# haesungpyun/seoul_tourism_recommendation_NGCF

Hardware: NVIDIA B200
Metric: ngcf_epoch_time_fwd_bwd_bpr (lower is better)
Workload: dtype f32

## Files before the change

### include/ngcf_b200.h

```cpp
#ifndef NGCF_B200_H
#define NGCF_B200_H

#include <stddef.h>
#include <stdint.h>

#ifdef __cplusplus
extern "C" {
#endif

#define NGCF_B200_ABI_VERSION 4
#define NGCF_MAX_LAYERS 8
#define NGCF_MAX_WIDTH 128
#define NGCF_ADAM_MAX_TENSORS 32

typedef enum {
    NGCF_OK = 0,
    NGCF_ERR_INVALID = -1,
    NGCF_ERR_CUDA = -2,
    NGCF_ERR_WORKSPACE = -3
} ngcf_status;

int ngcf_abi_version(void);
const char* ngcf_last_error(void);
uint64_t ngcf_launch_count(void);

int ngcf_coo_to_csr_workspace(int64_t nnz, int64_t n_rows, size_t* bytes_host);
int ngcf_coo_to_csr(const int64_t* coo_row, const int64_t* coo_col, int64_t nnz,
                    int64_t n_rows, int64_t n_cols, int transpose,
                    int32_t* rowptr ,
                    int32_t* colidx , int32_t* perm ,
                    void* workspace, size_t workspace_bytes, void* stream);

typedef struct ngcf_csr {
    int64_t n_rows;
    const int32_t* rowptr;
    const int32_t* ent;
    const int32_t* tiles;
    const int32_t* hub_of_row;
    const int32_t* hub_chunk_ptr;
    const int32_t* chunk_ptr;
    const int32_t* hub_ent;
    const int32_t* chunk_row;
    const int32_t* chunk_tiles;
    const int32_t* hub_rows;
    int32_t* hub_done;
    const uint32_t* key_l;
    const uint32_t* key_t;
    int64_t key_row_offset;
    int32_t n_tiles, n_hub, n_chunks, n_chunk_tiles;
    int32_t rowptr_nnz;
    const uint32_t* tile_hubmask;
} ngcf_csr;

int ngcf_spmm_split_threshold(void);
int ngcf_spmm_tile_rows(void);
int ngcf_spmm_tile_entries(void);

int ngcf_edge_entries(const int32_t* colidx, const float* coo_val, const int32_t* perm, const uint8_t* keep_mask,
                      int32_t* ent_out, int64_t nnz, void* stream);

int ngcf_feature_mix(float* user_w, int64_t n_user, int d,
                     const float* const* tables_host, const int* widths_host,
                     const int64_t* const* idx_host, const int64_t* u_id, int64_t batch,
                     float ratio, int32_t* winner, void* stream);

int ngcf_spmm(const ngcf_csr* csr_host, const float* X, int64_t ldx, int d,
              const float* addend, int64_t ld_add,
              const int32_t* slot, const float* gsum, int64_t ld_gsum,
              float* hub_partial,
              float drop_p, uint64_t seed, const uint64_t* seed_dev, int layer, int transposed, int64_t row_offset,
              const uint8_t* keep_bits, const int32_t* c_ent, const int32_t* c_cnt,
              float* Y, int64_t ldy, void* stream);

int ngcf_node_dropout_bits(const ngcf_csr* csr_host, float drop_p, uint64_t seed, const uint64_t* seed_dev,
                           int n_layers, int64_t row_offset, uint8_t* bits_as_L, uint8_t* bits_as_Lt, void* stream);

int ngcf_node_dropout_compact(const ngcf_csr* csr_host, float drop_p, uint64_t seed, const uint64_t* seed_dev,
                              int n_layers, int64_t row_offset,
                              int32_t* const* ent_as_L_host, int32_t* const* cnt_as_L_host,
                              int32_t* const* ent_as_Lt_host, int32_t* const* cnt_as_Lt_host, void* stream);

int ngcf_entry_keys(const ngcf_csr* csr_host, int64_t row_offset, uint32_t* key_l, uint32_t* key_t, void* stream);

int ngcf_plgraph_entries(int64_t n_user, int64_t n_item, int64_t n_edges, double alpha, uint64_t seed,
                         int64_t row0, int64_t n_rows, unsigned long long* total_dev,
                         unsigned long long* keys_or_null, int64_t capacity, void* stream);
int ngcf_build_tiles(const int32_t* rowptr, int64_t n_rows, int max_rows, int max_ent, int32_t* next_scratch,
                     int32_t* tiles_out, int64_t capacity, int32_t* count_out, void* stream);

int ngcf_exchange_flag_words(void);
int ngcf_push_rows(float* const* matrix_on_rank_host, uint32_t* const* flags_on_rank_host, uint32_t* local_state,
                   int world, int rank, int64_t row0, int64_t n_rows, int d, float* multicast_or_null, void* stream);
int ngcf_push_selected_rows(float* const* matrix_on_rank_host, uint32_t* const* flags_on_rank_host, uint32_t* local_state,
                            int world, int rank, int64_t row0, int64_t n_rows, int d,
                            const int64_t* const* lists_host, const int64_t* list_offsets_host,
                            const int64_t* list_sizes_host, int n_lists, float* multicast_or_null, void* stream);

int ngcf_pack_weights(const float* W1, const float* b1, const float* W2, const float* b2,
                      int d_in, int d_out, float* wcat , float* bias_eff ,
                      void* stream);
int ngcf_pack_weights_all(const float* const* W1_host, const float* const* b1_host, const float* const* W2_host,
                          const float* const* b2_host, const int* d_in_host, const int* d_out_host, int n_layers,
                          float* const* wcat_host, float* const* bias_host, void* stream);
int ngcf_dense_fwd(const float* S, const float* E, int64_t n_rows, int d_in, int d_out,
                   const float* wcat, const float* bias_eff, float slope,
                   const float* mess_mult, const uint32_t* mess_bits, float mess_p, uint64_t seed,
                   const uint64_t* seed_dev, int layer, int64_t row_offset, float* E_out, void* stream);

int ngcf_mess_dropout_bits(int64_t n_rows, int d_out, float mess_p, uint64_t seed, const uint64_t* seed_dev, int layer,
                           int64_t row_offset, uint32_t* bits, void* stream);

int ngcf_gather_concat(const float* const* layers_host, const int* dims_host, int n_layers_plus1,
                       const int64_t* rows, int64_t row_offset, int64_t n_out,
                       float* out, int64_t ld_out, void* stream);
int ngcf_gather_concat_sets(const float* const* layers_host, const int* dims_host, int n_layers_plus1,
                            const int64_t* const* rows_host, const int64_t* offsets_host, const int64_t* sizes_host,
                            float* const* outs_host, int n_sets, int64_t ld_out, void* stream);

int ngcf_bpr_fwd_bwd(const float* u, const float* p, const float* n, int64_t batch, int D,
                     float weight_decay, float batch_size_ctor, float reg_w_u, float reg_w_p, float reg_w_n,
                     float* loss, float* gu, float* gp, float* gn, void* stream);

int ngcf_rowgrad_scatter(const int64_t* const* rows_host, const int64_t* offsets_host,
                         const float* const* g_host, const int64_t* batch_host, int n_sets, int D,
                         int32_t* slot, float* gsum, void* stream);
int ngcf_rowgrad_normalize(const int64_t* const* rows_host, const int64_t* offsets_host,
                           const int64_t* batch_host, int n_sets, const float* const* layers_host,
                           const int* dims_host, int n_layers_plus1, const int32_t* slot, float* gsum, int D,
                           void* stream);
int ngcf_rowgrad_reset(const int64_t* const* rows_host, const int64_t* offsets_host,
                       const int64_t* batch_host, int n_sets, int32_t* slot, void* stream);

int ngcf_set_wgrad_stream(void* stream_or_null);
int ngcf_wgrad_stream_forked(void);
int ngcf_dense_bwd(const float* gE_next, const int32_t* slot, const float* gsum, int64_t ld_gsum, int col_off,
                   const float* E_out, const float* S, const float* E, int64_t n_rows, int d_in, int d_out,
                   const float* W1, const float* W2, float slope,
                   const float* mess_mult, const uint32_t* mess_bits, float mess_p, uint64_t seed,
                   const uint64_t* seed_dev, int layer, int64_t row_offset, int gh_normalized, float* gS, float* gEl,
                   float* gW1, float* gb1, float* gW2, float* gb2, float* gM_scratch, void* stream);

int ngcf_score_topk_workspace(int64_t n_users, int64_t n_items, int D, int k, size_t* bytes_host);
int ngcf_score_topk(const float* U, int64_t n_users, const float* I, int64_t n_items, int D, int k,
                    float* out_val , int64_t* out_idx ,
                    void* workspace, size_t workspace_bytes, void* stream);
int ngcf_score_topk_excluding(const float* U, int64_t n_users, const float* I, int64_t n_items, int D, int k,
                              const int64_t* excl_ptr , const int32_t* excl_idx,
                              float* out_val , int64_t* out_idx ,
                              void* workspace, size_t workspace_bytes, void* stream);

int ngcf_rank_metrics(const int64_t* topk_idx, int64_t n_users, int k, const int64_t* truth_ptr,
                      const int32_t* truth_idx, const int* Ks_host, int n_K, float* per_user, float* totals,
                      void* stream);

int ngcf_adam_step(float* const* params_host, float* const* grads_host, float* const* exp_avg_host,
                   float* const* exp_avg_sq_host, const int64_t* sizes_host, int n_tensors, double lr, double beta1,
                   double beta2, double eps, double weight_decay, int64_t step, const int64_t* step_dev,
                   int zero_grads, void* stream);

int ngcf_eval_groups(const float* u, const float* items, const int64_t* item_ids, const float* rating,
                     const int64_t* group_ptr, int64_t n_groups, int group, int D, int k_hr, int k_ndcg, float weight_decay,
                     float batch_size_ctor, float* bpr, float* hit, float* ndcg, float* rmse, float* scores,
                     float* totals, void* stream);

int ngcf_sample_negatives(const int32_t* pos_ptr, const int32_t* pos_idx, const int64_t* row_user, int64_t n_rows,
                          const int64_t* candidates, int n_candidates, int ng_ratio, uint64_t seed, int64_t* out,
// ... 15 lines not shown
```

### seoul_tourism_recommendation_ngcf_b200/NGCF.py

```python
from __future__ import annotations

import ctypes as C
import os

import numpy as np
import torch
import torch.nn as nn

import torch.distributed as dist

from . import _lib
from .plan import LaplacianPlan, node_dropout_bits, node_dropout_compact, spmm
from .sharded import RowShards, all_gather_rows

LEAKY_SLOPE = 0.2


def _stream() -> int:
    return _lib.current_stream()


class _Ctx:
    __slots__ = ("plan", "E", "S", "dims", "vals_f", "vals_b", "mess_mult", "mess_p", "seed", "seed_dev", "masked", "drop_p", "bits_f", "bits_b", "comp_f", "comp_b", "mess_bits",
                 "rows", "offsets", "W1", "W2", "fresh_key", "node_mode", "last_partial", "fm_stream")


def _capturing() -> bool:
    return torch.cuda.is_current_stream_capturing()


def _join_feature_mix(st):
    if st.fm_stream is not None:
        torch.cuda.current_stream().wait_stream(st.fm_stream)
        st.fm_stream = None


class _Propagate(torch.autograd.Function):

    @staticmethod
    def forward(ctx, mod, st: _Ctx, n_sets, user_w, item_w, *wb):
        lib = _lib.load()
        K = mod.n_layer
        W1, b1, W2, b2 = wb[0:K], wb[K:2 * K], wb[2 * K:3 * K], wb[3 * K:4 * K]
        dev = user_w.device
        sh = mod._shard
        N = mod.n_user + mod.n_item
        r0, nloc, nv = (sh.r0, sh.rows, sh.valid) if sh is not None else (0, N, N)
        X0 = mod._packed_table()
        if mod._snapshot:
            _join_feature_mix(st)
            X0 = X0.clone()
        st.E, st.S, st.W1, st.W2 = [X0], [], list(W1), list(W2)
        side = st.plan.fwd
        st.bits_f = st.bits_b = st.comp_f = st.comp_b = None
        st.node_mode = mod._node_mode
        st.last_partial = None
        if st.drop_p > 0:
            shared = st.plan.side(True, False) is side
            node_mode = mod._node_mode if all(d % 4 == 0 for d in st.dims) or mod._node_mode == "inkernel" else "bits"
            st.node_mode = node_mode
            if node_mode == "compact":
                st.comp_f, ct = node_dropout_compact(side, st.drop_p, st.seed, st.seed_dev, K, r0, as_L=True, as_Lt=shared)
                if shared:
                    st.comp_b = ct
            elif node_mode == "bits":
                st.bits_f, bt = node_dropout_bits(side, st.drop_p, st.seed, st.seed_dev, K, r0, as_L=True, as_Lt=shared)
                if shared:
                    st.bits_b = bt
        self_uses_mess_bits = mod._mess_bits
        st.mess_bits = [None] * K
        for k in range(K):
            if self_uses_mess_bits and st.mess_mult is None and st.mess_p[k] > 0 and st.dims[k + 1] % 4 == 0:
                bits = torch.empty(nloc * ((st.dims[k + 1] + 31) // 32), dtype=torch.int32, device=dev)
                _lib.check(lib.ngcf_mess_dropout_bits(nv, st.dims[k + 1], float(st.mess_p[k]), st.seed,
                                                      _lib.ptr(st.seed_dev), k, r0, bits.data_ptr(), _stream()),
                           "mess_dropout_bits")
                st.mess_bits[k] = bits
        wcats = [torch.empty(2 * st.dims[k] * st.dims[k + 1], dtype=torch.float32, device=dev) for k in range(K)]
        biases = [torch.empty(st.dims[k + 1], dtype=torch.float32, device=dev) for k in range(K)]
        _lib.check(lib.ngcf_pack_weights_all(_lib.ptr_array(W1), _lib.ptr_array(b1), _lib.ptr_array(W2), _lib.ptr_array(b2),
                                             _lib.int_array(st.dims[:K]), _lib.int_array(st.dims[1:]), K,
                                             _lib.ptr_array(wcats), _lib.ptr_array(biases), _stream()), "pack_weights_all")
        _join_feature_mix(st)
        for k in range(K):
            d_in, d_out = st.dims[k], st.dims[k + 1]
            vals = st.vals_f[k] if st.vals_f is not None else None
            S = spmm(side, vals, st.E[k], d_in, drop_p=st.drop_p, seed=st.seed, seed_dev=st.seed_dev, layer=k,
                     row_offset=r0, keep_bits=st.bits_f,
                     compact=st.comp_f[k] if st.comp_f is not None else None)
            wcat, bias = wcats[k], biases[k]
            xkey = None
            if sh is None:
                Xn = En = torch.empty(N, d_out, dtype=torch.float32, device=dev)
            elif mod._xchg is not None and d_out % 4 == 0:
                xkey = ("E", k + 1)
                Xn = mod._xchg.matrix(xkey, sh.N_pad, d_out)
                En = Xn[r0:r0 + nloc]
            else:
                Xn = torch.empty(sh.N_pad, d_out, dtype=torch.float32, device=dev)
                En = torch.zeros(nloc, d_out, dtype=torch.float32, device=dev) if nv < nloc else \
                    torch.empty(nloc, d_out, dtype=torch.float32, device=dev)
            mm = st.mess_mult[k] if st.mess_mult is not None else None
            E_loc = st.E[k][r0:r0 + nloc]
            _lib.check(lib.ngcf_dense_fwd(S.data_ptr(), E_loc.data_ptr(), nv, d_in, d_out, wcat.data_ptr(),
                                          bias.data_ptr(), LEAKY_SLOPE, _lib.ptr(mm[r0:r0 + nloc] if mm is not None else None),
                                          _lib.ptr(st.mess_bits[k]), float(st.mess_p[k]), st.seed, _lib.ptr(st.seed_dev), k, r0, En.data_ptr(),
                                          _stream()),
                       "dense_fwd")
            if xkey is not None and k == K - 1:
                mod._xchg.push_selected(xkey, r0, nloc, st.rows[:n_sets], st.offsets[:n_sets])
                st.last_partial = xkey
            elif xkey is not None:
                mod._xchg.push(xkey, r0, nloc)
            elif sh is not None:
                all_gather_rows(Xn, En, mod._group)
            st.S.append(S)
            st.E.append(Xn)
        D = sum(st.dims)
        layers, dims = _lib.ptr_array(st.E), _lib.int_array(st.dims)
        outs = [torch.empty(st.rows[j].numel(), D, dtype=torch.float32, device=dev) for j in range(n_sets)]
        _lib.check(lib.ngcf_gather_concat_sets(layers, dims, K + 1, _lib.ptr_array(st.rows[:n_sets]),
                                               _lib.i64_array(st.offsets[:n_sets]),
                                               _lib.i64_array([r.numel() for r in st.rows[:n_sets]]), _lib.ptr_array(outs),
                                               n_sets, D, _stream()), "gather_concat_sets")
        ctx.st, ctx.mod, ctx.n_sets = st, mod, n_sets
        return tuple(outs)

    @staticmethod
    def backward(ctx, *gouts):
        lib = _lib.load()
        st, mod, n_sets = ctx.st, ctx.mod, ctx.n_sets
        mod._check_fresh(st, "loss.backward()")
        K, dims = mod.n_layer, st.dims
        dev = st.E[0].device
        sh = mod._shard
        N = mod.n_user + mod.n_item
        r0, nloc, nv, N_all = (sh.r0, sh.rows, sh.valid, sh.N_pad) if sh is not None else (0, N, N, N)
        D = sum(dims)
        g = [(go.contiguous() if go is not None else torch.zeros(st.rows[j].numel(), D, device=dev))
             for j, go in enumerate(gouts)]
        batch = [r.numel() for r in st.rows[:n_sets]]
        rows_h, offs_h = _lib.ptr_array(st.rows[:n_sets]), _lib.i64_array(st.offsets[:n_sets])
        g_h, batch_h = _lib.ptr_array(g), _lib.i64_array(batch)
        slot = mod._slot_map(N_all, dev)
        gsum = torch.empty(sum(batch), D, dtype=torch.float32, device=dev)
        _lib.check(lib.ngcf_rowgrad_scatter(rows_h, offs_h, g_h, batch_h, n_sets, D, slot.data_ptr(),
                                            gsum.data_ptr(), _stream()), "rowgrad_scatter")
        _lib.check(lib.ngcf_rowgrad_normalize(rows_h, offs_h, batch_h, n_sets, _lib.ptr_array(st.E), _lib.int_array(dims),
                                              K + 1, slot.data_ptr(), gsum.data_ptr(), D, _stream()), "rowgrad_normalize")
        slot_loc = slot[r0:r0 + nloc]
        sizes = [dims[k + 1] * dims[k] for k in range(K)]
        n_flat = 2 * sum(sizes) + 2 * sum(dims[1:])
        if sh is not None and mod._xchg is not None:
            f_pad = (n_flat + 3) // 4 * 4
            wg_all = mod._xchg.matrix(("wgrad", f_pad), sh.world, f_pad)
            flat = wg_all[sh.rank, :n_flat]
            flat.zero_()
        else:
            wg_all = None
            flat = torch.zeros(n_flat, dtype=torch.float32, device=dev)
        gW1, gW2, gb1, gb2, o = [], [], [], [], 0
        for k in range(K):
            gW1.append(flat[o:o + sizes[k]].view(dims[k + 1], dims[k])); o += sizes[k]
            gW2.append(flat[o:o + sizes[k]].view(dims[k + 1], dims[k])); o += sizes[k]
            gb1.append(flat[o:o + dims[k + 1]]); o += dims[k + 1]
            gb2.append(flat[o:o + dims[k + 1]]); o += dims[k + 1]
        side = st.plan.side(True, st.vals_b is not None)
        if st.drop_p > 0 and st.node_mode == "compact" and st.comp_b is None:
            _, st.comp_b = node_dropout_compact(side, st.drop_p, st.seed, st.seed_dev, K, r0, as_L=False, as_Lt=True)
        if st.drop_p > 0 and st.node_mode == "bits" and st.bits_b is None:
            _, st.bits_b = node_dropout_bits(side, st.drop_p, st.seed, st.seed_dev, K, r0, as_L=False, as_Lt=True)
        gE_next = None
        col_off = D
        overlap = _capturing() or (sh is not None and mod._xchg is not None)
        if overlap:
            if mod._side_stream is None:
                mod._side_stream = torch.cuda.Stream(device=dev)
            _lib.check(lib.ngcf_set_wgrad_stream(mod._side_stream.cuda_stream), "set_wgrad_stream")
            lib.ngcf_wgrad_stream_forked()
            gM_keep = []
        else:
            gM_scratch = torch.empty(nloc, max(dims[1:]), dtype=torch.float32, device=dev)
        for k in range(K - 1, -1, -1):
            d_in, d_out = dims[k], dims[k + 1]
            col_off -= d_out
            peer = sh is not None and mod._xchg is not None and d_in % 4 == 0
            if peer:
                gS_all = mod._xchg.matrix(("gS", d_in), N_all, d_in)
                gS = gS_all[r0:r0 + nloc]
            else:
                gS = torch.empty(nloc, d_in, dtype=torch.float32, device=dev)
            if peer and k == 0:
                gE0_all = mod._xchg.matrix(("gE0", d_in), N_all, d_in)
                gEl = gE0_all[r0:r0 + nloc]
            else:
                gEl = torch.empty(nloc, d_in, dtype=torch.float32, device=dev)
            mm = st.mess_mult[k] if st.mess_mult is not None else None
            if overlap:
                gM_scratch = torch.empty(nloc, dims[k + 1], dtype=torch.float32, device=dev)
                gM_keep.append(gM_scratch)
            _lib.check(lib.ngcf_dense_bwd(_lib.ptr(gE_next), slot_loc.data_ptr(), gsum.data_ptr(), D, col_off,
                                          st.E[k + 1][r0:r0 + nloc].data_ptr(), st.S[k].data_ptr(),
                                          st.E[k][r0:r0 + nloc].data_ptr(), nv, d_in, d_out,
                                          st.W1[k].data_ptr(), st.W2[k].data_ptr(), LEAKY_SLOPE,
                                          _lib.ptr(mm[r0:r0 + nloc] if mm is not None else None),
                                          _lib.ptr(st.mess_bits[k]), float(st.mess_p[k]), st.seed,
                                          _lib.ptr(st.seed_dev), k, r0, 1, gS.data_ptr(),
                                          gEl.data_ptr(),
                                          gW1[k].data_ptr(), gb1[k].data_ptr(), gW2[k].data_ptr(), gb2[k].data_ptr(),
                                          gM_scratch.data_ptr(), _stream()), "dense_bwd")
            if peer:
                mod._xchg.push(("gS", d_in), r0, nloc)
            elif sh is not None:
                gS_all = torch.empty(N_all, d_in, dtype=torch.float32, device=dev)
                all_gather_rows(gS_all, gS, mod._group)
            else:
                gS_all = gS
            vals = st.vals_b[k] if st.vals_b is not None else None
            last = (k == 0)
            gE_next = spmm(side, vals, gS_all, d_in, addend=gEl, slot=slot_loc if last else None,
                           gsum=gsum if last else None, drop_p=st.drop_p, seed=st.seed, seed_dev=st.seed_dev, layer=k,
                           transposed=True, row_offset=r0, keep_bits=st.bits_b,
                           compact=st.comp_b[k] if st.comp_b is not None else None)
            if mod._trace is not None:
                mod._trace.append(dict(k=k, gS=gS.clone(), gEl=gEl.clone(), gE=gE_next.clone()))
        if overlap:
            _lib.check(lib.ngcf_set_wgrad_stream(None), "set_wgrad_stream")
            if lib.ngcf_wgrad_stream_forked():
                torch.cuda.current_stream().wait_stream(mod._side_stream)
        _lib.check(lib.ngcf_rowgrad_reset(rows_h, offs_h, batch_h, n_sets, slot.data_ptr(), _stream()),
                   "rowgrad_reset")
        if sh is not None:
            if mod._xchg is not None and dims[0] % 4 == 0:
                mod._xchg.push(("gE0", dims[0]), r0, nloc)
                gE0 = gE0_all.clone()
            else:
                gE0 = torch.empty(N_all, dims[0], dtype=torch.float32, device=dev)
                all_gather_rows(gE0, gE_next, mod._group)
            if wg_all is not None:
                mod._xchg.push(("wgrad", wg_all.shape[1]), sh.rank, 1)
                total = wg_all.sum(0)[:n_flat]
                gW1, gW2, gb1, gb2, o = [], [], [], [], 0
                for k in range(K):
                    gW1.append(total[o:o + sizes[k]].view(dims[k + 1], dims[k])); o += sizes[k]
                    gW2.append(total[o:o + sizes[k]].view(dims[k + 1], dims[k])); o += sizes[k]
                    gb1.append(total[o:o + dims[k + 1]]); o += dims[k + 1]
                    gb2.append(total[o:o + dims[k + 1]]); o += dims[k + 1]
            else:
                dist.all_reduce(flat, group=mod._group)
        else:
            gE0 = gE_next
        gU, gI = gE0[:mod.n_user], gE0[mod.n_user:N]
        return (None, None, None, gU, gI, *gW1, *gb1, *gW2, *gb2)


class NGCF(nn.Module):

    def __init__(self, embed_size: int, layer_size: list, node_dropout: float, mess_dropout: list,
                 emb_ratio: float, lap_list: list, num_dict: dict, batch_size: int, device, *, rng: str = "device",
                 snapshot: bool = False):
        super().__init__()
        if rng not in ("device", "reference"):
            raise ValueError("rng must be 'device' or 'reference'")
        self.n_user = int(num_dict['user'])
        self.n_item = int(num_dict['item'])
        self.emb_size = int(embed_size)
        self.weight_size = list(layer_size)
        self.n_layer = len(self.weight_size)
# ... 59 lines not shown
        self.w2_list = nn.Sequential(*w2)
        self.node_dropout_list = nn.Sequential(*nd)
        self.mess_dropout_list = nn.Sequential(*md)

    def shard(self, group=None, shards=None):
        if not dist.is_initialized():
            raise RuntimeError("NGCF.shard() needs an initialised torch.distributed process group")
        if self.rng != "device":
            raise ValueError("row-sharded runs need rng='device' (masks are keyed on global coordinates in-kernel)")
        world, rank = dist.get_world_size(group), dist.get_rank(group)
        self._shard = shards if shards is not None else RowShards(self.n_user + self.n_item, world, rank)
        if self._shard.N != self.n_user + self.n_item or self._shard.world != world or self._shard.rank != rank:
            raise ValueError("the shard descriptor does not match this model / process group")
        self._group = group
        self._plans, self._table, self._slot = {}, None, None
        self._xchg = None
        if world > 1 and os.environ.get("NGCF_B200_EXCHANGE", "peer") != "nccl":
            try:
                from .sharded import PeerExchange
                self._xchg = PeerExchange(group, self.user_embedding.weight.device)
            except Exception as e:
                self._xchg_error = f"{type(e).__name__}: {e}"
                ok = torch.tensor([0], device=self.user_embedding.weight.device)
            else:
                ok = torch.tensor([1], device=self.user_embedding.weight.device)
            dist.all_reduce(ok, op=dist.ReduceOp.MIN, group=group)
            if int(ok) == 0:
                self._xchg = None
        if self._xchg is None and world > 1 and not getattr(self._shard, "equal", True):
            raise RuntimeError("unequal row blocks (BalancedShards) need the peer-memory exchange, which is not available "
                               "here: " + getattr(self, "_xchg_error", "disabled by NGCF_B200_EXCHANGE=nccl"))
        return self

    def exchange_description(self) -> str:
        if self._shard is None:
            return "single GPU"
        if self._xchg is not None:
            how = "NVLS multicast stores (multimem.st)" if self._xchg.multicast() else "peer-memory stores"
            return (f"contiguous row blocks; per-layer exchange of E / gS / table-gradient rows by {how} over NVLink "
                    "(ngcf_push_rows on symmetric memory, no NCCL collective anywhere in the step; the last layer's "
                    "output travels for the batch rows only; W/b gradients: one more push + a rank-ordered sum)")
        return "equal row blocks, per-layer NCCL all-gather of E / gS, all-reduce of W/b grads"

    def _packed_table(self) -> torch.Tensor:
        u, i = self.user_embedding.weight, self.item_embedding.weight
        d = self.emb_size
        adjacent = (u.is_contiguous() and i.is_contiguous() and u.dtype == torch.float32 and
                    u.data_ptr() + self.n_user * d * 4 == i.data_ptr() and
                    getattr(self, "_table", None) is not None and self._table.data_ptr() == u.data_ptr())
        if not adjacent:
            n_rows = self._shard.N_pad if self._shard is not None else self.n_user + self.n_item
            table = torch.zeros(n_rows, d, dtype=torch.float32, device=u.device)
            table[:self.n_user].copy_(u.data)
            table[self.n_user:self.n_user + self.n_item].copy_(i.data)
            u.data = table[:self.n_user]
            i.data = table[self.n_user:self.n_user + self.n_item]
            self._table = table
        return self._table if self._shard is None else self._table

    def _slot_map(self, N, dev):
        if self._slot is None or self._slot.device != dev or self._slot.numel() != N:
            self._slot = torch.full((N,), -1, dtype=torch.int32, device=dev)
        return self._slot

    def _plan(self, year_idx: int, dev) -> LaplacianPlan:
        L = self.lap_list[year_idx]
        p = self._plans.get(year_idx)
        if p is None or p.src is not L or p.coo_val.device != dev:
            p = LaplacianPlan(L, dev, shard=self._shard)
            self._plans[year_idx] = p
        return p

    def _reference_node_masks(self, nnz: int, dev):
        alive = np.arange(nnz)
        out = []
        for _ in range(self.n_layer):
            m = nn.Dropout(self.node_dropout)(torch.tensor(np.ones(alive.size))).type(torch.bool).numpy()
            alive = alive[m]
            full = np.zeros(nnz, dtype=np.uint8)
            full[alive] = 1
            out.append(torch.from_numpy(full).to(dev))
        return out

    @_lib.on_device
    def forward(self, year, u_id, age, sex, month, day, dow, pos_item, neg_item, node_flag):
        lib = _lib.load()
        dev = self.user_embedding.weight.device
        if dev.type != "cuda":
            raise RuntimeError("NGCF (B200) runs on a CUDA device only; there is no CPU fallback. "
                               "Move the module with .to('cuda').")
        K, N = self.n_layer, self.n_user + self.n_item
        if (self._side_stream is None or self._side_stream.device != dev) and not _capturing():
            self._side_stream, self._side_stream3 = (torch.cuda.Stream(device=dev) for _ in range(2))

        def ix(t):
            return t.to(device=dev, dtype=torch.int64).contiguous()

        u_id, pos_item = ix(u_id), ix(pos_item)
        feats_idx = [ix(age), ix(sex), ix(month), ix(day), ix(dow)]
        has_neg = len(neg_item) > 0
        neg_item = ix(neg_item) if has_neg else None
        year_idx = int(year.min()) % 18

        table = self._packed_table()
        if self._winner is None or self._winner.device != dev or self._winner.numel() != self.n_user:
            self._winner = torch.full((self.n_user,), -1, dtype=torch.int32, device=dev)
        tabs = [self.age_emb.weight, self.sex_emb.weight, self.month_emb.weight, self.day_emb.weight, self.dow_emb.weight]
        def mix():
            _lib.check(lib.ngcf_feature_mix(table.data_ptr(), self.n_user, self.emb_size, _lib.ptr_array(tabs),
                                            _lib.int_array(self.feat_widths), _lib.ptr_array(feats_idx), u_id.data_ptr(),
                                            u_id.numel(), float(self.emb_ratio), self._winner.data_ptr(), _stream()),
                       "feature_mix")

        fm_stream = None
        if self._shard is None and _capturing() and bool(node_flag) and \
                (self.node_dropout or 0) > 0 and self.rng == "device":
            main = torch.cuda.current_stream()
            if self._side_stream3 is None:
                self._side_stream3 = torch.cuda.Stream(device=dev)
            self._side_stream3.wait_stream(main)
            with torch.cuda.stream(self._side_stream3):
                mix()
            fm_stream = self._side_stream3
        else:
            mix()

        self._mix_count += 1
        st = _Ctx()
        st.fm_stream = fm_stream
        st.fresh_key = self._fresh_key()
        st.plan = plan = self._plan(year_idx, dev)
        if self._shard is not None and "edge_keep" in (self._inject or {}):
            raise ValueError("explicit edge masks are not supported in row-sharded mode")
        if plan.N != N:
            raise ValueError(f"Laplacian is {plan.N}x{plan.N} but n_user+n_item = {N}")
        st.dims = [self.emb_size] + self.weight_size
        inj = self._inject or {}
        st.masked = bool(node_flag) and (self.node_dropout is not None) and \
            (self.node_dropout > 0 or "edge_keep" in inj)
        st.vals_f = st.vals_b = None
        st.drop_p = 0.0
        masks = None
        if st.masked:
            if "edge_keep" in inj:
                masks = [m.to(device=dev, dtype=torch.uint8).contiguous() for m in inj["edge_keep"]]
            elif self.rng == "reference":
                masks = self._reference_node_masks(plan.nnz, dev)
            else:
                st.drop_p = float(self.node_dropout)
        st.mess_mult = None
        st.mess_p = [0.0] * K
        if "mess_mult" in inj:
            st.mess_mult = [m.to(device=dev, dtype=torch.float32).contiguous() for m in inj["mess_mult"]]
        elif self.training and self.mess_dropout is not None:
            st.mess_p = [float(p) for p in self.mess_dropout[:K]]
        need_seed = st.drop_p > 0 or any(p > 0 for p in st.mess_p)
        if not need_seed:
            st.seed = 0
        elif self.rng == "reference":
            if self._seed_gen is None:
                self._seed_gen = torch.Generator().manual_seed(torch.initial_seed() & (2 ** 63 - 1))
            st.seed = int(torch.randint(0, 2 ** 62, (1,), generator=self._seed_gen).item())
        else:
            st.seed = int(torch.randint(0, 2 ** 62, (1,)).item())
        st.seed_dev = self._seed_dev if need_seed else None
        if masks is not None:
            st.vals_f = [plan.entries(plan.fwd, masks[k]) for k in range(K)]
            st.vals_b = [plan.entries(plan.bwd, masks[k]) for k in range(K)]
        st.rows = [u_id, pos_item] + ([neg_item] if has_neg else [])
        st.offsets = [0, self.n_user] + ([self.n_user] if has_neg else [])

        wb = [l.weight for l in self.w1_list] + [l.bias for l in self.w1_list] + \
             [l.weight for l in self.w2_list] + [l.bias for l in self.w2_list]
        outs = _Propagate.apply(self, st, len(st.rows), self.user_embedding.weight, self.item_embedding.weight, *wb)
        self._last, self._all_E = st, None
        u_embeddings, pos_i_embeddings = outs[0], outs[1]
        neg_i_embeddings = outs[2] if has_neg else torch.empty(0)
        return u_embeddings, pos_i_embeddings, neg_i_embeddings

    def _fresh_key(self):
        return (self._mix_count, _lib.param_epoch(), self.user_embedding.weight._version,
                self.item_embedding.weight._version)

    def _check_fresh(self, st, what: str):
        if self._snapshot or st.fresh_key == self._fresh_key():
            return
        why = "the step that produced it also ran the optimizer" if st.fresh_key is None else \
            "another forward (feature mix) or an optimizer step ran since"
        raise RuntimeError(f"NGCF (B200): {what} needs the embedding table as the forward left it, but {why}. "
                           "Run the forward again, or construct the module with snapshot=True to keep a per-forward "
                           "copy like the reference's torch.cat (NGCF.py:120).")

    @_lib.on_device
    def _materialize(self):
        if self._last is None:
            raise AttributeError("all_users_emb / all_items_emb exist after the first forward (NGCF.py:148-149)")
        if self._all_E is None:
            self._check_fresh(self._last, "all_users_emb / all_items_emb")
            if self._last.last_partial is not None:
                sh = self._shard
                self._xchg.push(self._last.last_partial, sh.r0, sh.rows)
                self._last.last_partial = None
            st, lib = self._last, _lib.load()
            N, D = self.n_user + self.n_item, sum(st.dims)
            out = torch.empty(N, D, dtype=torch.float32, device=st.E[0].device)
            _lib.check(lib.ngcf_gather_concat(_lib.ptr_array(st.E), _lib.int_array(st.dims), self.n_layer + 1, None, 0,
                                              N, out.data_ptr(), D, _stream()), "gather_concat")
            self._all_E = out
        return self._all_E

    @property
    def all_users_emb(self):
        return self._materialize()[:self.n_user, :]

    @property
    def all_items_emb(self):
        return self._materialize()[self.n_user:, :]
```

### seoul_tourism_recommendation_ngcf_b200/_lib.py

```python
from __future__ import annotations

import ctypes as C
import os

_PKG = os.path.dirname(os.path.abspath(__file__))
LIB_PATH = os.environ.get("NGCF_B200_LIB") or os.path.join(_PKG, "libngcf_b200.so")

_vp, _i64, _i32, _f32, _u64, _sz = C.c_void_p, C.c_int64, C.c_int32, C.c_float, C.c_uint64, C.c_size_t



class NgcfCsr(C.Structure):
    _fields_ = [("n_rows", _i64), ("rowptr", _vp), ("ent", _vp), ("tiles", _vp),
                ("hub_of_row", _vp), ("hub_chunk_ptr", _vp), ("chunk_ptr", _vp), ("hub_ent", _vp),
                ("chunk_row", _vp), ("chunk_tiles", _vp), ("hub_rows", _vp), ("hub_done", _vp), ("key_l", _vp), ("key_t", _vp), ("key_row_offset", _i64),
                ("n_tiles", _i32), ("n_hub", _i32), ("n_chunks", _i32),
                ("n_chunk_tiles", _i32), ("rowptr_nnz", _i32), ("tile_hubmask", _vp)]


_csr_p = C.POINTER(NgcfCsr)

SIGNATURES = {
    "ngcf_abi_version": [],
    "ngcf_last_error": [],
    "ngcf_launch_count": [],
    "ngcf_coo_to_csr_workspace": [_i64, _i64, C.POINTER(_sz)],
    "ngcf_coo_to_csr": [_vp, _vp, _i64, _i64, _i64, C.c_int, _vp, _vp, _vp, _vp, _sz, _vp],
    "ngcf_edge_entries": [_vp, _vp, _vp, _vp, _vp, _i64, _vp],
    "ngcf_spmm_tile_rows": [],
    "ngcf_spmm_tile_entries": [],
    "ngcf_feature_mix": [_vp, _i64, C.c_int, C.POINTER(_vp), C.POINTER(C.c_int), C.POINTER(_vp), _vp, _i64, _f32,
                         _vp, _vp],
    "ngcf_spmm_split_threshold": [],
    "ngcf_spmm": [_csr_p, _vp, _i64, C.c_int, _vp, _i64, _vp, _vp, _i64, _vp, _f32, _u64, _vp, C.c_int, C.c_int, _i64,
                  _vp, _vp, _vp, _vp, _i64, _vp],
    "ngcf_entry_keys": [_csr_p, _i64, _vp, _vp, _vp],
    "ngcf_node_dropout_compact": [_csr_p, _f32, _u64, _vp, C.c_int, _i64, C.POINTER(_vp), C.POINTER(_vp), C.POINTER(_vp),
                                  C.POINTER(_vp), _vp],
    "ngcf_node_dropout_bits": [_csr_p, _f32, _u64, _vp, C.c_int, _i64, _vp, _vp, _vp],
    "ngcf_pack_weights": [_vp, _vp, _vp, _vp, C.c_int, C.c_int, _vp, _vp, _vp],
    "ngcf_pack_weights_all": [C.POINTER(_vp), C.POINTER(_vp), C.POINTER(_vp), C.POINTER(_vp), C.POINTER(C.c_int),
                              C.POINTER(C.c_int), C.c_int, C.POINTER(_vp), C.POINTER(_vp), _vp],
    "ngcf_dense_fwd": [_vp, _vp, _i64, C.c_int, C.c_int, _vp, _vp, _f32, _vp, _vp, _f32, _u64, _vp, C.c_int, _i64, _vp,
                       _vp],
    "ngcf_mess_dropout_bits": [_i64, C.c_int, _f32, _u64, _vp, C.c_int, _i64, _vp, _vp],
    "ngcf_gather_concat": [C.POINTER(_vp), C.POINTER(C.c_int), C.c_int, _vp, _i64, _i64, _vp, _i64, _vp],
    "ngcf_gather_concat_sets": [C.POINTER(_vp), C.POINTER(C.c_int), C.c_int, C.POINTER(_vp), C.POINTER(_i64), C.POINTER(_i64),
                                C.POINTER(_vp), C.c_int, _i64, _vp],
    "ngcf_bpr_fwd_bwd": [_vp, _vp, _vp, _i64, C.c_int, _f32, _f32, _f32, _f32, _f32, _vp, _vp, _vp, _vp, _vp],
    "ngcf_rowgrad_scatter": [C.POINTER(_vp), C.POINTER(_i64), C.POINTER(_vp), C.POINTER(_i64), C.c_int, C.c_int, _vp,
                             _vp, _vp],
    "ngcf_rowgrad_reset": [C.POINTER(_vp), C.POINTER(_i64), C.POINTER(_i64), C.c_int, _vp, _vp],
    "ngcf_dense_bwd": [_vp, _vp, _vp, _i64, C.c_int, _vp, _vp, _vp, _i64, C.c_int, C.c_int, _vp, _vp, _f32, _vp, _vp, _f32,
                       _u64, _vp, C.c_int, _i64, C.c_int, _vp, _vp, _vp, _vp, _vp, _vp, _vp, _vp],
    "ngcf_set_wgrad_stream": [_vp],
    "ngcf_wgrad_stream_forked": [],
    "ngcf_rowgrad_normalize": [C.POINTER(_vp), C.POINTER(_i64), C.POINTER(_i64), C.c_int, C.POINTER(_vp),
                               C.POINTER(C.c_int), C.c_int, _vp, _vp, C.c_int, _vp],
    "ngcf_adam_step": [C.POINTER(_vp), C.POINTER(_vp), C.POINTER(_vp), C.POINTER(_vp), C.POINTER(_i64), C.c_int,
                       C.c_double, C.c_double, C.c_double, C.c_double, C.c_double, _i64, _vp, C.c_int, _vp],
    "ngcf_debug_bwd_timeline": [C.c_int, _vp],
    "ngcf_debug_spmm_timeline": [_vp],
    "ngcf_debug_compact_timeline": [_vp],
    "ngcf_score_topk_workspace": [_i64, _i64, C.c_int, C.c_int, C.POINTER(_sz)],
    "ngcf_eval_groups": [_vp, _vp, _vp, _vp, _vp, _i64, C.c_int, C.c_int, C.c_int, C.c_int, _f32, _f32, _vp, _vp, _vp, _vp, _vp,
                         _vp, _vp],
    "ngcf_sample_negatives": [_vp, _vp, _vp, _i64, _vp, C.c_int, C.c_int, _u64, _vp, _vp, _vp],
    "ngcf_laplacian_entries": [_vp, _vp, _vp, _i64, _i64, _i64, _vp, _vp, _vp, _vp, _vp],
    "ngcf_plgraph_entries": [_i64, _i64, _i64, C.c_double, _u64, _i64, _i64, _vp, _vp, _i64, _vp],
    "ngcf_build_tiles": [_vp, _i64, C.c_int, C.c_int, _vp, _vp, _i64, _vp, _vp],
    "ngcf_exchange_flag_words": [],
    "ngcf_push_rows": [C.POINTER(_vp), C.POINTER(_vp), _vp, C.c_int, C.c_int, _i64, _i64, C.c_int, _vp, _vp],
    "ngcf_push_selected_rows": [C.POINTER(_vp), C.POINTER(_vp), _vp, C.c_int, C.c_int, _i64, _i64, C.c_int, C.POINTER(_vp),
                                C.POINTER(_i64), C.POINTER(_i64), C.c_int, _vp, _vp],
    "ngcf_score_topk": [_vp, _i64, _vp, _i64, C.c_int, C.c_int, _vp, _vp, _vp, _sz, _vp],
    "ngcf_score_topk_excluding": [_vp, _i64, _vp, _i64, C.c_int, C.c_int, _vp, _vp, _vp, _vp, _vp, _sz, _vp],
    "ngcf_rank_metrics": [_vp, _i64, C.c_int, _vp, _vp, C.POINTER(C.c_int), C.c_int, _vp, _vp, _vp],
}

_lib = None


def load() -> C.CDLL:
    global _lib
    if _lib is not None:
        return _lib
    if not os.path.exists(LIB_PATH):
        raise RuntimeError(
            f"{LIB_PATH} is missing: the NGCF B200 hot path has no CPU/PyTorch fallback. "
            "Build it with `python -m seoul_tourism_recommendation_ngcf_b200.build` (needs nvcc, targets sm_100a).")
    lib = C.CDLL(LIB_PATH)
    for name, argtypes in SIGNATURES.items():
        fn = getattr(lib, name)
        fn.argtypes = argtypes
        fn.restype = {"ngcf_last_error": C.c_char_p, "ngcf_launch_count": C.c_uint64}.get(name, C.c_int)
    _lib = lib
    return lib


def check(rc: int, what: str = "") -> None:
    if rc != 0:
        msg = load().ngcf_last_error()
        raise RuntimeError(f"ngcf_b200 {what} failed (status {rc}): {msg.decode() if msg else '?'}")


def ptr(t) -> int | None:
    return None if t is None else t.data_ptr()


def ptr_array(tensors):
    return (_vp * len(tensors))(*[None if t is None else t.data_ptr() for t in tensors])


def ptr_array_int(addrs):
    return (_vp * len(addrs))(*[int(a) for a in addrs])


def int_array(vals):
    return (C.c_int * len(vals))(*[int(v) for v in vals])


# ... 48 lines not shown
```

### seoul_tourism_recommendation_ngcf_b200/csrc/bpr.cu

```cuda
#include "common.cuh"

namespace {

struct GatherArgs {
    const float* layer[NGCF_MAX_LAYERS + 1];
    int dim[NGCF_MAX_LAYERS + 1];
    int n;
    const int64_t* rows;
    int64_t row_offset;
    int64_t n_out;
    float* out;
    int64_t ld_out;
};

struct GatherSetsArgs {
    const float* layer[NGCF_MAX_LAYERS + 1];
    int dim[NGCF_MAX_LAYERS + 1];
    int n;
    const int64_t* rows[4];
    int64_t row_offset[4];
    int64_t base[5];
    float* out[4];
    int n_sets;
    int64_t ld_out;
// ... 30 lines not shown
    if (b >= a.n_out) return;
    gather_row(a, (a.rows ? a.rows[b] : b) + a.row_offset, a.out + b * a.ld_out, lane);
}
__global__ void gather_concat_sets_kernel(GatherSetsArgs a) {
    const int64_t b = (blockIdx.x * (int64_t)blockDim.x + threadIdx.x) >> 5;
    const int lane = threadIdx.x & 31;
    if (b >= a.base[a.n_sets]) return;
    int j = 0;
    while (b >= a.base[j + 1]) ++j;
    const int64_t i = b - a.base[j];
    gather_row(a, a.rows[j][i] + a.row_offset[j], a.out[j] + i * a.ld_out, lane);
}

constexpr int BPR_WARPS = 8;

__global__ void __launch_bounds__(BPR_WARPS * 32)
bpr_kernel(const float* __restrict__ u, const float* __restrict__ p, const float* __restrict__ n, int64_t batch, int D,
           float wd, float wu, float wp, float wn, float inv_bs, float* __restrict__ loss, float* __restrict__ gu,
           float* __restrict__ gp, float* __restrict__ gn) {
    __shared__ float part[BPR_WARPS];
    const int warp = threadIdx.x >> 5, lane = threadIdx.x & 31;
    const int64_t b = (int64_t)blockIdx.x * BPR_WARPS + warp;
    float contrib = 0.f;
    if (b < batch) {
        const float* ur = u + b * D;
        const float* pr = p + b * D;
        const float* nr = n + b * D;
        float xp = 0.f, xn = 0.f, su = 0.f, sp = 0.f, sn = 0.f;
        for (int c = lane; c < D; c += 32) {
            const float a = ur[c], bb = pr[c], cc = nr[c];
            xp = fmaf(a, bb, xp); xn = fmaf(a, cc, xn);
            su = fmaf(a, a, su); sp = fmaf(bb, bb, sp); sn = fmaf(cc, cc, sn);
        }
        xp = warp_sum(xp); xn = warp_sum(xn); su = warp_sum(su); sp = warp_sum(sp); sn = warp_sum(sn);
        const float x = fabsf(xp) - fabsf(xn);
        const float logsig = fminf(x, 0.f) - log1pf(expf(-fabsf(x)));
        contrib = (-logsig + wd * (wu * su + wp * sp + wn * sn)) * inv_bs;
        if (gu) {
            const float c = -1.f / (1.f + expf(x));
            const float sgp = xp > 0.f ? 1.f : (xp < 0.f ? -1.f : 0.f);
            const float sgn = xn > 0.f ? 1.f : (xn < 0.f ? -1.f : 0.f);
            const float cp = c * sgp * inv_bs, cn = -c * sgn * inv_bs;
            const float ru = 2.f * wd * wu * inv_bs, rp = 2.f * wd * wp * inv_bs, rn = 2.f * wd * wn * inv_bs;
            for (int col = lane; col < D; col += 32) {
                const float a = ur[col], bb = pr[col], cc = nr[col];
                gu[b * D + col] = cp * bb + cn * cc + ru * a;
                gp[b * D + col] = cp * a + rp * bb;
                gn[b * D + col] = cn * a + rn * cc;
            }
        }
    }
    if (lane == 0) part[warp] = contrib;
    __syncthreads();
    if (threadIdx.x == 0) {
        float s = 0.f;
#pragma unroll
        for (int w = 0; w < BPR_WARPS; ++w) s += part[w];
        atomicAdd(loss, s);
    }
}

struct RowSets {
    const int64_t* rows[4];
    int64_t offset[4];
    const float* g[4];
    int64_t batch[4];
    int64_t base[4];
    int n_sets;
    int64_t total;
};

__device__ __forceinline__ bool locate(const RowSets& s, int64_t i, int& j, int64_t& b) {
    if (i >= s.total) return false;
    j = 0;
    while (j + 1 < s.n_sets && i >= s.base[j + 1]) ++j;
    b = i - s.base[j];
    return true;
}

__global__ void rowgrad_claim_kernel(RowSets s, int32_t* __restrict__ slot) {
    const int64_t i = blockIdx.x * (int64_t)blockDim.x + threadIdx.x;
    int j; int64_t b;
    if (!locate(s, i, j, b)) return;
    slot[s.rows[j][b] + s.offset[j]] = (int32_t)i;
}

__global__ void rowgrad_accum_kernel(RowSets s, int D, const int32_t* __restrict__ slot, float* __restrict__ gsum) {
    const int64_t i = (blockIdx.x * (int64_t)blockDim.x + threadIdx.x) >> 5;
    const int lane = threadIdx.x & 31;
    int j; int64_t b;
    if (!locate(s, i, j, b)) return;
    const int32_t w = slot[s.rows[j][b] + s.offset[j]];
    const float* g = s.g[j] + b * D;
    float* dst = gsum + (int64_t)w * D;
    for (int c = lane; c < D; c += 32) atomicAdd(dst + c, g[c]);
}

struct NormArgs {
    const float* layer[NGCF_MAX_LAYERS + 1];
    int dim[NGCF_MAX_LAYERS + 1];
    int n;
};
__global__ void rowgrad_normalize_kernel(RowSets s, NormArgs L, int D, const int32_t* __restrict__ slot,
                                         float* __restrict__ gsum) {
    const int64_t i = (blockIdx.x * (int64_t)blockDim.x + threadIdx.x) >> 5;
    const int lane = threadIdx.x & 31;
    int j; int64_t b;
    if (!locate(s, i, j, b)) return;
    const int64_t row = s.rows[j][b] + s.offset[j];
    if (slot[row] != (int32_t)i) return;
    float* g = gsum + i * D;
    int col = L.dim[0];
    for (int k = 1; k < L.n; ++k) {
        const int d = L.dim[k];
        const float* e = L.layer[k] + row * d;
        float nrm2 = 0.f, dot = 0.f;
        for (int c = lane; c < d; c += 32) {
            nrm2 = fmaf(e[c], e[c], nrm2);
            dot = fmaf(e[c], g[col + c], dot);
        }
        nrm2 = warp_sum(nrm2);
        dot = warp_sum(dot);
        const float n = fmaxf(sqrtf(nrm2), 1e-12f);
        const float hd = dot / n;
        for (int c = lane; c < d; c += 32) g[col + c] = (g[col + c] - (e[c] / n) * hd) / n;
        col += d;
    }
}

__global__ void rowgrad_reset_kernel(RowSets s, int32_t* __restrict__ slot) {
    const int64_t i = blockIdx.x * (int64_t)blockDim.x + threadIdx.x;
    int j; int64_t b;
    if (!locate(s, i, j, b)) return;
    slot[s.rows[j][b] + s.offset[j]] = -1;
}

int fill_sets(RowSets& s, const int64_t* const* rows_host, const int64_t* offsets_host, const float* const* g_host,
              const int64_t* batch_host, int n_sets) {
    NGCF_REQUIRE(rows_host && offsets_host && batch_host, "rowgrad: null host array");
    NGCF_REQUIRE(n_sets >= 1 && n_sets <= 4, "rowgrad: n_sets %d not in [1,4]", n_sets);
    s.n_sets = n_sets;
    s.total = 0;
    for (int j = 0; j < 4; ++j) {
        s.rows[j] = nullptr; s.g[j] = nullptr; s.offset[j] = 0; s.batch[j] = 0; s.base[j] = 0;
    }
    for (int j = 0; j < n_sets; ++j) {
        NGCF_REQUIRE(batch_host[j] >= 0 && (batch_host[j] == 0 || rows_host[j]), "rowgrad: set %d has no rows", j);
        s.rows[j] = rows_host[j];
        s.offset[j] = offsets_host[j];
        s.g[j] = g_host ? g_host[j] : nullptr;
        s.batch[j] = batch_host[j];
        s.base[j] = s.total;
        s.total += batch_host[j];
    }
    NGCF_REQUIRE(s.total < ((int64_t)1 << 31), "rowgrad: too many rows");
    return NGCF_OK;
}

}

extern "C" int ngcf_gather_concat(const float* const* layers_host, const int* dims_host, int n_layers_plus1,
                                  const int64_t* rows, int64_t row_offset, int64_t n_out, float* out, int64_t ld_out,
                                  void* stream) {
    NGCF_REQUIRE(layers_host && dims_host && out, "gather_concat: null pointer");
    NGCF_REQUIRE(n_layers_plus1 >= 1 && n_layers_plus1 <= NGCF_MAX_LAYERS + 1, "gather_concat: %d blocks", n_layers_plus1);
    GatherArgs a;
    int D = 0;
    for (int k = 0; k < n_layers_plus1; ++k) {
        NGCF_REQUIRE(layers_host[k] && dims_host[k] > 0 && dims_host[k] <= NGCF_MAX_WIDTH, "gather_concat: bad block %d", k);
        a.layer[k] = layers_host[k];
        a.dim[k] = dims_host[k];
        D += dims_host[k];
    }
    NGCF_REQUIRE(ld_out >= D, "gather_concat: ld_out %lld < total width %d", (long long)ld_out, D);
    a.n = n_layers_plus1; a.rows = rows; a.row_offset = row_offset; a.n_out = n_out; a.out = out; a.ld_out = ld_out;
    if (n_out <= 0) return NGCF_OK;
    gather_concat_kernel<<<(unsigned)ceil_div64(n_out * 32, 256), 256, 0, as_stream(stream)>>>(a);
    NGCF_LAUNCH_OK("gather_concat_kernel");
    return NGCF_OK;
}

extern "C" int ngcf_gather_concat_sets(const float* const* layers_host, const int* dims_host, int n_layers_plus1,
                                       const int64_t* const* rows_host, const int64_t* offsets_host,
                                       const int64_t* sizes_host, float* const* outs_host, int n_sets, int64_t ld_out,
                                       void* stream) {
    NGCF_REQUIRE(layers_host && dims_host && rows_host && offsets_host && sizes_host && outs_host, "gather_concat_sets: null pointer");
    NGCF_REQUIRE(n_layers_plus1 >= 1 && n_layers_plus1 <= NGCF_MAX_LAYERS + 1, "gather_concat_sets: %d blocks", n_layers_plus1);
    NGCF_REQUIRE(n_sets >= 1 && n_sets <= 4, "gather_concat_sets: n_sets %d not in [1,4]", n_sets);
    GatherSetsArgs a{};
    int D = 0;
    for (int k = 0; k < n_layers_plus1; ++k) {
        NGCF_REQUIRE(layers_host[k] && dims_host[k] > 0 && dims_host[k] <= NGCF_MAX_WIDTH, "gather_concat_sets: bad block %d", k);
        a.layer[k] = layers_host[k];
        a.dim[k] = dims_host[k];
        D += dims_host[k];
    }
    NGCF_REQUIRE(ld_out >= D, "gather_concat_sets: ld_out %lld < total width %d", (long long)ld_out, D);
    a.n = n_layers_plus1; a.n_sets = n_sets; a.ld_out = ld_out;
    int64_t total = 0;
    for (int j = 0; j < n_sets; ++j) {
        NGCF_REQUIRE(sizes_host[j] >= 0 && (sizes_host[j] == 0 || (rows_host[j] && outs_host[j])), "gather_concat_sets: set %d", j);
        a.rows[j] = rows_host[j]; a.row_offset[j] = offsets_host[j]; a.out[j] = outs_host[j];
        a.base[j] = total;
        total += sizes_host[j];
    }
    for (int j = n_sets; j <= 4; ++j) a.base[j] = total;
    if (total == 0) return NGCF_OK;
    gather_concat_sets_kernel<<<(unsigned)ceil_div64(total * 32, 256), 256, 0, as_stream(stream)>>>(a);
    NGCF_LAUNCH_OK("gather_concat_sets_kernel");
    return NGCF_OK;
}

extern "C" int ngcf_bpr_fwd_bwd(const float* u, const float* p, const float* n, int64_t batch, int D,
                                float weight_decay, float batch_size_ctor, float reg_w_u, float reg_w_p,
                                float reg_w_n, float* loss, float* gu, float* gp, float* gn, void* stream) {
    NGCF_REQUIRE(u && p && n && loss, "bpr: null pointer");
    NGCF_REQUIRE((gu && gp && gn) || (!gu && !gp && !gn), "bpr: give all three gradient buffers or none");
    NGCF_REQUIRE(batch >= 0 && D > 0 && batch_size_ctor != 0.f, "bpr: bad sizes");
    cudaStream_t st = as_stream(stream);
    NGCF_CUDA(cudaMemsetAsync(loss, 0, sizeof(float), st));
    if (batch == 0) return NGCF_OK;
    bpr_kernel<<<(unsigned)ceil_div64(batch, BPR_WARPS), BPR_WARPS * 32, 0, st>>>(
        u, p, n, batch, D, weight_decay, reg_w_u, reg_w_p, reg_w_n, 1.0f / batch_size_ctor, loss, gu, gp, gn);
    NGCF_LAUNCH_OK("bpr_kernel");
    return NGCF_OK;
}

extern "C" int ngcf_rowgrad_scatter(const int64_t* const* rows_host, const int64_t* offsets_host,
                                    const float* const* g_host, const int64_t* batch_host, int n_sets, int D,
                                    int32_t* slot, float* gsum, void* stream) {
    NGCF_REQUIRE(g_host && slot && gsum && D > 0, "rowgrad_scatter: null pointer");
    RowSets s;
    int rc = fill_sets(s, rows_host, offsets_host, g_host, batch_host, n_sets);
    if (rc != NGCF_OK) return rc;
    for (int j = 0; j < n_sets; ++j) NGCF_REQUIRE(s.batch[j] == 0 || s.g[j], "rowgrad_scatter: set %d has no gradient", j);
    if (s.total == 0) return NGCF_OK;
    cudaStream_t st = as_stream(stream);
    NGCF_CUDA(cudaMemsetAsync(gsum, 0, sizeof(float) * (size_t)s.total * D, st));
    rowgrad_claim_kernel<<<(unsigned)ceil_div64(s.total, 256), 256, 0, st>>>(s, slot);
    NGCF_LAUNCH_OK("rowgrad_claim_kernel");
    rowgrad_accum_kernel<<<(unsigned)ceil_div64(s.total * 32, 256), 256, 0, st>>>(s, D, slot, gsum);
    NGCF_LAUNCH_OK("rowgrad_accum_kernel");
    return NGCF_OK;
}

extern "C" int ngcf_rowgrad_normalize(const int64_t* const* rows_host, const int64_t* offsets_host,
                                      const int64_t* batch_host, int n_sets, const float* const* layers_host,
                                      const int* dims_host, int n_layers_plus1, const int32_t* slot, float* gsum,
                                      int D, void* stream) {
    NGCF_REQUIRE(slot && gsum && layers_host && dims_host, "rowgrad_normalize: null pointer");
    NGCF_REQUIRE(n_layers_plus1 >= 1 && n_layers_plus1 <= NGCF_MAX_LAYERS + 1, "rowgrad_normalize: %d blocks", n_layers_plus1);
    RowSets s;
    int rc = fill_sets(s, rows_host, offsets_host, nullptr, batch_host, n_sets);
    if (rc != NGCF_OK) return rc;
    NormArgs L;
    int total = 0;
    for (int k = 0; k < n_layers_plus1; ++k) {
        NGCF_REQUIRE(layers_host[k] && dims_host[k] > 0 && dims_host[k] <= NGCF_MAX_WIDTH, "rowgrad_normalize: bad block %d", k);
        L.layer[k] = layers_host[k];
        L.dim[k] = dims_host[k];
        total += dims_host[k];
    }
    L.n = n_layers_plus1;
    NGCF_REQUIRE(total == D, "rowgrad_normalize: block widths sum to %d, D = %d", total, D);
    if (s.total == 0 || n_layers_plus1 == 1) return NGCF_OK;
    rowgrad_normalize_kernel<<<(unsigned)ceil_div64(s.total * 32, 256), 256, 0, as_stream(stream)>>>(s, L, D, slot, gsum);
    NGCF_LAUNCH_OK("rowgrad_normalize_kernel");
    return NGCF_OK;
}

extern "C" int ngcf_rowgrad_reset(const int64_t* const* rows_host, const int64_t* offsets_host,
                                  const int64_t* batch_host, int n_sets, int32_t* slot, void* stream) {
    NGCF_REQUIRE(slot, "rowgrad_reset: null pointer");
    RowSets s;
    int rc = fill_sets(s, rows_host, offsets_host, nullptr, batch_host, n_sets);
    if (rc != NGCF_OK) return rc;
    if (s.total == 0) return NGCF_OK;
    rowgrad_reset_kernel<<<(unsigned)ceil_div64(s.total, 256), 256, 0, as_stream(stream)>>>(s, slot);
    NGCF_LAUNCH_OK("rowgrad_reset_kernel");
    return NGCF_OK;
}
```

### seoul_tourism_recommendation_ngcf_b200/csrc/dense.cu

```cuda
#include "common.cuh"

namespace {

__global__ void pack_weights_kernel(const float* __restrict__ W1, const float* __restrict__ b1,
                                    const float* __restrict__ W2, const float* __restrict__ b2, int d_in, int d_out,
                                    float* __restrict__ wcat, float* __restrict__ bias_eff) {
    const int total = 2 * d_in * d_out;
    for (int i = blockIdx.x * blockDim.x + threadIdx.x; i < total; i += gridDim.x * blockDim.x) {
        const int k = i / d_out, o = i % d_out;
        wcat[i] = k < d_in ? W1[o * d_in + k] : W2[o * d_in + (k - d_in)];
    }
    for (int o = blockIdx.x * blockDim.x + threadIdx.x; o < d_out; o += gridDim.x * blockDim.x)
        bias_eff[o] = 2.0f * b1[o] + b2[o];
}

struct PackAllArgs {
    const float* W1[NGCF_MAX_LAYERS];
    const float* b1[NGCF_MAX_LAYERS];
    const float* W2[NGCF_MAX_LAYERS];
    const float* b2[NGCF_MAX_LAYERS];
    float* wcat[NGCF_MAX_LAYERS];
    float* bias[NGCF_MAX_LAYERS];
    int d_in[NGCF_MAX_LAYERS], d_out[NGCF_MAX_LAYERS];
};
// ... 330 lines not shown
                               fmaf(t2[r][2], e4.z, t1[r][2]), fmaf(t2[r][3], e4.w, t1[r][3])};
                float ge[4] = {fmaf(t2[r][0], s4.x, t1[r][0]), fmaf(t2[r][1], s4.y, t1[r][1]),
                               fmaf(t2[r][2], s4.z, t1[r][2]), fmaf(t2[r][3], s4.w, t1[r][3])};
                if (vec_in) {
                    st_f4(a.gS + row * d_in + j0, make_float4(gs[0], gs[1], gs[2], gs[3]));
                    st_f4(a.gEl + row * d_in + j0, make_float4(ge[0], ge[1], ge[2], ge[3]));
                } else {
#pragma unroll
                    for (int c = 0; c < 4; ++c)
                        if (j0 + c < d_in) {
                            a.gS[row * d_in + j0 + c] = gs[c];
                            a.gEl[row * d_in + j0 + c] = ge[c];
                        }
                }
            }
        }

        for (int r = 0; r < R; ++r) {
            const float4 s4 = ld_f4(Ss + r * LD + tx * 4), e4 = ld_f4(Es + r * LD + tx * 4);
            const float x1[4] = {s4.x + e4.x, s4.y + e4.y, s4.z + e4.z, s4.w + e4.w};
            const float x2[4] = {s4.x * e4.x, s4.y * e4.y, s4.z * e4.z, s4.w * e4.w};
#pragma unroll
            for (int q = 0; q < OB; ++q) {
                const float4 g4 = ld_f4(GM + r * LD + (ty + TY * q) * 4);
                const float g[4] = {g4.x, g4.y, g4.z, g4.w};
#pragma unroll
                for (int o = 0; o < 4; ++o)
#pragma unroll
                    for (int j = 0; j < 4; ++j) {
                        accW1[q][o][j] = fmaf(g[o], x1[j], accW1[q][o][j]);
                        accW2[q][o][j] = fmaf(g[o], x2[j], accW2[q][o][j]);
                    }
            }
        }
    }

#pragma unroll
    for (int q = 0; q < OB; ++q)
#pragma unroll
        for (int o = 0; o < 4; ++o) {
            const int oo = (ty + TY * q) * 4 + o;
            if (oo >= d_out) continue;
#pragma unroll
            for (int j = 0; j < 4; ++j) {
                const int jj = tx * 4 + j;
                if (jj < d_in) {
                    atomicAdd(a.gW1 + oo * d_in + jj, accW1[q][o][j]);
                    atomicAdd(a.gW2 + oo * d_in + jj, accW2[q][o][j]);
                }
            }
        }
    __syncthreads();
#pragma unroll
    for (int q = 0; q < QN; ++q) CS[warp * DC + lane + 32 * q] = colsum[q];
    __syncthreads();
    for (int c = tid; c < d_out; c += THREADS) {
        float s = 0.f;
        for (int w = 0; w < NW; ++w) s += CS[w * DC + c];
        atomicAdd(a.gb2 + c, s);
        atomicAdd(a.gb1 + c, 2.0f * s);
    }
}

template <typename K>
int set_smem(K kernel, size_t bytes) {
    if (bytes > 48 * 1024) {
        cudaError_t e = cudaFuncSetAttribute(kernel, cudaFuncAttributeMaxDynamicSharedMemorySize, (int)bytes);
        if (e != cudaSuccess) {
            ngcf_set_error("cudaFuncSetAttribute(%zu bytes smem) failed: %s", bytes, cudaGetErrorString(e));
            return NGCF_ERR_CUDA;
        }
    }
    return NGCF_OK;
}

inline bool aligned16(const void* p) { return (reinterpret_cast<uintptr_t>(p) & 15) == 0; }

}

bool ngcf_dense_fwd_tc_eligible(int d_in, int d_out);
int ngcf_dense_fwd_tc(const float* S, const float* E, int64_t n_rows, int d_in, int d_out, const float* wcat,
                      const float* bias_eff, float slope, const float* mess_mult, const uint32_t* mess_bits, float mess_p,
                      uint64_t seed,
                      const uint64_t* seed_dev, int layer, int64_t row_offset, float* E_out, cudaStream_t st);

bool ngcf_dense_bwd_tc_eligible(int d_in, int d_out, int gh_normalized);
int ngcf_dense_bwd_tc(const float* gE_next, const int32_t* slot, const float* gsum, int64_t ld_gsum, int col_off,
                      const float* E_out, const float* S, const float* E, int64_t n_rows, int d_in, int d_out,
                      const float* W1, const float* W2, float slope, const float* mess_mult, const uint32_t* mess_bits,
                      float mess_p,
                      uint64_t seed, const uint64_t* seed_dev, int layer, int64_t row_offset, int gh_normalized, float* gS, float* gEl,
                      float* gW1, float* gb1, float* gW2, float* gb2, float* gM_scratch, cudaStream_t st);

extern "C" int ngcf_pack_weights(const float* W1, const float* b1, const float* W2, const float* b2, int d_in,
                                 int d_out, float* wcat, float* bias_eff, void* stream) {
    NGCF_REQUIRE(W1 && b1 && W2 && b2 && wcat && bias_eff, "pack_weights: null pointer");
    NGCF_REQUIRE(d_in > 0 && d_in <= NGCF_MAX_WIDTH && d_out > 0 && d_out <= NGCF_MAX_WIDTH,
                 "pack_weights: widths %d -> %d not in [1,%d]", d_in, d_out, NGCF_MAX_WIDTH);
    pack_weights_kernel<<<32, 256, 0, as_stream(stream)>>>(W1, b1, W2, b2, d_in, d_out, wcat, bias_eff);
    NGCF_LAUNCH_OK("pack_weights_kernel");
    return NGCF_OK;
}

extern "C" int ngcf_pack_weights_all(const float* const* W1_host, const float* const* b1_host, const float* const* W2_host,
                                     const float* const* b2_host, const int* d_in_host, const int* d_out_host, int n_layers,
                                     float* const* wcat_host, float* const* bias_host, void* stream) {
    NGCF_REQUIRE(W1_host && b1_host && W2_host && b2_host && d_in_host && d_out_host && wcat_host && bias_host,
                 "pack_weights_all: null pointer");
    NGCF_REQUIRE(n_layers >= 1 && n_layers <= NGCF_MAX_LAYERS, "pack_weights_all: %d layers", n_layers);
    PackAllArgs a{};
    for (int l = 0; l < n_layers; ++l) {
        NGCF_REQUIRE(W1_host[l] && b1_host[l] && W2_host[l] && b2_host[l] && wcat_host[l] && bias_host[l],
                     "pack_weights_all: null pointer (layer %d)", l);
        NGCF_REQUIRE(d_in_host[l] > 0 && d_in_host[l] <= NGCF_MAX_WIDTH && d_out_host[l] > 0 && d_out_host[l] <= NGCF_MAX_WIDTH,
                     "pack_weights_all: widths %d -> %d not in [1,%d]", d_in_host[l], d_out_host[l], NGCF_MAX_WIDTH);
        a.W1[l] = W1_host[l]; a.b1[l] = b1_host[l]; a.W2[l] = W2_host[l]; a.b2[l] = b2_host[l];
        a.wcat[l] = wcat_host[l]; a.bias[l] = bias_host[l]; a.d_in[l] = d_in_host[l]; a.d_out[l] = d_out_host[l];
    }
    pack_weights_all_kernel<<<dim3(32, (unsigned)n_layers), 256, 0, as_stream(stream)>>>(a);
    NGCF_LAUNCH_OK("pack_weights_all_kernel");
    return NGCF_OK;
}

extern "C" int ngcf_dense_fwd(const float* S, const float* E, int64_t n_rows, int d_in, int d_out, const float* wcat,
                              const float* bias_eff, float slope, const float* mess_mult, const uint32_t* mess_bits, float mess_p,
                      uint64_t seed,
                              const uint64_t* seed_dev, int layer, int64_t row_offset, float* E_out, void* stream) {
    NGCF_REQUIRE(S && E && wcat && bias_eff && E_out, "dense_fwd: null pointer");
    NGCF_REQUIRE(d_in > 0 && d_in <= NGCF_MAX_WIDTH && d_out > 0 && d_out <= NGCF_MAX_WIDTH,
                 "dense_fwd: widths %d -> %d not in [1,%d]", d_in, d_out, NGCF_MAX_WIDTH);
    NGCF_REQUIRE(mess_p >= 0.f && mess_p < 1.f, "dense_fwd: mess_p %f not in [0,1)", mess_p);
    NGCF_REQUIRE(n_rows >= 0 && n_rows < ((int64_t)1 << 31), "dense_fwd: n_rows %lld", (long long)n_rows);
    if (n_rows == 0) return NGCF_OK;
    if (ngcf_dense_fwd_tc_eligible(d_in, d_out) && aligned16(S) && aligned16(E) &&
        aligned16(E_out) && (!mess_mult || aligned16(mess_mult)))
        return ngcf_dense_fwd_tc(S, E, n_rows, d_in, d_out, wcat, bias_eff, slope, mess_mult, mess_bits, mess_p, seed, seed_dev,
                                 layer, row_offset, E_out, as_stream(stream));
    FwdArgs a{S, E, n_rows, d_in, d_out, wcat, bias_eff, slope, mess_mult, mess_bits, mess_p, seed, seed_dev, layer, E_out,
              (2 * d_in + 3) & ~3, (int)ceil_div64(n_rows, FWD_R), row_offset};
    const int ncg = d_out <= 64 ? 1 : 2;
    const size_t smem = sizeof(float) * ((size_t)a.KP * 64 * ncg + (size_t)FWD_R * (a.KP + 4) + 64 * ncg);
    const int per_sm = smem > 110 * 1024 ? 1 : (smem > 72 * 1024 ? 2 : 3);
    const int grid = (int)min((int64_t)a.n_tiles, (int64_t)ngcf_num_sms() * per_sm);
    int rc;
    if (ncg == 1) {
        if ((rc = set_smem(dense_fwd_kernel<1>, smem)) != NGCF_OK) return rc;
        dense_fwd_kernel<1><<<grid, FWD_THREADS, smem, as_stream(stream)>>>(a);
    } else {
        if ((rc = set_smem(dense_fwd_kernel<2>, smem)) != NGCF_OK) return rc;
        dense_fwd_kernel<2><<<grid, FWD_THREADS, smem, as_stream(stream)>>>(a);
    }
    NGCF_LAUNCH_OK("dense_fwd_kernel");
    return NGCF_OK;
}

extern "C" int ngcf_dense_bwd(const float* gE_next, const int32_t* slot, const float* gsum, int64_t ld_gsum,
                              int col_off, const float* E_out, const float* S, const float* E, int64_t n_rows,
                              int d_in, int d_out, const float* W1, const float* W2, float slope,
                              const float* mess_mult, const uint32_t* mess_bits, float mess_p, uint64_t seed,
                              const uint64_t* seed_dev, int layer, int64_t row_offset, int gh_normalized, float* gS,
                              float* gEl, float* gW1, float* gb1, float* gW2, float* gb2, float* gM_scratch, void* stream) {
    NGCF_REQUIRE(E_out && S && E && W1 && W2 && gS && gEl && gW1 && gb1 && gW2 && gb2, "dense_bwd: null pointer");
    NGCF_REQUIRE(!slot || gsum, "dense_bwd: slot given without gsum");
    NGCF_REQUIRE(d_in > 0 && d_in <= NGCF_MAX_WIDTH && d_out > 0 && d_out <= NGCF_MAX_WIDTH,
                 "dense_bwd: widths %d -> %d not in [1,%d]", d_in, d_out, NGCF_MAX_WIDTH);
    NGCF_REQUIRE(mess_p >= 0.f && mess_p < 1.f, "dense_bwd: mess_p %f not in [0,1)", mess_p);
    NGCF_REQUIRE(n_rows >= 0 && n_rows < ((int64_t)1 << 31), "dense_bwd: n_rows %lld", (long long)n_rows);
    if (n_rows == 0) return NGCF_OK;
    if (gM_scratch && ngcf_dense_bwd_tc_eligible(d_in, d_out, gh_normalized) && aligned16(S) &&
        aligned16(E) && aligned16(gS) && aligned16(gEl) && aligned16(gM_scratch))
        return ngcf_dense_bwd_tc(gE_next, slot, gsum, ld_gsum, col_off, E_out, S, E, n_rows, d_in, d_out, W1, W2,
                                 slope, mess_mult, mess_bits, mess_p, seed, seed_dev, layer, row_offset, gh_normalized, gS,
                                 gEl, gW1, gb1, gW2, gb2, gM_scratch, as_stream(stream));
    BwdArgs a{gE_next, slot, gsum, ld_gsum, col_off, E_out, S, E, n_rows, d_in, d_out, W1, W2, slope, mess_mult,
              mess_bits, mess_p, seed, seed_dev, layer, gS, gEl, gW1, gb1, gW2, gb2, 0, row_offset, gh_normalized};
    int rc;
    if (d_in <= 64 && d_out <= 64) {
        constexpr int DC = 64, R = 64, T = 256;
        a.n_tiles = (int)ceil_div64(n_rows, R);
        const size_t smem = sizeof(float) * (2 * DC * DC + 3 * R * (DC + 4) + (T / 32) * DC);
        const int grid = (int)min((int64_t)a.n_tiles, (int64_t)ngcf_num_sms() * 2);
        if ((rc = set_smem(dense_bwd_kernel<DC, R, T>, smem)) != NGCF_OK) return rc;
        dense_bwd_kernel<DC, R, T><<<grid, T, smem, as_stream(stream)>>>(a);
    } else {
        constexpr int DC = 128, R = 32, T = 512;
        a.n_tiles = (int)ceil_div64(n_rows, R);
        const size_t smem = sizeof(float) * (2 * DC * DC + 3 * R * (DC + 4) + (T / 32) * DC);
        const int grid = (int)min((int64_t)a.n_tiles, (int64_t)ngcf_num_sms());
        if ((rc = set_smem(dense_bwd_kernel<DC, R, T>, smem)) != NGCF_OK) return rc;
        dense_bwd_kernel<DC, R, T><<<grid, T, smem, as_stream(stream)>>>(a);
    }
    NGCF_LAUNCH_OK("dense_bwd_kernel");
    return NGCF_OK;
}

namespace {
__global__ void mess_bits_kernel(int64_t n_rows, int d_out, int words, float p, uint64_t seed0, const uint64_t* seed_dev,
                                 int layer, int64_t row_off, uint32_t* __restrict__ bits) {
    const int64_t i = blockIdx.x * (int64_t)blockDim.x + threadIdx.x;
    if (i >= n_rows * words) return;
    const int64_t row = i / words;
    const int w = (int)(i % words);
    const uint64_t seed = ngcf_seed(seed0, seed_dev);
    uint32_t out = 0;
#pragma unroll
    for (int q = 0; q < 8; ++q) {
        const int col = w * 32 + q * 4;
        if (col < d_out) {
            const float4 m = mess_multiplier4(p, seed, layer, (uint64_t)((row + row_off) * d_out + col) >> 2);
            out |= (m.x != 0.f ? 1u : 0u) << (q * 4) | (m.y != 0.f ? 2u : 0u) << (q * 4) | (m.z != 0.f ? 4u : 0u) << (q * 4) |
                   (m.w != 0.f ? 8u : 0u) << (q * 4);
        }
    }
    bits[i] = out;
}
}

extern "C" int ngcf_mess_dropout_bits(int64_t n_rows, int d_out, float mess_p, uint64_t seed, const uint64_t* seed_dev,
                                      int layer, int64_t row_offset, uint32_t* bits, void* stream) {
    NGCF_REQUIRE(bits && n_rows >= 0, "mess_dropout_bits: null pointer");
    NGCF_REQUIRE(d_out > 0 && d_out <= NGCF_MAX_WIDTH && d_out % 4 == 0, "mess_dropout_bits: width %d", d_out);
    NGCF_REQUIRE(mess_p > 0.f && mess_p < 1.f, "mess_dropout_bits: mess_p %f not in (0,1)", mess_p);
    if (n_rows == 0) return NGCF_OK;
    const int words = (d_out + 31) / 32;
    mess_bits_kernel<<<(unsigned)ceil_div64(n_rows * words, 256), 256, 0, as_stream(stream)>>>(
        n_rows, d_out, words, mess_p, seed, seed_dev, layer, row_offset, bits);
    NGCF_LAUNCH_OK("mess_bits_kernel");
    return NGCF_OK;
}
```

### seoul_tourism_recommendation_ngcf_b200/csrc/dense_tc.cu

```cuda
#include <stdlib.h>

#include "tc.cuh"
#include "tmap.h"

namespace {

using namespace tc;

__device__ long long g_bwd_dbg[4][8][8];
__device__ int g_bwd_dbg_on = 0;
#define BWD_STAMP(role, it, k)                                                   \
    do {                                                                         \
        if (dbg && lane == 0 && (it) < 8) g_bwd_dbg[role][it][k] = clock64();    \
    } while (0)

constexpr int TC_ROWS = 128;
constexpr int TC_EPI_WARPS = 4;
constexpr int TC_LOAD_WARPS = 8;
constexpr int TC_THREADS = (TC_EPI_WARPS + 1 + TC_LOAD_WARPS) * 32;
constexpr int TC_MAX_KB = 4;
constexpr int TC_A_BLOCK = TC_ROWS * 128;

struct FwdTcArgs {
    const float* S;
    const float* E;
    int64_t n_rows;
    int d_in, d_out;
    const float* wcat;
    const float* bias_eff;
    float slope;
    const float* mess_mult;
    const uint32_t* mess_bits;
    float mess_p;
    uint64_t seed;
    const uint64_t* seed_dev;
    int layer;
    float* E_out;
    int n_tiles;
    int64_t row_off;
    int64_t ld_in;
    int in_off, w_row1, w_row2, out_off, d_out_full, mode;
};
enum { FW_SINGLE = 0, FW_PARTIAL = 1, FW_FINAL = 2 };

constexpr int FW_EPI_WARPS = 8;
constexpr int FW_MMA_WARP = FW_EPI_WARPS;

__device__ __forceinline__ int stage_off(int r, int c) { return r * 32 + ((c ^ (r & 7)) << 2); }

enum { MM_NONE = 0, MM_MULT = 1, MM_BITS = 2, MM_HASH = 3 };
static inline int mess_mode(const float* mess_mult, const uint32_t* mess_bits, float mess_p) {
    return mess_mult ? MM_MULT : (mess_p > 0.f ? (mess_bits ? MM_BITS : MM_HASH) : MM_NONE);
}

template <int MM>
__device__ __forceinline__ void fwd_epilogue_role(const FwdTcArgs& a, float* stage, const float* bias_s, uint64_t* tmem_full,
                                                  uint64_t* tmem_empty, uint32_t tmem_base, int n_my, int warp, int lane,
                                                  bool dbg) {
    const int d_out = a.d_out;
    const uint64_t seed = MM == MM_HASH ? ngcf_seed(a.seed, a.seed_dev) : 0ull;
    const uint32_t thr = ngcf_threshold16(a.mess_p);
    float* st = stage + warp * 32 * 32;
    const int quarter = warp & 3, c = warp >> 2;
    const int rr = lane >> 3, c4 = lane & 7;
    const bool has_chunk = c * 32 < d_out;
    const float inv_keep = 1.0f / (1.0f - a.mess_p);
    for (int it = 0; it < n_my; ++it) {
        const int tile = blockIdx.x + it * gridDim.x;
        const int buf = it & 1;
        BWD_STAMP(0, it, 0);
        mbar_wait(&tmem_full[buf], (it >> 1) & 1);
        BWD_STAMP(0, it, 1);
        tc_fence_after_sync();
        float v[32];
        if (has_chunk) tmem_ld_32x32(tmem_base + ((uint32_t)(quarter * 32) << 16) + buf * 64 + c * 32, v);
        tc_fence_before_sync();
        __syncwarp();
        if (lane == 0) mbar_arrive(&tmem_empty[buf]);
        BWD_STAMP(0, it, 3);
        if (!has_chunk) continue;
        const int64_t row_base = (int64_t)tile * TC_ROWS + quarter * 32;
#pragma unroll
        for (int j = 0; j < 32; j += 4)
            st_f4(st + stage_off(lane, j >> 2), make_float4(v[j], v[j + 1], v[j + 2], v[j + 3]));
        __syncwarp();
        float4 r4[8];
#pragma unroll
        for (int i = 0; i < 8; ++i) r4[i] = ld_f4(st + stage_off(i * 4 + rr, c4));
        __syncwarp();
        BWD_STAMP(0, it, 4);
        const int col = c * 32 + c4 * 4;
        if (col < d_out) {
            const int gcol = a.out_off + col;
            const float4 b4 = *reinterpret_cast<const float4*>(bias_s + col);
            const int words = (a.d_out_full + 31) >> 5;
#pragma unroll
            for (int i = 0; i < 8; ++i) {
                const int64_t row = row_base + i * 4 + rr;
                if (row >= a.n_rows) continue;
                float* dst = a.E_out + row * a.d_out_full + gcol;
                float4 x = r4[i];
                if (a.mode == FW_PARTIAL) {
                    st_f4(dst, x);
                    continue;
                }
                if (a.mode == FW_FINAL) {
                    const float4 prev = ld_f4(dst);
                    x.x += prev.x; x.y += prev.y; x.z += prev.z; x.w += prev.w;
                }
                x.x += b4.x; x.y += b4.y; x.z += b4.z; x.w += b4.w;
                x.x = x.x > 0.f ? x.x : a.slope * x.x;
                x.y = x.y > 0.f ? x.y : a.slope * x.y;
                x.z = x.z > 0.f ? x.z : a.slope * x.z;
                x.w = x.w > 0.f ? x.w : a.slope * x.w;
                if (MM == MM_BITS) {
                    const uint32_t w = a.mess_bits[row * words + (gcol >> 5)] >> (gcol & 31);
                    x.x = w & 1u ? x.x * inv_keep : 0.f; x.y = w & 2u ? x.y * inv_keep : 0.f;
                    x.z = w & 4u ? x.z * inv_keep : 0.f; x.w = w & 8u ? x.w * inv_keep : 0.f;
                } else if (MM == MM_HASH) {
                    const float4 mm = mess_multiplier4_pre(thr, inv_keep, seed, a.layer,
                                                           (uint64_t)((row + a.row_off) * a.d_out_full + gcol) >> 2);
                    x.x *= mm.x; x.y *= mm.y; x.z *= mm.z; x.w *= mm.w;
                } else if (MM == MM_MULT) {
                    const float4 mm = ld_f4(a.mess_mult + row * a.d_out_full + gcol);
                    x.x *= mm.x; x.y *= mm.y; x.z *= mm.z; x.w *= mm.w;
                }
                st_f4(dst, x);
            }
        }
        BWD_STAMP(0, it, 2);
    }
}

constexpr int F2_CONV_WARPS = 4;
constexpr int F2_TMA_WARP = FW_EPI_WARPS + 1;
constexpr int F2_THREADS = (FW_EPI_WARPS + 2 + F2_CONV_WARPS) * 32;
constexpr int F2_RAW_STAGES = 2;
constexpr int F2_A_SLOTS = 2;
constexpr int F2_RAW_BYTES = 2 * TC_A_BLOCK;

struct FwdTmaArgs {
    FwdTcArgs b;
    alignas(64) CUtensorMap tmS;
    alignas(64) CUtensorMap tmE;
};

struct Bars2 {
    uint64_t raw_full[F2_RAW_STAGES], raw_empty[F2_RAW_STAGES];
    uint64_t a_full[F2_A_SLOTS], a_empty[F2_A_SLOTS];
    uint64_t tmem_full[2], tmem_empty[2];
    uint64_t b_ready;
    uint32_t tmem_base;
};

template <int MM>
__global__ void __launch_bounds__(F2_THREADS, 1) dense_fwd_tma_kernel(const __grid_constant__ FwdTmaArgs p) {
    extern __shared__ uint8_t smem_raw[];
    const FwdTcArgs& a = p.b;
    const uint32_t base = (smem_u32(smem_raw) + 1023u) & ~1023u;
    uint8_t* smem = smem_raw + (base - smem_u32(smem_raw));
    const int d_in = a.d_in, d_out = a.d_out;
    const int KBH = d_in / 32, KB = 2 * KBH;
    const int b_block = d_out * 128;
    uint8_t* RAW = smem;
    uint8_t* AOP = RAW + F2_RAW_STAGES * F2_RAW_BYTES;
    uint8_t* B_hi = AOP + F2_A_SLOTS * 2 * TC_A_BLOCK;
    uint8_t* B_lo = B_hi + KB * b_block;
    float* bias_s = reinterpret_cast<float*>(B_lo + KB * b_block);
    float* stage = bias_s + 64;
    Bars2* bars = reinterpret_cast<Bars2*>(stage + FW_EPI_WARPS * 32 * 32);

    const int tid = threadIdx.x, warp = tid >> 5, lane = tid & 31;
    pdl_launch_dependents();
    if (tid == 0) {
        for (int i = 0; i < F2_RAW_STAGES; ++i) {
            mbar_init(&bars->raw_full[i], 1);
            mbar_init(&bars->raw_empty[i], F2_CONV_WARPS);
        }
        for (int i = 0; i < F2_A_SLOTS; ++i) {
            mbar_init(&bars->a_full[i], F2_CONV_WARPS);
            mbar_init(&bars->a_empty[i], 1);
        }
        for (int i = 0; i < 2; ++i) {
            mbar_init(&bars->tmem_full[i], 1);
            mbar_init(&bars->tmem_empty[i], FW_EPI_WARPS);
        }
        mbar_init(&bars->b_ready, FW_EPI_WARPS);
        fence_mbar_init();
        tma_prefetch_desc(&p.tmS);
        tma_prefetch_desc(&p.tmE);
    }
    if (warp == FW_MMA_WARP) tmem_alloc(&bars->tmem_base, 128);
    tc_fence_before_sync();
    __syncthreads();
    tc_fence_after_sync();
    const uint32_t tmem_base = bars->tmem_base;
    const int n_my = (a.n_tiles - (int)blockIdx.x + (int)gridDim.x - 1) / (int)gridDim.x;
    const int n_q = n_my * KBH;
    const bool dbg = g_bwd_dbg_on == 1 && blockIdx.x == 0 && (warp == 0 || warp >= FW_MMA_WARP);
    if (dbg && lane == 0 && warp == 0) g_bwd_dbg[0][7][7] = clock64();
    pdl_wait();
    if (dbg && lane == 0 && warp == 0) g_bwd_dbg[0][7][6] = clock64();

    if (warp < FW_EPI_WARPS) {
        constexpr int ET = FW_EPI_WARPS * 32;
        constexpr int WMAX = 64 * TC_MAX_KB * 8 / ET;
        float4 wv[WMAX];
        const int n_items = d_out * KB * 8;
// ... 109 lines not shown
                    split_tf32_trunc(x, hi, lo);
                    *reinterpret_cast<float4*>(hi_p + off) = hi;
                    *reinterpret_cast<float4*>(hi_p + TC_A_BLOCK + off) = lo;
                }
                fence_proxy_async_smem();
                __syncwarp();
                if (lane == 0) {
                    mbar_arrive(&bars->raw_empty[s]);
                    mbar_arrive(&bars->a_full[slot]);
                }
            }
            {
                const int slot = (j + 1) % F2_A_SLOTS;
                mbar_wait(&bars->a_empty[slot], (((j + 1) / F2_A_SLOTS) & 1) ^ 1);
                uint8_t* hi_p = AOP + slot * 2 * TC_A_BLOCK;
#pragma unroll
                for (int i = 0; i < NQ; ++i) {
                    const uint32_t off = (uint32_t)(i * LT + lt) * 16u;
                    const float4 x = make_float4(sv[i].x * ev[i].x, sv[i].y * ev[i].y, sv[i].z * ev[i].z, sv[i].w * ev[i].w);
                    float4 hi, lo;
                    split_tf32_trunc(x, hi, lo);
                    *reinterpret_cast<float4*>(hi_p + off) = hi;
                    *reinterpret_cast<float4*>(hi_p + TC_A_BLOCK + off) = lo;
                }
                fence_proxy_async_smem();
                __syncwarp();
                if (lane == 0) mbar_arrive(&bars->a_full[slot]);
                if (dbg && lane == 0 && warp == F2_TMA_WARP + 1 && q / KBH < 8) g_bwd_dbg[2][q / KBH][(q % KBH) * 3 + 2] = clock64();
            }
        }
    }

    tc_fence_before_sync();
    __syncthreads();
    if (dbg && lane == 0 && warp == 0) g_bwd_dbg[1][7][7] = clock64();
    if (warp == FW_MMA_WARP) {
        tc_fence_after_sync();
        tmem_dealloc(tmem_base, 128);
    }
}

}
namespace {

struct BwdTcArgs {
    const float* gE_next;
    const int32_t* slot;
    const float* gsum;
    int64_t ld_gsum;
    int col_off;
    const float* E_out;
    const float* S;
    const float* E;
    int64_t n_rows;
    int d_in, d_out;
    const float* W1;
    const float* W2;
    float slope;
    const float* mess_mult;
    const uint32_t* mess_bits;
    float mess_p;
    uint64_t seed;
    const uint64_t* seed_dev;
    int layer;
    float* gS;
    float* gEl;
    float* gM;
    float* gb1;
    float* gb2;
    int n_tiles;
    int64_t row_off;
    int d_out_full, out_off, d_in_full, in_off, accumulate, first_in;
    int pf;
};

struct BwdBars {
    uint64_t full_gm, empty_gm, tmem_full[2], tmem_empty[2];
    uint32_t tmem_base;
    float colsum[64];
};

__device__ __forceinline__ uint32_t es_off(int r, int c) { return (uint32_t)r * 256u + (uint32_t)((c ^ (r & 15)) << 4); }

template <int MM, bool PRE>
__global__ void __launch_bounds__(TC_THREADS, 1) dense_bwd_tc_kernel(BwdTcArgs a) {
    extern __shared__ uint8_t smem_raw[];
    const uint32_t base = (smem_u32(smem_raw) + 1023u) & ~1023u;
    uint8_t* smem = smem_raw + (base - smem_u32(smem_raw));
    constexpr int d_in = 64;
    const int d_out = a.d_out;
    const int KBo = d_out / 32;
    uint8_t* GM_hi = smem;
    uint8_t* GM_lo = GM_hi + KBo * TC_A_BLOCK;
    uint8_t* BT_hi = GM_lo + KBo * TC_A_BLOCK;
    uint8_t* BT_lo = BT_hi + KBo * TC_A_BLOCK;
    uint8_t* E_s = BT_lo + KBo * TC_A_BLOCK;
    uint8_t* S_s = E_s + TC_ROWS * 256;
    BwdBars* bars = reinterpret_cast<BwdBars*>(S_s + TC_ROWS * 256);

    const int tid = threadIdx.x, warp = tid >> 5, lane = tid & 31;
    pdl_launch_dependents();

    if (tid == 0) {
        mbar_init(&bars->full_gm, TC_LOAD_WARPS);
        mbar_init(&bars->empty_gm, 1);
        for (int i = 0; i < 2; ++i) {
            mbar_init(&bars->tmem_full[i], 1);
            mbar_init(&bars->tmem_empty[i], TC_EPI_WARPS);
        }
        fence_mbar_init();
    }
    if (warp == TC_EPI_WARPS) tmem_alloc(&bars->tmem_base, 256);
    if (tid < 64) bars->colsum[tid] = 0.f;
    auto prefetch_tile = [&](int tile, bool fwd_tensors, bool grad) {
        const int64_t row0 = (int64_t)tile * TC_ROWS;
        if (row0 >= a.n_rows) return;
        const int64_t nr = a.n_rows - row0 < TC_ROWS ? a.n_rows - row0 : TC_ROWS;
        if (fwd_tensors) {
            l2_prefetch_bulk(a.E_out + row0 * a.d_out_full, (uint32_t)(nr * a.d_out_full * 4));
            l2_prefetch_bulk(a.S + row0 * a.d_in_full, (uint32_t)(nr * a.d_in_full * 4));
            l2_prefetch_bulk(a.E + row0 * a.d_in_full, (uint32_t)(nr * a.d_in_full * 4));
        }
        if (grad && a.gE_next) l2_prefetch_bulk(a.gE_next + row0 * a.d_out_full, (uint32_t)(nr * a.d_out_full * 4));
    };
    if (a.pf > 0 && warp == TC_EPI_WARPS + 1 && lane == 0) {
        for (int i = 0; i < a.pf; ++i) {
            const int tile = blockIdx.x + i * gridDim.x;
            if (tile < a.n_tiles) prefetch_tile(tile, true, false);
        }
    }
    for (int i = tid; i < 128 * KBo * 8; i += TC_THREADS) {
        const int n = i & 127, c = (i >> 7) & 7, kb = i >> 10;
        const float* W = (n < d_in ? a.W1 : a.W2) + a.in_off + (n & 63);
        const int o0 = a.out_off + kb * 32 + c * 4;
        const int64_t ldw = a.d_in_full;
        float4 w = make_float4(W[(int64_t)o0 * ldw], W[(int64_t)(o0 + 1) * ldw], W[(int64_t)(o0 + 2) * ldw],
                               W[(int64_t)(o0 + 3) * ldw]);
        float4 hi, lo;
        split_tf32(w, hi, lo);
        const uint32_t off = kb * TC_A_BLOCK + sw128_offset(n, c);
        *reinterpret_cast<float4*>(BT_hi + off) = hi;
        *reinterpret_cast<float4*>(BT_lo + off) = lo;
    }
    fence_proxy_async_smem();
    tc_fence_before_sync();
    __syncthreads();
    tc_fence_after_sync();
    pdl_wait();
    const uint32_t tmem_base = bars->tmem_base;
    const int n_my = (a.n_tiles - (int)blockIdx.x + (int)gridDim.x - 1) / (int)gridDim.x;
    const bool dbg = g_bwd_dbg_on == 1 && blockIdx.x == 0 && (warp == 0 || warp == TC_EPI_WARPS || warp == TC_EPI_WARPS + 1);
    if (dbg && lane == 0 && warp == 0) g_bwd_dbg[0][7][7] = clock64();

    if (warp < TC_EPI_WARPS) {
        const int r = warp * 32 + lane;
        uint8_t* e_row = E_s + r * 256;
        uint8_t* s_row = S_s + r * 256;
        const int sw = r & 15;
        const int c = lane & 15, hsel = lane >> 4;
        const uint32_t e_s32 = smem_u32(E_s), s_s32 = smem_u32(S_s);
        auto fill = [&](int tile) {
            const int64_t row0 = (int64_t)tile * TC_ROWS;
#pragma unroll 4
            for (int i = 0; i < 16; ++i) {
                const int rl = warp * 32 + 2 * i + hsel;
                const int64_t row = row0 + rl;
                const bool ok = row < a.n_rows;
// ... 46 lines not shown
                const int rl = warp * 32 + 2 * i + hsel;
                const int64_t row = row0 + rl;
                const uint32_t off = es_off(rl, c);
                float4 x = *reinterpret_cast<const float4*>(E_s + off);
                float4 y = *reinterpret_cast<const float4*>(S_s + off);
                if (row < a.n_rows) {
                    float* ps = a.gS + row * a.d_in_full + a.in_off + c * 4;
                    float* pe = a.gEl + row * a.d_in_full + a.in_off + c * 4;
                    if (a.accumulate) {
                        const float4 x0 = ld_f4(ps), y0 = ld_f4(pe);
                        x.x += x0.x; x.y += x0.y; x.z += x0.z; x.w += x0.w;
                        y.x += y0.x; y.y += y0.y; y.z += y0.z; y.w += y0.w;
                    }
                    st_f4(ps, x);
                    st_f4(pe, y);
                }
            }
            __syncwarp();
            BWD_STAMP(0, it, 4);
            if (it + 1 < n_my) fill(tile + gridDim.x);
        }
    } else if (warp == TC_EPI_WARPS) {
        const uint32_t idesc1 = umma_idesc_tf32(TC_ROWS, 2 * d_in, 0, 0);
        if (a.pf > 0 && lane == 0)
            for (int i = 0; i < a.pf && i < n_my; ++i) prefetch_tile(blockIdx.x + i * gridDim.x, false, true);
        for (int it = 0; it < n_my; ++it) {
            const int buf = it & 1;
            BWD_STAMP(1, it, 0);
            if (a.pf > 0 && lane == 0 && it + a.pf < n_my) prefetch_tile(blockIdx.x + (it + a.pf) * gridDim.x, true, true);
            mbar_wait(&bars->full_gm, it & 1);
            BWD_STAMP(1, it, 1);
            mbar_wait(&bars->tmem_empty[buf], ((it >> 1) & 1) ^ 1);
            BWD_STAMP(1, it, 2);
            tc_fence_after_sync();
            if (lane == 0) {
                const uint32_t tmem_t = tmem_base + buf * 128;
                const uint32_t gm_hi = smem_u32(GM_hi), gm_lo = smem_u32(GM_lo);
                uint32_t acc1 = 0;
                for (int kb = 0; kb < KBo; ++kb) {
#pragma unroll
                    for (int k = 0; k < 4; ++k) {
                        const uint32_t off = kb * TC_A_BLOCK + k * 32;
                        const uint64_t dah = umma_desc_sw128(gm_hi + off, 16, 1024);
                        const uint64_t dal = umma_desc_sw128(gm_lo + off, 16, 1024);
                        const uint64_t dbh = umma_desc_sw128(smem_u32(BT_hi) + off, 16, 1024);
                        const uint64_t dbl = umma_desc_sw128(smem_u32(BT_lo) + off, 16, 1024);
                        umma_tf32(tmem_t, dah, dbh, idesc1, acc1);
                        umma_tf32(tmem_t, dal, dbh, idesc1, 1);
                        umma_tf32(tmem_t, dah, dbl, idesc1, 1);
                        acc1 = 1;
                    }
                }
                umma_commit(&bars->tmem_full[buf]);
                umma_commit(&bars->empty_gm);
            }
            __syncwarp();
            BWD_STAMP(1, it, 3);
        }
    } else {
        const int lw = warp - (TC_EPI_WARPS + 1);
        const int hl = lane & 15, hsel = lane >> 4;
        const int c0 = hl * 4;
        const bool col_ok = c0 < d_out;
        const uint64_t seed = MM == MM_HASH ? ngcf_seed(a.seed, a.seed_dev) : 0ull;
        const uint32_t thr = ngcf_threshold16(a.mess_p);
        const float inv_keep = 1.0f / (1.0f - a.mess_p);
        float4 colsum = make_float4(0.f, 0.f, 0.f, 0.f);
        constexpr int HP = TC_ROWS / (4 * TC_LOAD_WARPS);
        struct Half {
            float4 e[HP], gn[HP];
            int sl[HP];
        };
        auto issue = [&](Half& h, int tile, int half) {
            const int64_t row0 = (int64_t)tile * TC_ROWS;
#pragma unroll
            for (int j = 0; j < HP; ++j) {
                const int64_t row = row0 + 2 * (lw + TC_LOAD_WARPS * (half * HP + j)) + hsel;
                const bool ok = row < a.n_rows && col_ok;
                h.e[j] = h.gn[j] = make_float4(0.f, 0.f, 0.f, 0.f);
                h.sl[j] = -1;
                if (ok) {
                    h.e[j] = ld_stream_f4(a.E_out + row * a.d_out_full + a.out_off + c0);
                    if (a.gE_next) h.gn[j] = ld_stream_f4(a.gE_next + row * a.d_out_full + a.out_off + c0);
                    if (a.slot) h.sl[j] = a.slot[row];
                }
            }
        };
        auto compute = [&](Half& h, int tile, int half) {
            const int64_t row0 = (int64_t)tile * TC_ROWS;
            if (PRE) {
#pragma unroll
                for (int j = 0; j < HP; ++j) {
                    const int s = h.sl[j];
                    if (s >= 0) {
                        const float* gp = a.gsum + (int64_t)s * a.ld_gsum + a.col_off + a.out_off + c0;
                        h.gn[j].x += gp[0]; h.gn[j].y += gp[1]; h.gn[j].z += gp[2]; h.gn[j].w += gp[3];
                    }
                }
            } else {
#pragma unroll
                for (int j = 0; j < HP; ++j) {
                    const int s = h.sl[j];
                    if (__any_sync(FULL_MASK, s >= 0)) {
                        float4 gh = make_float4(0.f, 0.f, 0.f, 0.f);
                        if (s >= 0) {
                            const float* gp = a.gsum + (int64_t)s * a.ld_gsum + a.col_off + a.out_off + c0;
                            gh = make_float4(gp[0], gp[1], gp[2], gp[3]);
                        }
                        const float4 e = h.e[j];
                        float nrm2 = e.x * e.x + e.y * e.y + e.z * e.z + e.w * e.w;
                        float dot = e.x * gh.x + e.y * gh.y + e.z * gh.z + e.w * gh.w;
#pragma unroll
                        for (int o = 8; o > 0; o >>= 1) {
                            nrm2 += __shfl_xor_sync(FULL_MASK, nrm2, o);
                            dot += __shfl_xor_sync(FULL_MASK, dot, o);
                        }
                        if (s >= 0) {
                            const float rn = 1.0f / fmaxf(sqrtf(nrm2), 1e-12f);
                            const float hd = dot * rn;
                            h.gn[j].x += (gh.x - (e.x * rn) * hd) * rn;
                            h.gn[j].y += (gh.y - (e.y * rn) * hd) * rn;
                            h.gn[j].z += (gh.z - (e.z * rn) * hd) * rn;
                            h.gn[j].w += (gh.w - (e.w * rn) * hd) * rn;
                        }
                    }
                }
            }
#pragma unroll
            for (int j = 0; j < HP; ++j) {
                const int r = 2 * (lw + TC_LOAD_WARPS * (half * HP + j)) + hsel;
                const int64_t row = row0 + r;
                const bool in = row < a.n_rows && col_ok;
                const float4 e = h.e[j];
                float4 g = h.gn[j];
                float4 mult = make_float4(1.f, 1.f, 1.f, 1.f);
                if (MM == MM_MULT) {
                    if (in) mult = ld_f4(a.mess_mult + row * a.d_out_full + a.out_off + c0);
                } else if (MM == MM_BITS) {
                    uint32_t w = 0;
                    if (in) w = a.mess_bits[row * ((a.d_out_full + 31) >> 5) + ((a.out_off + c0) >> 5)] >> ((a.out_off + c0) & 31);
                    mult = make_float4(w & 1u ? inv_keep : 0.f, w & 2u ? inv_keep : 0.f, w & 4u ? inv_keep : 0.f,
                                       w & 8u ? inv_keep : 0.f);
                } else if (MM == MM_HASH) {
                    mult = mess_multiplier4_pre(thr, inv_keep, seed, a.layer,
                                                (uint64_t)((row + a.row_off) * a.d_out_full + a.out_off + c0) >> 2);
                }
                g.x *= mult.x * (e.x > 0.f ? 1.f : a.slope);
                g.y *= mult.y * (e.y > 0.f ? 1.f : a.slope);
                g.z *= mult.z * (e.z > 0.f ? 1.f : a.slope);
                g.w *= mult.w * (e.w > 0.f ? 1.f : a.slope);
                if (!in) g = make_float4(0.f, 0.f, 0.f, 0.f);
                if (in && a.first_in) st_f4(a.gM + row * a.d_out_full + a.out_off + c0, g);
                colsum.x += g.x; colsum.y += g.y; colsum.z += g.z; colsum.w += g.w;
                if (col_ok) {
                    float4 hi, lo;
                    split_tf32_trunc(g, hi, lo);
                    const uint32_t off = (hl >> 3) * TC_A_BLOCK + sw128_offset(r, hl & 7);
                    *reinterpret_cast<float4*>(GM_hi + off) = hi;
                    *reinterpret_cast<float4*>(GM_lo + off) = lo;
                }
            }
        };
        Half h0, h1;
        if (n_my > 0) issue(h0, blockIdx.x, 0);
        for (int it = 0; it < n_my; ++it) {
            const int tile = blockIdx.x + it * gridDim.x;
            BWD_STAMP(2, it, 0);
            issue(h1, tile, 1);
            BWD_STAMP(2, it, 1);
            mbar_wait(&bars->empty_gm, (it & 1) ^ 1);
            BWD_STAMP(2, it, 2);
            compute(h0, tile, 0);
            BWD_STAMP(3, it, 0);
            if (it + 1 < n_my) issue(h0, tile + gridDim.x, 0);
            BWD_STAMP(3, it, 1);
            compute(h1, tile, 1);
            BWD_STAMP(3, it, 2);
            fence_proxy_async_smem();
            BWD_STAMP(3, it, 3);
            __syncwarp();
            if (lane == 0) mbar_arrive(&bars->full_gm);
            BWD_STAMP(2, it, 3);
        }
        colsum.x += __shfl_xor_sync(FULL_MASK, colsum.x, 16);
        colsum.y += __shfl_xor_sync(FULL_MASK, colsum.y, 16);
        colsum.z += __shfl_xor_sync(FULL_MASK, colsum.z, 16);
        colsum.w += __shfl_xor_sync(FULL_MASK, colsum.w, 16);
        if (hsel == 0 && col_ok) {
            atomicAdd(&bars->colsum[c0 + 0], colsum.x);
            atomicAdd(&bars->colsum[c0 + 1], colsum.y);
            atomicAdd(&bars->colsum[c0 + 2], colsum.z);
            atomicAdd(&bars->colsum[c0 + 3], colsum.w);
        }
        asm volatile("bar.sync 1, %0;" ::"n"(TC_LOAD_WARPS * 32) : "memory");
        const int lt = tid - (TC_EPI_WARPS + 1) * 32;
        if (lt < d_out && a.first_in) {
            const float cs = bars->colsum[lt];
            atomicAdd(a.gb2 + a.out_off + lt, cs);
            atomicAdd(a.gb1 + a.out_off + lt, 2.0f * cs);
        }
    }

    tc_fence_before_sync();
    __syncthreads();
    if (dbg && lane == 0 && warp == 0) g_bwd_dbg[1][7][7] = clock64();
    if (warp == TC_EPI_WARPS) {
        tc_fence_after_sync();
        tmem_dealloc(tmem_base, 256);
    }
}

constexpr int WG_ROWS = 64;
constexpr int WG_BLOCK = WG_ROWS * 128;

struct WgradArgs {
    const float* S;
    const float* E;
    const float* gM;
    int64_t n_rows;
    int d_out;
    float* gW1;
    float* gW2;
    int n_chunks;
    int d_in_full, in_off, d_out_full, out_off;
    int pf;
};

struct WgBars {
// ... 88 lines not shown
        constexpr int LT = TC_LOAD_WARPS * 32;
        const int gq = d_out / 4;
        struct Half {
            float4 s[2], e[2], g[2];
        };
        const int total = 2 * n_my;
        auto issue = [&](Half& h, int i) {
            const int64_t row0 = (int64_t)(blockIdx.x + (i >> 1) * gridDim.x) * WG_ROWS;
#pragma unroll
            for (int q2 = 0; q2 < 2; ++q2) {
                const int idx = ((i & 1) * 2 + q2) * LT + lt, r = idx >> 4, c = idx & 15;
                const int64_t row = row0 + r;
                h.s[q2] = h.e[q2] = h.g[q2] = make_float4(0.f, 0.f, 0.f, 0.f);
                if (row < a.n_rows) {
                    h.s[q2] = ld_stream_f4(a.S + row * a.d_in_full + a.in_off + c * 4);
                    h.e[q2] = ld_stream_f4(a.E + row * a.d_in_full + a.in_off + c * 4);
                    if (c < gq) h.g[q2] = ld_stream_f4(a.gM + row * a.d_out_full + a.out_off + c * 4);
                }
            }
        };
        auto convert = [&](const Half& h, int i) {
            const int sgi = (i >> 1) & 1;
            uint8_t* x_hi = smem + sgi * stage_bytes;
            uint8_t* x_lo = x_hi + 4 * WG_BLOCK;
            uint8_t* g_hi = x_lo + 4 * WG_BLOCK;
            uint8_t* g_lo = g_hi + KBo * WG_BLOCK;
#pragma unroll
            for (int q2 = 0; q2 < 2; ++q2) {
                const int idx = ((i & 1) * 2 + q2) * LT + lt, r = idx >> 4, c = idx & 15;
                const uint32_t off = (c >> 3) * WG_BLOCK + sw128b32_offset(r, c & 7);
                const float4 sv = h.s[q2], ev = h.e[q2];
                const float4 x1 = make_float4(sv.x + ev.x, sv.y + ev.y, sv.z + ev.z, sv.w + ev.w);
                const float4 x2 = make_float4(sv.x * ev.x, sv.y * ev.y, sv.z * ev.z, sv.w * ev.w);
                float4 hi, lo;
                split_tf32(x1, hi, lo);
                *reinterpret_cast<float4*>(x_hi + off) = hi;
                *reinterpret_cast<float4*>(x_lo + off) = lo;
                split_tf32(x2, hi, lo);
                *reinterpret_cast<float4*>(x_hi + 2 * WG_BLOCK + off) = hi;
                *reinterpret_cast<float4*>(x_lo + 2 * WG_BLOCK + off) = lo;
                if (c < gq) {
                    split_tf32(h.g[q2], hi, lo);
                    *reinterpret_cast<float4*>(g_hi + off) = hi;
                    *reinterpret_cast<float4*>(g_lo + off) = lo;
                }
            }
        };
        Half h0, h1;
        if (total > 0) issue(h0, 0);
        for (int i = 0; i < total; i += 2) {
            const int it = i >> 1, sgi = it & 1;
            issue(h1, i + 1);
            mbar_wait(&bars->empty[sgi], ((it >> 1) & 1) ^ 1);
            convert(h0, i);
            if (i + 2 < total) issue(h0, i + 2);
            convert(h1, i + 1);
            fence_proxy_async_smem();
            __syncwarp();
            if (lane == 0) mbar_arrive(&bars->full[sgi]);
            BWD_STAMP(2, it, 0);
        }
    }

    tc_fence_before_sync();
    __syncthreads();
    if (dbg && lane == 0 && warp == 0) g_bwd_dbg[1][7][7] = clock64();
    if (warp == TC_EPI_WARPS) {
        tc_fence_after_sync();
        tmem_dealloc(tmem_d, 64);
    }
}

}

bool ngcf_dense_fwd_tc_eligible(int d_in, int d_out) {
    const bool in_ok = d_in == 32 || d_in == 64 || d_in == 128;
    const bool out_ok = (d_out >= 16 && d_out <= 64 && d_out % 16 == 0) || d_out == 128;
    return in_ok && out_ok;
}

int ngcf_dense_fwd_tc(const float* S, const float* E, int64_t n_rows, int d_in, int d_out, const float* wcat,
                      const float* bias_eff, float slope, const float* mess_mult, const uint32_t* mess_bits, float mess_p,
                      uint64_t seed, const uint64_t* seed_dev, int layer, int64_t row_offset, float* E_out,
                      cudaStream_t st) {
    static bool attr_set_dev[64] = {};
    int cur_dev = 0;
    NGCF_CUDA(cudaGetDevice(&cur_dev));
    bool& attr_set = attr_set_dev[cur_dev & 63];
    if (!attr_set) {
        NGCF_CUDA(cudaFuncSetAttribute(dense_fwd_tma_kernel<MM_NONE>, cudaFuncAttributeMaxDynamicSharedMemorySize, 227 * 1024));
        NGCF_CUDA(cudaFuncSetAttribute(dense_fwd_tma_kernel<MM_MULT>, cudaFuncAttributeMaxDynamicSharedMemorySize, 227 * 1024));
        NGCF_CUDA(cudaFuncSetAttribute(dense_fwd_tma_kernel<MM_BITS>, cudaFuncAttributeMaxDynamicSharedMemorySize, 227 * 1024));
        NGCF_CUDA(cudaFuncSetAttribute(dense_fwd_tma_kernel<MM_HASH>, cudaFuncAttributeMaxDynamicSharedMemorySize, 227 * 1024));
        attr_set = true;
    }
    const int bk = d_in > 64 ? 64 : d_in, bn = d_out > 64 ? 64 : d_out;
    const int KH = d_in / bk, NH = d_out / bn;
    const int n_tiles = (int)ceil_div64(n_rows, TC_ROWS);
    const int grid = (int)min((int64_t)n_tiles, (int64_t)ngcf_num_sms());
    const int KB = 2 * bk / 32;
    const size_t smem = 1024 + (size_t)F2_RAW_STAGES * F2_RAW_BYTES + (size_t)F2_A_SLOTS * 2 * TC_A_BLOCK +
                        (size_t)KB * 2 * bn * 128 + 64 * sizeof(float) + FW_EPI_WARPS * 32 * 32 * sizeof(float) +
                        sizeof(Bars2);
    FwdTmaArgs p{};
    int rc = ngcf_encode_tmap_2d(&p.tmS, S, (uint64_t)n_rows, (uint64_t)d_in, (uint64_t)d_in, 32, TC_ROWS,
                                 CU_TENSOR_MAP_SWIZZLE_128B);
    if (rc == 0)
        rc = ngcf_encode_tmap_2d(&p.tmE, E, (uint64_t)n_rows, (uint64_t)d_in, (uint64_t)d_in, 32, TC_ROWS,
                                 CU_TENSOR_MAP_SWIZZLE_128B);
    NGCF_REQUIRE(rc == 0, "dense_fwd: cuTensorMapEncodeTiled failed (%d)", rc);
    for (int nh = 0; nh < NH; ++nh)
        for (int kh = 0; kh < KH; ++kh) {
            FwdTcArgs a{S, E, n_rows, bk, bn, wcat, bias_eff, slope, mess_mult, mess_bits, mess_p, seed, seed_dev, layer,
                        E_out, n_tiles, row_offset};
            a.ld_in = d_in; a.in_off = kh * bk;
            a.w_row1 = kh * bk; a.w_row2 = d_in + kh * bk;
            a.out_off = nh * bn; a.d_out_full = d_out;
            a.mode = KH == 1 ? FW_SINGLE : (kh == 0 ? FW_PARTIAL : FW_FINAL);
            const int mm = a.mode == FW_PARTIAL ? MM_NONE : mess_mode(mess_mult, mess_bits, mess_p);
            p.b = a;
            switch (mm) {
                case MM_NONE: NGCF_CUDA(ngcf_launch_pdl(dense_fwd_tma_kernel<MM_NONE>, dim3(grid), dim3(F2_THREADS), smem, st, p)); break;
                case MM_MULT: NGCF_CUDA(ngcf_launch_pdl(dense_fwd_tma_kernel<MM_MULT>, dim3(grid), dim3(F2_THREADS), smem, st, p)); break;
                case MM_BITS: NGCF_CUDA(ngcf_launch_pdl(dense_fwd_tma_kernel<MM_BITS>, dim3(grid), dim3(F2_THREADS), smem, st, p)); break;
                default: NGCF_CUDA(ngcf_launch_pdl(dense_fwd_tma_kernel<MM_HASH>, dim3(grid), dim3(F2_THREADS), smem, st, p)); break;
            }
            NGCF_LAUNCH_OK("dense_fwd_tma_kernel");
        }
    return NGCF_OK;
}

static thread_local cudaStream_t g_wgrad_stream = nullptr;
static thread_local int g_wgrad_forked = 0;
extern "C" int ngcf_set_wgrad_stream(void* stream_or_null) {
    g_wgrad_stream = as_stream(stream_or_null);
    return NGCF_OK;
}
extern "C" int ngcf_wgrad_stream_forked(void) {
    const int v = g_wgrad_forked;
    g_wgrad_forked = 0;
    return v;
}

static int dense_prefetch_tiles() {
    static int v = -1;
    if (v < 0) {
        const char* e = getenv("NGCF_B200_PREFETCH");
        v = e ? atoi(e) : 0;
        if (v < 0) v = 0;
        if (v > 8) v = 8;
    }
    return v;
}

bool ngcf_dense_bwd_tc_eligible(int d_in, int d_out, int gh_normalized) {
    if (d_in == 64 && (d_out == 32 || d_out == 64)) return true;
    return (d_in == 64 || d_in == 128) && (d_out == 64 || d_out == 128) && (d_out <= 64 || gh_normalized);
}

int ngcf_dense_bwd_tc(const float* gE_next, const int32_t* slot, const float* gsum, int64_t ld_gsum, int col_off,
                      const float* E_out, const float* S, const float* E, int64_t n_rows, int d_in, int d_out,
                      const float* W1, const float* W2, float slope, const float* mess_mult, const uint32_t* mess_bits,
                      float mess_p, uint64_t seed, const uint64_t* seed_dev, int layer, int64_t row_offset,
                      int gh_normalized, float* gS, float* gEl, float* gW1, float* gb1, float* gW2, float* gb2,
                      float* gM_scratch, cudaStream_t st) {
    const int bn = d_out > 64 ? 64 : d_out;
    const int IH = d_in / 64, OH = d_out / bn;
    const int KBo = bn / 32;
    const int n_tiles = (int)ceil_div64(n_rows, TC_ROWS);
    const size_t smem = 1024 + (size_t)4 * KBo * TC_A_BLOCK + 2 * TC_ROWS * 256 + sizeof(BwdBars);
    const int grid = (int)min((int64_t)n_tiles, (int64_t)ngcf_num_sms());
    void (*kern)(BwdTcArgs) = nullptr;
    const bool pre = gh_normalized != 0;
    switch (mess_mode(mess_mult, mess_bits, mess_p)) {
        case MM_NONE: kern = pre ? dense_bwd_tc_kernel<MM_NONE, true> : dense_bwd_tc_kernel<MM_NONE, false>; break;
        case MM_MULT: kern = pre ? dense_bwd_tc_kernel<MM_MULT, true> : dense_bwd_tc_kernel<MM_MULT, false>; break;
        case MM_BITS: kern = pre ? dense_bwd_tc_kernel<MM_BITS, true> : dense_bwd_tc_kernel<MM_BITS, false>; break;
        default: kern = pre ? dense_bwd_tc_kernel<MM_HASH, true> : dense_bwd_tc_kernel<MM_HASH, false>; break;
    }
    NGCF_CUDA(cudaFuncSetAttribute(kern, cudaFuncAttributeMaxDynamicSharedMemorySize, 227 * 1024));
    NGCF_CUDA(cudaFuncSetAttribute(wgrad_tc_kernel, cudaFuncAttributeMaxDynamicSharedMemorySize, 227 * 1024));
    for (int ih = 0; ih < IH; ++ih)
        for (int oh = 0; oh < OH; ++oh) {
            BwdTcArgs a{gE_next, slot, gsum, ld_gsum, col_off, E_out, S, E, n_rows, 64, bn, W1, W2, slope, mess_mult,
                        mess_bits, mess_p, seed, seed_dev, layer, gS, gEl, gM_scratch, gb1, gb2, n_tiles, row_offset};
            a.d_out_full = d_out; a.out_off = oh * bn; a.d_in_full = d_in; a.in_off = ih * 64;
            a.accumulate = oh > 0; a.first_in = ih == 0;
            const bool contiguous = d_out == bn && d_in == 64 && ((uintptr_t)E_out & 15) == 0 && ((uintptr_t)S & 15) == 0 &&
                                    ((uintptr_t)E & 15) == 0 && ((uintptr_t)gE_next & 15) == 0 && bn % 4 == 0;
            a.pf = contiguous ? dense_prefetch_tiles() : 0;
            NGCF_CUDA(ngcf_launch_pdl(kern, dim3(grid), dim3(TC_THREADS), smem, st, a));
            NGCF_LAUNCH_OK("dense_bwd_tc_kernel");
        }
    const int n_chunks = (int)ceil_div64(n_rows, WG_ROWS);
    const size_t smem2 = 1024 + (size_t)2 * (8 + 2 * KBo) * WG_BLOCK + sizeof(WgBars);
    const int grid2 = (int)min((int64_t)n_chunks, (int64_t)ngcf_num_sms());
    cudaStream_t ws = st;
    if (g_wgrad_stream && g_wgrad_stream != st) {
        static cudaEvent_t ev[64] = {};
        int dev = 0;
        NGCF_CUDA(cudaGetDevice(&dev));
        if (!ev[dev & 63]) NGCF_CUDA(cudaEventCreateWithFlags(&ev[dev & 63], cudaEventDisableTiming));
        NGCF_CUDA(cudaEventRecord(ev[dev & 63], st));
        NGCF_CUDA(cudaStreamWaitEvent(g_wgrad_stream, ev[dev & 63], 0));
        ws = g_wgrad_stream;
        g_wgrad_forked = 1;
    }
    for (int ih = 0; ih < IH; ++ih)
        for (int oh = 0; oh < OH; ++oh) {
            WgradArgs w{S, E, gM_scratch, n_rows, bn, gW1, gW2, n_chunks, d_in, ih * 64, d_out, oh * bn, 0};
            w.pf = (d_out == bn && d_in == 64 && ((uintptr_t)S & 15) == 0 && ((uintptr_t)E & 15) == 0 &&
                    ((uintptr_t)gM_scratch & 15) == 0 && bn % 4 == 0) ? dense_prefetch_tiles() : 0;
            NGCF_CUDA(ngcf_launch_pdl(wgrad_tc_kernel, dim3(grid2), dim3(TC_THREADS), smem2, ws, w));
            NGCF_LAUNCH_OK("wgrad_tc_kernel");
        }
    return NGCF_OK;
}

extern "C" int ngcf_debug_bwd_timeline(int enable, long long* out_host ) {
    NGCF_CUDA(cudaMemcpyToSymbol(g_bwd_dbg_on, &enable, sizeof(int)));
    if (out_host) NGCF_CUDA(cudaMemcpyFromSymbol(out_host, g_bwd_dbg, sizeof(long long) * 4 * 8 * 8));
    return NGCF_OK;
}
```

### seoul_tourism_recommendation_ngcf_b200/csrc/spmm.cu

```cuda
#include "spmm_core.cuh"

namespace {

using namespace ngcf;

#ifndef NGCF_SPMM_THREADS
#define NGCF_SPMM_THREADS 64
#endif
constexpr int SP_THREADS = NGCF_SPMM_THREADS;
constexpr int SP_WARPS = SP_THREADS / 32;

struct TileSide {
    const TileInfo* tiles;
    const int32_t* rowptr;
    const int2* ent;
    const int32_t* row_key;
    const uint8_t* bits;
    const int2* cent;
    const int32_t* ccnt;
    float* Y;
    int64_t ldy;
};

struct SpmmArgs {
// ... 369 lines not shown
    const int2* ent;
    const int32_t* row_key;
    float p;
    uint64_t seed;
    const uint64_t* seed_dev;
    int n_layers;
    uint32_t row_off;
    uint8_t* out_f;
    uint8_t* out_t;
};

constexpr int BITS_THREADS = 256;
constexpr int BITS_TILES = 8;
__global__ void __launch_bounds__(BITS_THREADS) dropout_bits_kernel(BitsArgs a, int n_tiles) {
    __shared__ int rp_s[BITS_TILES * SP_TILE_ROWS + 1];
    const int tid = threadIdx.x;
    const int t0 = blockIdx.x * BITS_TILES, t1 = min(t0 + BITS_TILES, n_tiles) - 1;
    const int4 first = *reinterpret_cast<const int4*>(a.tiles + t0);
    const int4 last = *reinterpret_cast<const int4*>(a.tiles + t1);
    const int r0 = first.x, nr = last.y - first.x, e0 = first.z, cnt = last.w - first.z;
    for (int i = tid; i <= nr; i += BITS_THREADS) rp_s[i] = a.rowptr[r0 + i] - e0;
    __syncthreads();
    const uint64_t seed = ngcf_seed(a.seed, a.seed_dev);
    for (int i = tid; i < cnt; i += BITS_THREADS) {
        const uint32_t c = ent_col(ld_stream_i2(a.ent + e0 + i).x);
        int lo = 0, hi = nr - 1;
        while (lo < hi) {
            const int mid = (lo + hi + 1) >> 1;
            if (rp_s[mid] <= i) lo = mid; else hi = mid - 1;
        }
        const uint32_t r = (uint32_t)(a.row_key ? a.row_key[r0 + lo] : r0 + lo) + a.row_off;
        if (a.out_f) a.out_f[e0 + i] = (uint8_t)node_keep_bits(a.p, seed, a.n_layers, r, c);
        if (a.out_t) a.out_t[e0 + i] = (uint8_t)node_keep_bits(a.p, seed, a.n_layers, c, r);
    }
}

struct KeyArgs {
    const TileInfo* tiles;
    const int32_t* rowptr;
    const int2* ent;
    const int32_t* row_key;
    uint32_t row_off;
    uint32_t* key_l;
    uint32_t* key_t;
};
__global__ void __launch_bounds__(BITS_THREADS) entry_keys_kernel(KeyArgs a, int n_tiles) {
    __shared__ int rp_s[BITS_TILES * SP_TILE_ROWS + 1];
    const int tid = threadIdx.x;
    const int t0 = blockIdx.x * BITS_TILES, t1 = min(t0 + BITS_TILES, n_tiles) - 1;
    const int4 first = *reinterpret_cast<const int4*>(a.tiles + t0);
    const int4 last = *reinterpret_cast<const int4*>(a.tiles + t1);
    const int r0 = first.x, nr = last.y - first.x, e0 = first.z, cnt = last.w - first.z;
    for (int i = tid; i <= nr; i += BITS_THREADS) rp_s[i] = a.rowptr[r0 + i] - e0;
    __syncthreads();
    for (int i = tid; i < cnt; i += BITS_THREADS) {
        const uint32_t c = ent_col(ld_stream_i2(a.ent + e0 + i).x);
        int lo = 0, hi = nr - 1;
        while (lo < hi) {
            const int mid = (lo + hi + 1) >> 1;
            if (rp_s[mid] <= i) lo = mid; else hi = mid - 1;
        }
        const uint32_t r = (uint32_t)(a.row_key ? a.row_key[r0 + lo] : r0 + lo) + a.row_off;
        a.key_l[e0 + i] = ngcf_node_key(r, c);
        a.key_t[e0 + i] = ngcf_node_key(c, r);
    }
}

constexpr int WS_PER = SP_TILE_ENT / 32;
static_assert(WS_PER * 32 == SP_TILE_ENT, "tile entries must be a multiple of the warp size");

struct CompactArgs {
    const TileInfo* tiles;
    const int2* ent;
    const int32_t* row_key;
    float p;
    uint64_t seed;
    const uint64_t* seed_dev;
    int n_layers;
    uint32_t row_off;
    const uint32_t* key_l;
    const uint32_t* key_t;
    int2* out_ent[2][NGCF_MAX_LAYERS];
    int32_t* out_cnt[2][NGCF_MAX_LAYERS];
};

constexpr int CW_WARPS = 4;
__global__ void __launch_bounds__(CW_WARPS * 32) compact_kernel(CompactArgs a, int n_tiles) {
    const int lane = threadIdx.x & 31;
    const int t = blockIdx.x * CW_WARPS + (threadIdx.x >> 5);
    if (t >= n_tiles) return;
    const int4 raw = *reinterpret_cast<const int4*>(a.tiles + t);
    const TileInfo ti{raw.x, raw.y, raw.z, raw.w};
    const int cnt = ti.e1 - ti.e0;
    const int K = a.n_layers;
    const bool want_l = a.out_ent[0][0] != nullptr, want_t = a.out_ent[1][0] != nullptr;
    int2 e[WS_PER];
    uint32_t kl[WS_PER], kt[WS_PER];
#pragma unroll
    for (int q = 0; q < WS_PER; ++q) {
        const int p = q * 32 + lane;
        e[q] = make_int2(0, 0);
        kl[q] = kt[q] = 0;
        if (p < cnt) {
            e[q] = ld_stream_i2(a.ent + ti.e0 + p);
            if (a.key_l) {
                if (want_l) kl[q] = a.key_l[ti.e0 + p];
                if (want_t) kt[q] = a.key_t[ti.e0 + p];
            }
        }
    }
    const uint64_t seed = ngcf_seed(a.seed, a.seed_dev);
    const uint32_t thr = ngcf_threshold16(a.p);
    uint32_t keep[WS_PER];
#pragma unroll
    for (int q = 0; q < WS_PER; ++q) {
        const int p = q * 32 + lane;
        keep[q] = 0;
        if (p < cnt) {
            if (!a.key_l) {
                const int lr = ent_lrow(e[q].x);
                const uint32_t r = (uint32_t)(a.row_key ? a.row_key[ti.r0 + lr] : ti.r0 + lr) + a.row_off;
                kl[q] = ngcf_node_key(r, ent_col(e[q].x));
                kt[q] = ngcf_node_key(ent_col(e[q].x), r);
            }
            if (want_l) keep[q] = node_keep_bits_key(thr, seed, K, kl[q]);
            if (want_t) keep[q] |= node_keep_bits_key(thr, seed, K, kt[q]) << K;
        }
    }
    const uint32_t below = (1u << lane) - 1u;
    for (int c = 0; c < 2 * K; ++c) {
        const int dir = c >= K, layer = dir ? c - K : c;
        int2* out = a.out_ent[dir][layer];
        if (!out) continue;
        int base = 0;
#pragma unroll
        for (int q = 0; q < WS_PER; ++q) {
            const bool k = (keep[q] >> c) & 1u;
            const uint32_t m = __ballot_sync(FULL_MASK, k);
            if (k) out[ti.e0 + base + __popc(m & below)] = e[q];
            base += __popc(m);
        }
        if (lane == 0) a.out_cnt[dir][layer][t] = base;
    }
}

template <int G>
int launch(const SpmmArgs& a, int n_ctas, bool stream, cudaStream_t st) {
    if (n_ctas <= 0) return NGCF_OK;
    if constexpr (G > 0) {
        if (stream) {
            NGCF_CUDA(ngcf_launch_pdl(spmm_stream_kernel<G>, dim3((unsigned)n_ctas), dim3(SP_THREADS), 0, st, a));
            NGCF_LAUNCH_OK("spmm_stream_kernel");
            if (a.n_hub > 0) {
                NGCF_CUDA(ngcf_launch_pdl(hub_finish_kernel<G>, dim3((unsigned)a.n_hub), dim3(HF_THREADS), 0, st, a));
                NGCF_LAUNCH_OK("hub_finish_kernel");
            }
            return NGCF_OK;
        }
    }
    NGCF_CUDA(ngcf_launch_pdl(spmm_tile_kernel<G>, dim3((unsigned)n_ctas), dim3(SP_THREADS), 0, st, a));
    NGCF_LAUNCH_OK("spmm_tile_kernel");
    return NGCF_OK;
}

int launch_any(const SpmmArgs& a, int n_ctas, bool vec, bool stream, cudaStream_t st) {
    if (!vec) return launch<0>(a, n_ctas, false, st);
    const int d4 = a.d / 4;
    if (d4 <= 1) return launch<1>(a, n_ctas, stream, st);
    if (d4 <= 2) return launch<2>(a, n_ctas, stream, st);
    if (d4 <= 4) return launch<4>(a, n_ctas, stream, st);
    if (d4 <= 8) return launch<8>(a, n_ctas, stream, st);
    if (d4 <= 16) return launch<16>(a, n_ctas, stream, st);
    return launch<32>(a, n_ctas, stream, st);
}

unsigned long long* g_spmm_dbg = nullptr;
unsigned long long* g_spmm_dbg_compact = nullptr;

inline bool aligned16(const void* p) { return (reinterpret_cast<uintptr_t>(p) & 15) == 0; }

}

extern "C" int ngcf_spmm_split_threshold(void) { return ngcf::SPLIT; }
extern "C" int ngcf_spmm_tile_rows(void) { return SP_TILE_ROWS; }
extern "C" int ngcf_spmm_tile_entries(void) { return SP_TILE_ENT; }

int ngcf_check_csr(const ngcf_csr* g, const char* who) {
    NGCF_REQUIRE(g != nullptr, "%s: csr descriptor is null", who);
    NGCF_REQUIRE(g->n_rows >= 0 && g->n_rows < ((int64_t)1 << 31), "%s: n_rows %lld", who, (long long)g->n_rows);
    NGCF_REQUIRE(g->n_rows == 0 || (g->rowptr && g->ent), "%s: rowptr/ent missing", who);
    NGCF_REQUIRE(g->n_hub >= 0 && g->n_chunks >= 0, "%s: negative hub counts", who);
    NGCF_REQUIRE(g->n_hub == 0 || (g->hub_of_row && g->hub_chunk_ptr && g->chunk_ptr && g->hub_ent && g->chunk_row),
                 "%s: hub arrays missing", who);
    return NGCF_OK;
}

extern "C" int ngcf_spmm(const ngcf_csr* g, const float* X, int64_t ldx, int d, const float* addend, int64_t ld_add,
                         const int32_t* slot, const float* gsum, int64_t ld_gsum, float* hub_partial, float drop_p,
                         uint64_t seed, const uint64_t* seed_dev, int layer, int transposed, int64_t row_offset,
                         const uint8_t* keep_bits, const int32_t* c_ent, const int32_t* c_cnt, float* Y, int64_t ldy,
                         void* stream) {
    int rc = ngcf_check_csr(g, "spmm");
    if (rc != NGCF_OK) return rc;
    NGCF_REQUIRE(X && Y, "spmm: null pointer");
    NGCF_REQUIRE(d > 0 && d <= NGCF_MAX_WIDTH, "spmm: width %d not in [1,%d]", d, NGCF_MAX_WIDTH);
    NGCF_REQUIRE(ldx >= d && ldy >= d && ldx < ((int64_t)1 << 31), "spmm: bad leading dimension");
    NGCF_REQUIRE(drop_p >= 0.f && drop_p < 1.f, "spmm: drop_p %f not in [0,1)", drop_p);
    NGCF_REQUIRE(layer >= 0 && layer < NGCF_MAX_LAYERS, "spmm: layer %d", layer);
    NGCF_REQUIRE(row_offset >= 0 && row_offset < ((int64_t)1 << 31), "spmm: row_offset %lld", (long long)row_offset);
    NGCF_REQUIRE(!slot || gsum, "spmm: slot given without gsum");
    NGCF_REQUIRE((c_ent == nullptr) == (c_cnt == nullptr), "spmm: c_ent and c_cnt go together");
    NGCF_REQUIRE(g->n_hub == 0 || hub_partial, "spmm: hub_partial scratch missing");
    NGCF_REQUIRE(g->n_tiles == 0 || g->tiles, "spmm: SpMM tiles missing");
    NGCF_REQUIRE(g->n_chunk_tiles == 0 || g->chunk_tiles, "spmm: chunk tiles missing");
    if (g->n_rows == 0) return NGCF_OK;
    cudaStream_t st = as_stream(stream);
    const bool vec = (d % 4 == 0) && (ldx % 4 == 0) && (ldy % 4 == 0) && aligned16(X) && aligned16(Y) &&
                     (!addend || (aligned16(addend) && ld_add % 4 == 0)) &&
                     (!slot || (aligned16(gsum) && ld_gsum % 4 == 0)) && (g->n_hub == 0 || aligned16(hub_partial));
    const bool hubs = g->n_hub > 0 && g->n_chunks > 0;
    const bool stream_k = vec && (!hubs || (g->tile_hubmask && g->hub_rows));
    NGCF_REQUIRE(stream_k || !c_ent, "spmm: compacted survivor lists need the streaming kernel (width %% 4 == 0)");
    NGCF_REQUIRE(stream_k || !hubs || g->hub_done, "spmm: hub_done counters missing");
    SpmmArgs a{};
    a.rows = TileSide{reinterpret_cast<const TileInfo*>(g->tiles), g->rowptr, reinterpret_cast<const int2*>(g->ent), nullptr,
                      keep_bits, reinterpret_cast<const int2*>(c_ent), c_cnt, Y, ldy};
    a.n_chunk_tiles = hubs ? g->n_chunk_tiles : 0;
    if (hubs)
        a.chunks = TileSide{reinterpret_cast<const TileInfo*>(g->chunk_tiles), g->chunk_ptr,
                            reinterpret_cast<const int2*>(g->hub_ent), g->chunk_row,
                            keep_bits ? keep_bits + g->rowptr_nnz : nullptr,
                            c_ent ? reinterpret_cast<const int2*>(c_ent) + g->rowptr_nnz : nullptr,
                            c_cnt ? c_cnt + g->n_tiles : nullptr, hub_partial, d};
    a.X = X; a.ldx = (uint32_t)ldx; a.d = d;
    a.addend = addend; a.ld_add = ld_add; a.slot = slot; a.gsum = gsum; a.ld_gsum = ld_gsum;
    a.drop_p = drop_p; a.seed = seed; a.seed_dev = seed_dev; a.layer = layer; a.transposed = transposed;
    a.row_off = (uint32_t)row_offset;
    a.dbg = g_spmm_dbg;
    a.hub_of_row = hubs ? g->hub_of_row : nullptr;
    a.hub_chunk_ptr = g->hub_chunk_ptr;
    a.hub_done = g->hub_done;
    a.Yrows = Y;
    a.ld_yrows = ldy;
    a.tile_hubmask = hubs ? g->tile_hubmask : nullptr;
    a.n_row_tiles = g->n_tiles;
    a.hub_rows = g->hub_rows;
    a.n_hub = hubs ? g->n_hub : 0;
    if (stream_k && addend) {
        if (addend != Y)
            NGCF_CUDA(cudaMemcpy2DAsync(Y, (size_t)ldy * sizeof(float), addend, (size_t)ld_add * sizeof(float),
                                        (size_t)d * sizeof(float), (size_t)g->n_rows, cudaMemcpyDeviceToDevice, st));
        a.add_mode = 1;
        a.addend = nullptr;
    }
    return launch_any(a, a.n_chunk_tiles + g->n_tiles, vec, stream_k, st);
}

extern "C" int ngcf_node_dropout_bits(const ngcf_csr* g, float drop_p, uint64_t seed, const uint64_t* seed_dev,
                                      int n_layers, int64_t row_offset, uint8_t* bits_as_L, uint8_t* bits_as_Lt,
                                      void* stream) {
    int rc = ngcf_check_csr(g, "node_dropout_bits");
    if (rc != NGCF_OK) return rc;
    NGCF_REQUIRE(drop_p > 0.f && drop_p < 1.f, "node_dropout_bits: drop_p %f not in (0,1)", drop_p);
    NGCF_REQUIRE(n_layers >= 1 && n_layers <= NGCF_MAX_LAYERS, "node_dropout_bits: n_layers %d", n_layers);
    NGCF_REQUIRE(bits_as_L || bits_as_Lt, "node_dropout_bits: no output");
    NGCF_REQUIRE(row_offset >= 0 && row_offset < ((int64_t)1 << 31), "node_dropout_bits: row_offset");
    cudaStream_t st = as_stream(stream);
    if (g->n_tiles > 0) {
        BitsArgs a{reinterpret_cast<const TileInfo*>(g->tiles), g->rowptr, reinterpret_cast<const int2*>(g->ent), nullptr,
                   drop_p, seed, seed_dev, n_layers, (uint32_t)row_offset, bits_as_L, bits_as_Lt};
        dropout_bits_kernel<<<(unsigned)ceil_div64(g->n_tiles, BITS_TILES), BITS_THREADS, 0, st>>>(a, g->n_tiles);
        NGCF_LAUNCH_OK("dropout_bits_kernel(rows)");
    }
    if (g->n_hub > 0 && g->n_chunk_tiles > 0) {
        BitsArgs a{reinterpret_cast<const TileInfo*>(g->chunk_tiles), g->chunk_ptr,
                   reinterpret_cast<const int2*>(g->hub_ent), g->chunk_row, drop_p, seed, seed_dev, n_layers,
                   (uint32_t)row_offset, bits_as_L ? bits_as_L + g->rowptr_nnz : nullptr,
                   bits_as_Lt ? bits_as_Lt + g->rowptr_nnz : nullptr};
        dropout_bits_kernel<<<(unsigned)ceil_div64(g->n_chunk_tiles, BITS_TILES), BITS_THREADS, 0, st>>>(a, g->n_chunk_tiles);
        NGCF_LAUNCH_OK("dropout_bits_kernel(hub chunks)");
    }
    return NGCF_OK;
}

extern "C" int ngcf_node_dropout_compact(const ngcf_csr* g, float drop_p, uint64_t seed, const uint64_t* seed_dev,
                                         int n_layers, int64_t row_offset, int32_t* const* ent_as_L_host,
                                         int32_t* const* cnt_as_L_host, int32_t* const* ent_as_Lt_host,
                                         int32_t* const* cnt_as_Lt_host, void* stream) {
    int rc = ngcf_check_csr(g, "node_dropout_compact");
    if (rc != NGCF_OK) return rc;
    NGCF_REQUIRE(drop_p > 0.f && drop_p < 1.f, "node_dropout_compact: drop_p %f not in (0,1)", drop_p);
    NGCF_REQUIRE(n_layers >= 1 && n_layers <= NGCF_MAX_LAYERS, "node_dropout_compact: n_layers %d", n_layers);
    NGCF_REQUIRE((ent_as_L_host && cnt_as_L_host) || (ent_as_Lt_host && cnt_as_Lt_host), "node_dropout_compact: no output");
    NGCF_REQUIRE((ent_as_L_host == nullptr) == (cnt_as_L_host == nullptr) &&
                 (ent_as_Lt_host == nullptr) == (cnt_as_Lt_host == nullptr), "node_dropout_compact: ent/cnt go together");
    NGCF_REQUIRE(row_offset >= 0 && row_offset < ((int64_t)1 << 31), "node_dropout_compact: row_offset");
    for (int k = 0; k < n_layers; ++k) {
        NGCF_REQUIRE(!ent_as_L_host || (ent_as_L_host[k] && cnt_as_L_host[k]), "node_dropout_compact: null L output %d", k);
        NGCF_REQUIRE(!ent_as_Lt_host || (ent_as_Lt_host[k] && cnt_as_Lt_host[k]), "node_dropout_compact: null L^T output %d", k);
    }
    cudaStream_t st = as_stream(stream);
    for (int pass = 0; pass < 2; ++pass) {
        const int n_tiles = pass ? g->n_chunk_tiles : g->n_tiles;
        if (n_tiles <= 0 || (pass && g->n_hub == 0)) continue;
        CompactArgs a{};
        a.tiles = reinterpret_cast<const TileInfo*>(pass ? g->chunk_tiles : g->tiles);
        a.ent = reinterpret_cast<const int2*>(pass ? g->hub_ent : g->ent);
        a.row_key = pass ? g->chunk_row : nullptr;
        a.p = drop_p; a.seed = seed; a.seed_dev = seed_dev; a.n_layers = n_layers; a.row_off = (uint32_t)row_offset;
        const size_t e_off = pass ? (size_t)g->rowptr_nnz : 0, t_off = pass ? (size_t)g->n_tiles : 0;
        if (g->key_l && g->key_t && g->key_row_offset == row_offset) {
            a.key_l = g->key_l + e_off;
            a.key_t = g->key_t + e_off;
        }
        for (int k = 0; k < n_layers; ++k) {
            if (ent_as_L_host) {
                a.out_ent[0][k] = reinterpret_cast<int2*>(ent_as_L_host[k]) + e_off;
                a.out_cnt[0][k] = cnt_as_L_host[k] + t_off;
            }
            if (ent_as_Lt_host) {
                a.out_ent[1][k] = reinterpret_cast<int2*>(ent_as_Lt_host[k]) + e_off;
                a.out_cnt[1][k] = cnt_as_Lt_host[k] + t_off;
            }
        }
        compact_kernel<<<(unsigned)ceil_div64(n_tiles, CW_WARPS), CW_WARPS * 32, 0, st>>>(a, n_tiles);
        NGCF_LAUNCH_OK(pass ? "compact_kernel(hub chunks)" : "compact_kernel(rows)");
    }
    return NGCF_OK;
}

extern "C" int ngcf_debug_spmm_timeline(unsigned long long* dev_buf_or_null) {
    g_spmm_dbg = dev_buf_or_null;
    return NGCF_OK;
}
extern "C" int ngcf_debug_compact_timeline(unsigned long long* dev_buf_or_null) {
    g_spmm_dbg_compact = dev_buf_or_null;
    return NGCF_OK;
}

extern "C" int ngcf_entry_keys(const ngcf_csr* g, int64_t row_offset, uint32_t* key_l, uint32_t* key_t, void* stream) {
    int rc = ngcf_check_csr(g, "entry_keys");
    if (rc != NGCF_OK) return rc;
    NGCF_REQUIRE(key_l && key_t, "entry_keys: null output");
    NGCF_REQUIRE(row_offset >= 0 && row_offset < ((int64_t)1 << 31), "entry_keys: row_offset");
    cudaStream_t st = as_stream(stream);
    if (g->n_tiles > 0) {
        KeyArgs a{reinterpret_cast<const TileInfo*>(g->tiles), g->rowptr, reinterpret_cast<const int2*>(g->ent), nullptr,
                  (uint32_t)row_offset, key_l, key_t};
        entry_keys_kernel<<<(unsigned)ceil_div64(g->n_tiles, BITS_TILES), BITS_THREADS, 0, st>>>(a, g->n_tiles);
        NGCF_LAUNCH_OK("entry_keys_kernel(rows)");
    }
    if (g->n_hub > 0 && g->n_chunk_tiles > 0) {
        KeyArgs a{reinterpret_cast<const TileInfo*>(g->chunk_tiles), g->chunk_ptr, reinterpret_cast<const int2*>(g->hub_ent),
                  g->chunk_row, (uint32_t)row_offset, key_l + g->rowptr_nnz, key_t + g->rowptr_nnz};
        entry_keys_kernel<<<(unsigned)ceil_div64(g->n_chunk_tiles, BITS_TILES), BITS_THREADS, 0, st>>>(a, g->n_chunk_tiles);
        NGCF_LAUNCH_OK("entry_keys_kernel(hub chunks)");
    }
    return NGCF_OK;
}
```

### seoul_tourism_recommendation_ngcf_b200/graph.py

```python
from __future__ import annotations

import torch

FIELDS = ("u_id", "age", "sex", "month", "day", "dow", "pos_item", "neg_item")


class GraphedStep:

    def __init__(self, model, criterion, batch_size: int, node_flag: bool = True, warmup: int = 1, optimizer=None):
        dev = model.user_embedding.weight.device
        if dev.type != "cuda":
            raise RuntimeError("GraphedStep needs the model on a CUDA device")
        self.model, self.criterion, self.node_flag, self.warmup = model, criterion, bool(node_flag), int(warmup)
        self.B = int(batch_size)
        self.optimizer = optimizer
        self.static_idx = torch.zeros(len(FIELDS), self.B, dtype=torch.int64, device=dev)
        self.stages = [torch.zeros(len(FIELDS), self.B, dtype=torch.int64).pin_memory() for _ in range(3)]
        self.stage_events = [None] * len(self.stages)
        self._stage_i = 0
        self.seed_dev = torch.zeros(1, dtype=torch.int64, device=dev)
        self.graphs = {}
        self.launches_per_step = None

    def _run(self, year, with_optimizer: bool = True):
        m = self.model
        f = {k: self.static_idx[i] for i, k in enumerate(FIELDS)}
        u, p, n = m(year=year, u_id=f["u_id"], age=f["age"], sex=f["sex"], month=f["month"], day=f["day"], dow=f["dow"],
                    pos_item=f["pos_item"], neg_item=f["neg_item"], node_flag=self.node_flag)
        loss = self.criterion(u, p, n)
        loss.backward()
        if self.optimizer is not None and with_optimizer:
            self.optimizer.step()
        self.seed_dev.add_(0x9E3779B97F4A7C15 & (2 ** 62 - 1))
        return loss

    def _capture(self, year):
        from . import _lib
        m = self.model
        m._seed_dev = self.seed_dev
        s = torch.cuda.Stream()
        s.wait_stream(torch.cuda.current_stream())
        with torch.cuda.stream(s):
            users_before = m.user_embedding.weight.detach().clone()
            for _ in range(self.warmup):
                m.zero_grad(set_to_none=True)
                self._run(year, with_optimizer=False)
            if self.optimizer is not None:
                self.optimizer.prepare([p for p in m.parameters() if p.grad is not None])
            m.user_embedding.weight.data.copy_(users_before)
        torch.cuda.current_stream().wait_stream(s)
        m.zero_grad(set_to_none=True)
        g = torch.cuda.CUDAGraph()
        n0 = _lib.load().ngcf_launch_count()
        with torch.cuda.graph(g):
            loss = self._run(year)
        self.launches_per_step = int(_lib.load().ngcf_launch_count() - n0)
        grads = {k: p.grad for k, p in m.named_parameters() if p.grad is not None}
        return g, loss, grads, m._last

    def __call__(self, batch):
        year = batch["year"]
        if year.device.type != "cpu":
            raise ValueError("GraphedStep: pass `year` as a host tensor (it is only used to pick lap_list[year % 18])")
        on_host = [batch[k].device.type == "cpu" for k in FIELDS]
        stage = None
        if any(on_host):
            j = self._stage_i
            self._stage_i = (j + 1) % len(self.stages)
            if self.stage_events[j] is not None:
                self.stage_events[j].synchronize()
            stage = self.stages[j]
        for i, k in enumerate(FIELDS):
            t = batch[k]
            if t.numel() != self.B:
                raise ValueError(f"GraphedStep was built for batches of {self.B} rows, got {t.numel()} for {k}")
            if on_host[i]:
                stage[i].copy_(t)
        if all(on_host):
            self.static_idx.copy_(stage, non_blocking=True)
        else:
            for i, k in enumerate(FIELDS):
                self.static_idx[i].copy_(stage[i] if on_host[i] else batch[k], non_blocking=True)
        if stage is not None:
            if self.stage_events[j] is None:
                self.stage_events[j] = torch.cuda.Event()
            self.stage_events[j].record()
        key = int(year.min()) % 18
        entry = self.graphs.get(key)
        if entry is None:
            entry = self.graphs[key] = self._capture(year)
        g, loss, grads, last = entry
        g.replay()
        self.model._last, self.model._all_E = last, None
        if self.optimizer is not None:
            from . import _lib
            _lib.bump_param_epoch()
            last.fresh_key = None
        else:
            self.model._mix_count += 1
            last.fresh_key = self.model._fresh_key()
        for k, p in self.model.named_parameters():
            if k in grads and p.grad is not grads[k]:
                p.grad = grads[k]
        return loss
```

### seoul_tourism_recommendation_ngcf_b200/plan.py

```python
from __future__ import annotations

import ctypes as C

import numpy as np
import torch

from . import _lib


def _stream() -> int:
    return _lib.current_stream()


def greedy_tiles(rowptr: np.ndarray, max_rows: int, max_ent: int) -> np.ndarray:
    rowptr = np.asarray(rowptr, dtype=np.int64)
    n = rowptr.size - 1
    out = []
    r = 0
    while r < n:
        k = int(np.searchsorted(rowptr, rowptr[r] + max_ent, side="right")) - 1
        r1 = max(r + 1, min(r + max_rows, k, n))
        out.append((r, r1, rowptr[r], rowptr[r1]))
        r = r1
    return np.asarray(out, dtype=np.int32).reshape(-1, 4)
# ... 14 lines not shown
        _lib.check(lib.ngcf_build_tiles(rowptr.data_ptr(), n, int(max_rows), int(max_ent), nxt.data_ptr(),
                                        tiles.data_ptr(), capacity, count.data_ptr(), _stream()), "build_tiles")
        if int(count) <= capacity:
            return tiles[:int(count)].contiguous()
    raise RuntimeError("tile builder overflow")


DEVICE_TILE_ROWS = 1 << 18


class CsrSide:

    def __init__(self, rowptr: torch.Tensor, colidx: torch.Tensor, perm, n_rows: int, nnz: int, vals=None):
        lib = _lib.load()
        dev = rowptr.device
        self.n_rows, self.nnz = int(n_rows), int(nnz)
        split = lib.ngcf_spmm_split_threshold()
        i32 = dict(dtype=torch.int32, device=dev)
        deg = (rowptr[1:] - rowptr[:-1]).to(torch.int64)
        hub_mask = deg > split
        hub = torch.nonzero(hub_mask).flatten()
        self.n_hub = int(hub.numel())
        colidx = colidx[:self.nnz]
        perm = perm[:self.nnz] if perm is not None else None
        self.vals = vals
        if self.n_hub:
            row_of_entry = torch.repeat_interleave(torch.arange(self.n_rows, device=dev), deg)
            ent_is_hub = hub_mask[row_of_entry]
            order = torch.cat([torch.nonzero(~ent_is_hub).flatten(), torch.nonzero(ent_is_hub).flatten()])
            self.colidx = colidx[order].contiguous()
            self.perm = perm[order].contiguous() if perm is not None else None
            if vals is not None:
                self.vals = vals[order].contiguous()
            del row_of_entry, ent_is_hub, order
            hdeg = deg[hub]
            self.nnz_hub = int(hdeg.sum())
            short_deg = torch.where(hub_mask, torch.zeros_like(deg), deg)
            nch = (hdeg + split - 1) // split
            cptr = torch.zeros(self.n_hub + 1, dtype=torch.int64, device=dev)
            cptr[1:] = torch.cumsum(nch, 0)
            self.n_chunks = int(cptr[-1])
            hub_base = torch.zeros(self.n_hub + 1, dtype=torch.int64, device=dev)
            hub_base[1:] = torch.cumsum(hdeg, 0)
            owner = torch.repeat_interleave(torch.arange(self.n_hub, device=dev), nch)
            local = torch.arange(self.n_chunks, device=dev) - cptr[owner]
            chunk_ptr = torch.empty(self.n_chunks + 1, dtype=torch.int64, device=dev)
            chunk_ptr[:-1] = hub_base[owner] + local * split
            chunk_ptr[-1] = self.nnz_hub
            self.hub_of_row = torch.full((self.n_rows,), -1, **i32)
            self.hub_of_row[hub] = torch.arange(self.n_hub, **i32)
            self.hub_chunk_ptr = cptr.to(torch.int32)
            self.chunk_ptr = chunk_ptr.to(torch.int32)
            self.chunk_row = hub[owner].to(torch.int32)
            self.hub_rows = hub.to(torch.int32).contiguous()
            self.hub_done = torch.zeros(self.n_hub, **i32)
        else:
            self.colidx, self.perm = colidx.contiguous(), (perm.contiguous() if perm is not None else None)
            self.nnz_hub, self.n_chunks = 0, 0
            short_deg = deg
            self.hub_of_row = self.hub_chunk_ptr = self.chunk_ptr = self.chunk_row = self.hub_rows = self.hub_done = None
        self.nnz_short = self.nnz - self.nnz_hub
        self.rowptr = torch.zeros(self.n_rows + 1, **i32)
        self.rowptr[1:] = torch.cumsum(short_deg, 0).to(torch.int32)
        tr, te = lib.ngcf_spmm_tile_rows(), lib.ngcf_spmm_tile_entries()
        if self.n_rows > DEVICE_TILE_ROWS:
            self.tiles = device_tiles(self.rowptr, tr, te)
            self.chunk_tiles = device_tiles(self.chunk_ptr, tr, te) if self.n_chunks else None
        else:
            self.tiles = torch.from_numpy(greedy_tiles(self.rowptr.cpu().numpy(), tr, te)).to(dev)
            self.chunk_tiles = torch.from_numpy(greedy_tiles(self.chunk_ptr.cpu().numpy(), tr, te)).to(dev) \
                if self.n_chunks else None
        self._pack_local_rows()
        if self.n_hub and self.tiles.shape[0]:
            hm = torch.zeros(self.n_rows + 32, dtype=torch.int64, device=dev)
            hm[:self.n_rows] = hub_mask.to(torch.int64)
            t0 = self.tiles[:, 0].to(torch.int64)
            nr = (self.tiles[:, 1] - self.tiles[:, 0]).to(torch.int64)
            bits = torch.zeros(self.tiles.shape[0], dtype=torch.int64, device=dev)
            for i in range(int(lib.ngcf_spmm_tile_rows())):
                bits |= (hm[t0 + i] * (i < nr).to(torch.int64)) << i
            self.tile_hubmask = (bits & 0xFFFFFFFF).to(torch.int32)
        else:
            self.tile_hubmask = None
        self.ent = None
        self.key_l = self.key_t = None
        self.key_row_offset = 0
        self._partial = {}
        self._struct_cache = {}

    LR_SHIFT = 27

    def _pack_local_rows(self):
        dev = self.rowptr.device
        if self.nnz_short:
            pos = torch.arange(self.nnz_short, device=dev)
            row = torch.searchsorted(self.rowptr.to(torch.int64), pos, right=True) - 1
            t0 = self.tiles[:, 0].to(torch.int64).contiguous()
            lr = row - t0[torch.searchsorted(t0, row, right=True) - 1]
            self.colidx[:self.nnz_short] |= (lr << self.LR_SHIFT).to(torch.int32)
        if self.n_chunks:
            pos = torch.arange(self.nnz_hub, device=dev)
            chunk = torch.searchsorted(self.chunk_ptr.to(torch.int64), pos, right=True) - 1
            t0 = self.chunk_tiles[:, 0].to(torch.int64).contiguous()
            lr = chunk - t0[torch.searchsorted(t0, chunk, right=True) - 1]
            self.colidx[self.nnz_short:self.nnz] |= (lr << self.LR_SHIFT).to(torch.int32)

    def descriptor(self, ent: torch.Tensor | None = None) -> "_lib.NgcfCsr":
        ent = self.ent if ent is None else ent
        key = ent.data_ptr()
        s = self._struct_cache.get(key)
        if s is None:
            if len(self._struct_cache) > 64:
                self._struct_cache.clear()
            s = _lib.NgcfCsr()
            s.n_rows = self.n_rows
            s.rowptr = self.rowptr.data_ptr()
            s.ent = ent.data_ptr()
            s.tiles = self.tiles.data_ptr()
            s.hub_of_row = _lib.ptr(self.hub_of_row)
            s.hub_chunk_ptr = _lib.ptr(self.hub_chunk_ptr)
            s.chunk_ptr = _lib.ptr(self.chunk_ptr)
            s.hub_ent = ent.data_ptr() + 8 * self.nnz_short
            s.chunk_row = _lib.ptr(self.chunk_row)
            s.chunk_tiles = _lib.ptr(self.chunk_tiles)
            s.hub_rows = _lib.ptr(self.hub_rows)
            s.hub_done = _lib.ptr(self.hub_done)
            s.key_l = _lib.ptr(self.key_l)
            s.key_t = _lib.ptr(self.key_t)
            s.key_row_offset = self.key_row_offset
            s.n_tiles = int(self.tiles.shape[0])
            s.n_hub = self.n_hub
            s.n_chunks = self.n_chunks
            s.n_chunk_tiles = int(self.chunk_tiles.shape[0]) if self.chunk_tiles is not None else 0
            s.rowptr_nnz = self.nnz_short
            s.tile_hubmask = _lib.ptr(self.tile_hubmask)
            self._struct_cache[key] = s
        return s

    def ensure_keys(self, row_offset: int = 0):
        if self.key_l is None or self.key_row_offset != row_offset:
            lib = _lib.load()
            dev = self.rowptr.device
            kl = torch.empty(max(self.nnz, 1), dtype=torch.int32, device=dev)
            kt = torch.empty(max(self.nnz, 1), dtype=torch.int32, device=dev)
            _lib.check(lib.ngcf_entry_keys(C.byref(self.descriptor(None)), int(row_offset), kl.data_ptr(), kt.data_ptr(),
                                           _stream()), "entry_keys")
            self.key_l, self.key_t, self.key_row_offset = kl, kt, int(row_offset)
            self._struct_cache.clear()

    def hub_partial(self, d: int):
        if not self.n_hub:
            return None
        buf = self._partial.get(d)
        if buf is None:
            buf = torch.empty(self.n_chunks * d, dtype=torch.float32, device=self.rowptr.device)
            self._partial[d] = buf
        return buf


class LaplacianPlan:

    def __init__(self, L, device, shard=None):
        from .plgraph import CsrLaplacian
        if isinstance(L, CsrLaplacian):
            self._init_from_csr(L, torch.device(device), shard)
            return
# ... 22 lines not shown
        else:
            from .sharded import shard_coo
            if shard.N != self.N:
                raise ValueError("shard descriptor and Laplacian disagree on N")
            n_rows, n_cols = shard.rows, shard.N_pad
            Ld = torch.sparse_coo_tensor(idx, self.coo_val, L.shape, is_coalesced=False, check_invariants=False)
            parts = list(shard_coo(Ld, shard))
        sides = []
        for row, col, pos in parts:
            nnz = int(row.numel())
            row, col = row.contiguous(), col.contiguous()
            need = C.c_size_t(0)
            _lib.check(lib.ngcf_coo_to_csr_workspace(nnz, n_rows, C.byref(need)), "coo_to_csr_workspace")
            ws = torch.empty(need.value, dtype=torch.uint8, device=device)
            rowptr = torch.empty(n_rows + 1, dtype=torch.int32, device=device)
            colidx = torch.empty(max(nnz, 1), dtype=torch.int32, device=device)
            perm = torch.empty(max(nnz, 1), dtype=torch.int32, device=device)
            _lib.check(lib.ngcf_coo_to_csr(row.data_ptr(), col.data_ptr(), nnz, n_rows, n_cols, 0,
                                           rowptr.data_ptr(), colidx.data_ptr(), perm.data_ptr(), ws.data_ptr(),
                                           need.value, _stream()), "coo_to_csr")
            perm = pos[perm[:nnz].to(torch.int64)].to(torch.int32) if nnz else perm
            side = CsrSide(rowptr, colidx, perm, n_rows, nnz)
            side.ent = self.entries(side, None)
            sides.append(side)
            torch.cuda.current_stream().synchronize()
            del ws
        self.fwd, self.bwd = sides
        self.symmetric = bool(self.fwd.nnz == self.bwd.nnz and torch.equal(self.fwd.rowptr, self.bwd.rowptr) and
                              torch.equal(self.fwd.ent, self.bwd.ent))

    def _init_from_csr(self, L, device, shard):
        if device.type != "cuda":
            raise RuntimeError("LaplacianPlan needs a CUDA device: the NGCF B200 path has no CPU fallback")
        self.src, self.N, self.shard = L, int(L.shape[0]), shard
        n_cols = shard.N_pad if shard is not None else self.N
        if n_cols >= (1 << CsrSide.LR_SHIFT):
            raise ValueError(f"graphs of up to {1 << CsrSide.LR_SHIFT} nodes are supported (27-bit column ids)")
        if shard is not None and (L.row0 != shard.r0 or L.n_rows != shard.rows):
            raise ValueError("the CSR shard does not cover this rank's row block")
        if shard is None and L.n_rows != self.N:
            raise ValueError("an unsharded plan needs all rows of the Laplacian")
        self.nnz = L.nnz
        self.coo_val = L.vals
        side = CsrSide(L.rowptr.to(device), L.colidx.to(device), None, L.n_rows, L.nnz, vals=L.vals.to(device))
        side.ent = self.entries(side, None)
        side.vals = None
        torch.cuda.current_stream().synchronize()
        self.fwd = self.bwd = side
        self.symmetric = True

    def side(self, transposed: bool, masked: bool) -> CsrSide:
        if transposed and not (self.symmetric and not masked):
            return self.bwd
        return self.fwd

    def entries(self, side: CsrSide, keep_mask):
        lib = _lib.load()
        if side.perm is None:
            if keep_mask is not None:
                raise ValueError("explicit COO-order edge masks need a reference-format (COO) Laplacian")
            out = torch.zeros(side.nnz + 2, 2, dtype=torch.int32, device=side.colidx.device)
            out[:side.nnz, 0] = side.colidx
            out[:side.nnz, 1] = side.vals.view(torch.int32)
            return out
        out = torch.zeros(side.nnz + 2, 2, dtype=torch.int32, device=self.coo_val.device)
        _lib.check(lib.ngcf_edge_entries(side.colidx.data_ptr(), self.coo_val.data_ptr(), side.perm.data_ptr(),
                                         _lib.ptr(keep_mask), out.data_ptr(), side.nnz, _stream()), "edge_entries")
        return out


def node_dropout_bits(side: CsrSide, drop_p: float, seed: int, seed_dev, n_layers: int, row_offset: int = 0,
                      as_L: bool = True, as_Lt: bool = False):
    lib = _lib.load()
    dev = side.rowptr.device
    bl = torch.empty(side.nnz, dtype=torch.uint8, device=dev) if as_L else None
    bt = torch.empty(side.nnz, dtype=torch.uint8, device=dev) if as_Lt else None
    _lib.check(lib.ngcf_node_dropout_bits(C.byref(side.descriptor(None)), float(drop_p), int(seed) & (2 ** 64 - 1),
                                          _lib.ptr(seed_dev), int(n_layers), int(row_offset), _lib.ptr(bl), _lib.ptr(bt),
                                          _stream()), "node_dropout_bits")
    return bl, bt


def node_dropout_compact(side: CsrSide, drop_p: float, seed: int, seed_dev, n_layers: int, row_offset: int = 0,
                         as_L: bool = True, as_Lt: bool = False, static_keys: bool = True):
    lib = _lib.load()
    dev = side.rowptr.device
    if static_keys:
        side.ensure_keys(row_offset)
    elif side.key_l is not None:
        side.key_l = side.key_t = None
        side._struct_cache.clear()
    n_t = int(side.tiles.shape[0]) + (int(side.chunk_tiles.shape[0]) if side.chunk_tiles is not None else 0)

    def alloc():
        return [(torch.empty(side.nnz + 2, 2, dtype=torch.int32, device=dev),
                 torch.empty(max(n_t, 1), dtype=torch.int32, device=dev)) for _ in range(n_layers)]

    cl = alloc() if as_L else None
    ct = alloc() if as_Lt else None

    def arrs(c):
        if c is None:
            return None, None
        return _lib.ptr_array([e for e, _ in c]), _lib.ptr_array([t for _, t in c])

    el, tl = arrs(cl)
    et, tt = arrs(ct)
    _lib.check(lib.ngcf_node_dropout_compact(C.byref(side.descriptor(None)), float(drop_p), int(seed) & (2 ** 64 - 1),
                                             _lib.ptr(seed_dev), int(n_layers), int(row_offset), el, tl, et, tt,
                                             _stream()), "node_dropout_compact")
    return cl, ct


def spmm(side: CsrSide, ent, X, d: int, out=None, addend=None, slot=None, gsum=None, drop_p: float = 0.0,
         seed: int = 0, seed_dev=None, layer: int = 0, transposed: bool = False, row_offset: int = 0, keep_bits=None,
         compact=None):
    lib = _lib.load()
    if out is None:
        if addend is not None and d % 4 == 0 and addend.shape[0] == side.n_rows and addend.stride(0) % 4 == 0:
            out = addend
        else:
            out = torch.empty(side.n_rows, d, dtype=torch.float32, device=X.device)
    _lib.check(lib.ngcf_spmm(C.byref(side.descriptor(ent)), X.data_ptr(), X.stride(0), d,
                             _lib.ptr(addend), addend.stride(0) if addend is not None else 0,
                             _lib.ptr(slot), _lib.ptr(gsum), gsum.stride(0) if gsum is not None else 0,
                             _lib.ptr(side.hub_partial(d)),
                             float(drop_p), int(seed) & (2 ** 64 - 1), _lib.ptr(seed_dev), int(layer), int(transposed),
                             int(row_offset), _lib.ptr(keep_bits),
                             _lib.ptr(compact[0]) if compact is not None else None,
                             _lib.ptr(compact[1]) if compact is not None else None,
                             out.data_ptr(), out.stride(0), _stream()), "spmm")
    return out
```

Baseline: 0.4922.

## Compute last NGCF layer only for batch rows, defer full layer lazily

In the last propagation layer, the forward pass computes the sparse aggregation and dense transform only for the rows in the current BPR batch (users, positive and negative items), not for every node. The backward pass uses row-restricted dense gradients, and the transposed compact dropout entries are filtered by a column slot map. The full last-layer output is rebuilt lazily through a list wrapper only when something reads it, such as the embedding export. This drops most of the last layer's SpMM and GEMM work, at the cost of considerable complexity and several new kernels, and relies on the deferred completion reproducing identical dropout seeds.

Result: faster. 0.4500, median of 6 (-8.6%).

```diff
diff --git a/include/ngcf_b200.h b/include/ngcf_b200.h
--- a/include/ngcf_b200.h
+++ b/include/ngcf_b200.h
@@ -82,6 +82,26 @@
 
 int ngcf_entry_keys(const ngcf_csr* csr_host, int64_t row_offset, uint32_t* key_l, uint32_t* key_t, void* stream);
 
+int ngcf_batch_rows(const int64_t* const* rows_host, const int64_t* offsets_host, const int64_t* batch_host, int n_sets,
+                    int32_t* slot, int32_t* row_ids, const uint64_t* seed_dev, uint64_t* seed_used, void* stream);
+int ngcf_node_dropout_compact_cols(const ngcf_csr* csr_host, float drop_p, uint64_t seed, const uint64_t* seed_dev,
+                                   int n_layers, int64_t row_offset,
+                                   int32_t* const* ent_as_L_host, int32_t* const* cnt_as_L_host,
+                                   int32_t* const* ent_as_Lt_host, int32_t* const* cnt_as_Lt_host,
+                                   const int32_t* col_slot, int slot_layer, void* stream);
+int ngcf_spmm_rows(const ngcf_csr* csr_host, const int32_t* row_ids, const int32_t* slot, int64_t n, const float* X,
+                   int d, const int32_t* c_ent, const int32_t* c_cnt, const int32_t* tile_of_row,
+                   const int32_t* tile_of_chunk, float* hub_partial, float* Y, float* Xrows, void* stream);
+int ngcf_dense_rows_eligible(int d_in, int d_out);
+int ngcf_dense_fwd_rows(const float* S, const float* E, int64_t n, int d_in, int d_out, const float* wcat,
+                        const float* bias_eff, float slope, float mess_p, uint64_t seed, const uint64_t* seed_dev,
+                        int layer, const int32_t* row_ids, float* E_out, float* E_rows, void* stream);
+int ngcf_dense_bwd_rows(const int32_t* row_ids, const float* gsum, int64_t ld_gsum, int col_off, const float* E_out,
+                        const float* S, const float* E, int64_t n, int d_in, int d_out, const float* W1,
+                        const float* W2, float slope, float mess_p, uint64_t seed, const uint64_t* seed_dev, int layer,
+                        float* gS, float* gEl, float* gW1, float* gb1, float* gW2, float* gb2, float* gM_scratch,
+                        void* stream);
+
 int ngcf_plgraph_entries(int64_t n_user, int64_t n_item, int64_t n_edges, double alpha, uint64_t seed,
                          int64_t row0, int64_t n_rows, unsigned long long* total_dev,
                          unsigned long long* keys_or_null, int64_t capacity, void* stream);
diff --git a/seoul_tourism_recommendation_ngcf_b200/NGCF.py b/seoul_tourism_recommendation_ngcf_b200/NGCF.py
--- a/seoul_tourism_recommendation_ngcf_b200/NGCF.py
+++ b/seoul_tourism_recommendation_ngcf_b200/NGCF.py
@@ -2,6 +2,7 @@
 
 import ctypes as C
 import os
+import weakref
 
 import numpy as np
 import torch
@@ -22,7 +23,32 @@
 
 class _Ctx:
     __slots__ = ("plan", "E", "S", "dims", "vals_f", "vals_b", "mess_mult", "mess_p", "seed", "seed_dev", "masked", "drop_p", "bits_f", "bits_b", "comp_f", "comp_b", "mess_bits",
-                 "rows", "offsets", "W1", "W2", "fresh_key", "node_mode", "last_partial", "fm_stream")
+                 "rows", "offsets", "W1", "W2", "fresh_key", "node_mode", "last_partial", "fm_stream", "lastc",
+                 "__weakref__")
+
+
+class _LastRows:
+    __slots__ = ("row_ids", "seed_used", "S", "X", "E", "E_rows", "wcat", "bias")
+
+
+class _PartialLast(list):
+
+    def __init__(self, items):
+        super().__init__(items)
+        self._pending = None
+
+    def complete(self):
+        if self._pending is not None:
+            mod, st = self._pending[0](), self._pending[1]()
+            if mod is None or st is None:
+                raise RuntimeError("NGCF (B200): the step that produced this layer list no longer exists")
+            mod._complete_last(st)
+
+    def __getitem__(self, i):
+        n = len(self)
+        if self._pending is not None and (isinstance(i, slice) or (n and int(i) % n == n - 1)):
+            self.complete()
+        return super().__getitem__(i)
 
 
 def _capturing() -> bool:
@@ -55,12 +81,25 @@
         st.bits_f = st.bits_b = st.comp_f = st.comp_b = None
         st.node_mode = mod._node_mode
         st.last_partial = None
+        st.lastc = None
+        n_batch = sum(r.numel() for r in st.rows[:n_sets])
+        rows_h, offs_h = _lib.ptr_array(st.rows[:n_sets]), _lib.i64_array(st.offsets[:n_sets])
+        batch_h = _lib.i64_array([r.numel() for r in st.rows[:n_sets]])
+        rows_only = mod._last_rows_only(st)
+        if rows_only:
+            slot = mod._slot_map(N, dev)
+            lc = st.lastc = _LastRows()
+            lc.row_ids = torch.empty(n_batch, dtype=torch.int32, device=dev)
+            lc.seed_used = torch.zeros(1, dtype=torch.int64, device=dev)
+            _lib.check(lib.ngcf_batch_rows(rows_h, offs_h, batch_h, n_sets, slot.data_ptr(), lc.row_ids.data_ptr(),
+                                           _lib.ptr(st.seed_dev), lc.seed_used.data_ptr(), _stream()), "batch_rows")
         if st.drop_p > 0:
             shared = st.plan.side(True, False) is side
             node_mode = mod._node_mode if all(d % 4 == 0 for d in st.dims) or mod._node_mode == "inkernel" else "bits"
             st.node_mode = node_mode
             if node_mode == "compact":
-                st.comp_f, ct = node_dropout_compact(side, st.drop_p, st.seed, st.seed_dev, K, r0, as_L=True, as_Lt=shared)
+                st.comp_f, ct = node_dropout_compact(side, st.drop_p, st.seed, st.seed_dev, K, r0, as_L=True, as_Lt=shared,
+                                                     col_slot=slot if rows_only and shared else None, slot_layer=K - 1)
                 if shared:
                     st.comp_b = ct
             elif node_mode == "bits":
@@ -84,6 +123,28 @@
         _join_feature_mix(st)
         for k in range(K):
             d_in, d_out = st.dims[k], st.dims[k + 1]
+            if rows_only and k == K - 1:
+                lc.S = torch.empty(n_batch, d_in, dtype=torch.float32, device=dev)
+                lc.X = torch.empty(n_batch, d_in, dtype=torch.float32, device=dev)
+                lc.E = torch.empty(n_batch, d_out, dtype=torch.float32, device=dev)
+                lc.wcat, lc.bias = wcats[k], biases[k]
+                _lib.check(lib.ngcf_spmm_rows(C.byref(side.descriptor(None)), lc.row_ids.data_ptr(), slot.data_ptr(),
+                                              n_batch, st.E[k].data_ptr(), d_in, st.comp_f[k][0].data_ptr(),
+                                              st.comp_f[k][1].data_ptr(), side.tile_of_row.data_ptr(),
+                                              _lib.ptr(side.tile_of_chunk), _lib.ptr(side.hub_partial(d_in)),
+                                              lc.S.data_ptr(), lc.X.data_ptr(), _stream()), "spmm_rows")
+                _lib.check(lib.ngcf_rowgrad_reset(rows_h, offs_h, batch_h, n_sets, slot.data_ptr(), _stream()),
+                           "rowgrad_reset")
+                En = torch.empty(N, d_out, dtype=torch.float32, device=dev)
+                _lib.check(lib.ngcf_dense_fwd_rows(lc.S.data_ptr(), lc.X.data_ptr(), n_batch, d_in, d_out,
+                                                   lc.wcat.data_ptr(), lc.bias.data_ptr(), LEAKY_SLOPE,
+                                                   float(st.mess_p[k]), st.seed, _lib.ptr(st.seed_dev), k,
+                                                   lc.row_ids.data_ptr(), lc.E.data_ptr(), En.data_ptr(), _stream()),
+                           "dense_fwd_rows")
+                lc.E_rows = En
+                st.S.append(None)
+                st.E.append(En)
+                continue
             vals = st.vals_f[k] if st.vals_f is not None else None
             S = spmm(side, vals, st.E[k], d_in, drop_p=st.drop_p, seed=st.seed, seed_dev=st.seed_dev, layer=k,
                      row_offset=r0, keep_bits=st.bits_f,
@@ -123,6 +184,9 @@
                                                _lib.i64_array(st.offsets[:n_sets]),
                                                _lib.i64_array([r.numel() for r in st.rows[:n_sets]]), _lib.ptr_array(outs),
                                                n_sets, D, _stream()), "gather_concat_sets")
+        if rows_only:
+            st.E, st.S = _PartialLast(st.E), _PartialLast(st.S)
+            mod._rearm_last(st)
         ctx.st, ctx.mod, ctx.n_sets = st, mod, n_sets
         return tuple(outs)
 
@@ -166,8 +230,10 @@
             gb1.append(flat[o:o + dims[k + 1]]); o += dims[k + 1]
             gb2.append(flat[o:o + dims[k + 1]]); o += dims[k + 1]
         side = st.plan.side(True, st.vals_b is not None)
+        lc = st.lastc
         if st.drop_p > 0 and st.node_mode == "compact" and st.comp_b is None:
-            _, st.comp_b = node_dropout_compact(side, st.drop_p, st.seed, st.seed_dev, K, r0, as_L=False, as_Lt=True)
+            _, st.comp_b = node_dropout_compact(side, st.drop_p, st.seed, st.seed_dev, K, r0, as_L=False, as_Lt=True,
+                                                col_slot=slot if lc is not None else None, slot_layer=K - 1)
         if st.drop_p > 0 and st.node_mode == "bits" and st.bits_b is None:
             _, st.bits_b = node_dropout_bits(side, st.drop_p, st.seed, st.seed_dev, K, r0, as_L=False, as_Lt=True)
         gE_next = None
@@ -184,6 +250,28 @@
         for k in range(K - 1, -1, -1):
             d_in, d_out = dims[k], dims[k + 1]
             col_off -= d_out
+            if lc is not None and k == K - 1:
+                n_batch = lc.row_ids.numel()
+                gS = torch.empty(n_batch, d_in, dtype=torch.float32, device=dev)
+                gEl = torch.empty(n_batch, d_in, dtype=torch.float32, device=dev)
+                gM = gM_scratch if not overlap and gM_scratch.numel() >= n_batch * d_out else \
+                    torch.empty(n_batch, d_out, dtype=torch.float32, device=dev)
+                if overlap:
+                    gM_keep.append(gM)
+                _lib.check(lib.ngcf_dense_bwd_rows(lc.row_ids.data_ptr(), gsum.data_ptr(), D, col_off, lc.E.data_ptr(),
+                                                   lc.S.data_ptr(), lc.X.data_ptr(), n_batch, d_in, d_out,
+                                                   st.W1[k].data_ptr(), st.W2[k].data_ptr(), LEAKY_SLOPE,
+                                                   float(st.mess_p[k]), st.seed, _lib.ptr(st.seed_dev), k,
+                                                   gS.data_ptr(), gEl.data_ptr(), gW1[k].data_ptr(), gb1[k].data_ptr(),
+                                                   gW2[k].data_ptr(), gb2[k].data_ptr(), gM.data_ptr(), _stream()),
+                           "dense_bwd_rows")
+                if k == 0:
+                    gEl.add_(gsum[:, :d_in])
+                gE_next = spmm(side, None, gS, d_in, slot=slot_loc, gsum=gEl, drop_p=st.drop_p, seed=st.seed,
+                               seed_dev=st.seed_dev, layer=k, transposed=True, compact=st.comp_b[k])
+                if mod._trace is not None:
+                    mod._trace.append(dict(k=k, gS=gS.clone(), gEl=gEl.clone(), gE=gE_next.clone()))
+                continue
             peer = sh is not None and mod._xchg is not None and d_in % 4 == 0
             if peer:
                 gS_all = mod._xchg.matrix(("gS", d_in), N_all, d_in)
@@ -409,6 +497,44 @@
             out.append(torch.from_numpy(full).to(dev))
         return out
 
+    def _last_rows_only(self, st) -> bool:
+        K = self.n_layer
+        return (self._shard is None and st.drop_p > 0 and st.node_mode == "compact" and st.vals_f is None and
+                st.mess_mult is None and not (self._mess_bits and st.mess_p[K - 1] > 0) and
+                all(d % 4 == 0 for d in st.dims) and
+                bool(_lib.load().ngcf_dense_rows_eligible(st.dims[K - 1], st.dims[K])))
+
+    def _rearm_last(self, st):
+        if st.lastc is None:
+            return
+        list.__setitem__(st.E, self.n_layer, st.lastc.E_rows)
+        list.__setitem__(st.S, self.n_layer - 1, None)
+        st.E._pending = st.S._pending = (weakref.ref(self), weakref.ref(st))
+
+    @_lib.on_device
+    def _complete_last(self, st):
+        if not isinstance(st.E, _PartialLast) or st.E._pending is None:
+            return
+        lib, lc, K = _lib.load(), st.lastc, self.n_layer
+        k, N = K - 1, self.n_user + self.n_item
+        d_in, d_out = st.dims[k], st.dims[K]
+        E_in = list.__getitem__(st.E, k)
+        if k == 0:
+            self._check_fresh(st, "the last layer's output")
+        S = spmm(st.plan.fwd, None, E_in, d_in, drop_p=st.drop_p, seed=st.seed, seed_dev=lc.seed_used, layer=k,
+                 compact=st.comp_f[k])
+        E = torch.empty(N, d_out, dtype=torch.float32, device=S.device)
+        _lib.check(lib.ngcf_dense_fwd(S.data_ptr(), E_in.data_ptr(), N, d_in, d_out, lc.wcat.data_ptr(), lc.bias.data_ptr(),
+                                      LEAKY_SLOPE, None, None, float(st.mess_p[k]), st.seed, lc.seed_used.data_ptr(), k, 0,
+                                      E.data_ptr(), _stream()), "dense_fwd")
+        sel = lc.row_ids >= 0
+        rows = lc.row_ids[sel].long()
+        S[rows] = lc.S[sel]
+        E[rows] = lc.E[sel]
+        list.__setitem__(st.E, K, E)
+        list.__setitem__(st.S, k, S)
+        st.E._pending = st.S._pending = None
+
     @_lib.on_device
     def forward(self, year, u_id, age, sex, month, day, dow, pos_item, neg_item, node_flag):
         lib = _lib.load()
@@ -529,6 +655,8 @@
                 self._xchg.push(self._last.last_partial, sh.r0, sh.rows)
                 self._last.last_partial = None
             st, lib = self._last, _lib.load()
+            if isinstance(st.E, _PartialLast):
+                st.E.complete()
             N, D = self.n_user + self.n_item, sum(st.dims)
             out = torch.empty(N, D, dtype=torch.float32, device=st.E[0].device)
             _lib.check(lib.ngcf_gather_concat(_lib.ptr_array(st.E), _lib.int_array(st.dims), self.n_layer + 1, None, 0,
diff --git a/seoul_tourism_recommendation_ngcf_b200/_lib.py b/seoul_tourism_recommendation_ngcf_b200/_lib.py
--- a/seoul_tourism_recommendation_ngcf_b200/_lib.py
+++ b/seoul_tourism_recommendation_ngcf_b200/_lib.py
@@ -37,6 +37,15 @@
     "ngcf_entry_keys": [_csr_p, _i64, _vp, _vp, _vp],
     "ngcf_node_dropout_compact": [_csr_p, _f32, _u64, _vp, C.c_int, _i64, C.POINTER(_vp), C.POINTER(_vp), C.POINTER(_vp),
                                   C.POINTER(_vp), _vp],
+    "ngcf_batch_rows": [C.POINTER(_vp), C.POINTER(_i64), C.POINTER(_i64), C.c_int, _vp, _vp, _vp, _vp, _vp],
+    "ngcf_node_dropout_compact_cols": [_csr_p, _f32, _u64, _vp, C.c_int, _i64, C.POINTER(_vp), C.POINTER(_vp),
+                                       C.POINTER(_vp), C.POINTER(_vp), _vp, C.c_int, _vp],
+    "ngcf_spmm_rows": [_csr_p, _vp, _vp, _i64, _vp, C.c_int, _vp, _vp, _vp, _vp, _vp, _vp, _vp, _vp],
+    "ngcf_dense_rows_eligible": [C.c_int, C.c_int],
+    "ngcf_dense_fwd_rows": [_vp, _vp, _i64, C.c_int, C.c_int, _vp, _vp, _f32, _f32, _u64, _vp, C.c_int, _vp, _vp, _vp,
+                            _vp],
+    "ngcf_dense_bwd_rows": [_vp, _vp, _i64, C.c_int, _vp, _vp, _vp, _i64, C.c_int, C.c_int, _vp, _vp, _f32, _f32, _u64,
+                            _vp, C.c_int, _vp, _vp, _vp, _vp, _vp, _vp, _vp, _vp],
     "ngcf_node_dropout_bits": [_csr_p, _f32, _u64, _vp, C.c_int, _i64, _vp, _vp, _vp],
     "ngcf_pack_weights": [_vp, _vp, _vp, _vp, C.c_int, C.c_int, _vp, _vp, _vp],
     "ngcf_pack_weights_all": [C.POINTER(_vp), C.POINTER(_vp), C.POINTER(_vp), C.POINTER(_vp), C.POINTER(C.c_int),
diff --git a/seoul_tourism_recommendation_ngcf_b200/csrc/bpr.cu b/seoul_tourism_recommendation_ngcf_b200/csrc/bpr.cu
--- a/seoul_tourism_recommendation_ngcf_b200/csrc/bpr.cu
+++ b/seoul_tourism_recommendation_ngcf_b200/csrc/bpr.cu
@@ -136,7 +136,17 @@
     const int64_t i = blockIdx.x * (int64_t)blockDim.x + threadIdx.x;
     int j; int64_t b;
     if (!locate(s, i, j, b)) return;
-    slot[s.rows[j][b] + s.offset[j]] = (int32_t)i;
+    atomicMin(reinterpret_cast<unsigned int*>(slot) + s.rows[j][b] + s.offset[j], (unsigned int)i);
+}
+
+__global__ void batch_rows_kernel(RowSets s, const int32_t* __restrict__ slot, int32_t* __restrict__ row_ids,
+                                  const uint64_t* __restrict__ seed_dev, uint64_t* __restrict__ seed_used) {
+    const int64_t i = blockIdx.x * (int64_t)blockDim.x + threadIdx.x;
+    if (i == 0) *seed_used = seed_dev ? *seed_dev : 0ull;
+    int j; int64_t b;
+    if (!locate(s, i, j, b)) return;
+    const int64_t row = s.rows[j][b] + s.offset[j];
+    row_ids[i] = slot[row] == (int32_t)i ? (int32_t)row : -1;
 }
 
 __global__ void rowgrad_accum_kernel(RowSets s, int D, const int32_t* __restrict__ slot, float* __restrict__ gsum) {
@@ -295,6 +305,24 @@
     NGCF_LAUNCH_OK("rowgrad_claim_kernel");
     rowgrad_accum_kernel<<<(unsigned)ceil_div64(s.total * 32, 256), 256, 0, st>>>(s, D, slot, gsum);
     NGCF_LAUNCH_OK("rowgrad_accum_kernel");
+    return NGCF_OK;
+}
+
+extern "C" int ngcf_batch_rows(const int64_t* const* rows_host, const int64_t* offsets_host, const int64_t* batch_host,
+                               int n_sets, int32_t* slot, int32_t* row_ids, const uint64_t* seed_dev, uint64_t* seed_used,
+                               void* stream) {
+    NGCF_REQUIRE(slot && row_ids && seed_used, "batch_rows: null pointer");
+    RowSets s;
+    int rc = fill_sets(s, rows_host, offsets_host, nullptr, batch_host, n_sets);
+    if (rc != NGCF_OK) return rc;
+    cudaStream_t st = as_stream(stream);
+    if (s.total > 0) {
+        rowgrad_claim_kernel<<<(unsigned)ceil_div64(s.total, 256), 256, 0, st>>>(s, slot);
+        NGCF_LAUNCH_OK("rowgrad_claim_kernel");
+    }
+    batch_rows_kernel<<<(unsigned)ceil_div64(s.total > 0 ? s.total : 1, 256), 256, 0, st>>>(s, slot, row_ids, seed_dev,
+                                                                                          seed_used);
+    NGCF_LAUNCH_OK("batch_rows_kernel");
     return NGCF_OK;
 }
 
diff --git a/seoul_tourism_recommendation_ngcf_b200/csrc/dense.cu b/seoul_tourism_recommendation_ngcf_b200/csrc/dense.cu
--- a/seoul_tourism_recommendation_ngcf_b200/csrc/dense.cu
+++ b/seoul_tourism_recommendation_ngcf_b200/csrc/dense.cu
@@ -436,7 +436,8 @@
 int ngcf_dense_fwd_tc(const float* S, const float* E, int64_t n_rows, int d_in, int d_out, const float* wcat,
                       const float* bias_eff, float slope, const float* mess_mult, const uint32_t* mess_bits, float mess_p,
                       uint64_t seed,
-                      const uint64_t* seed_dev, int layer, int64_t row_offset, float* E_out, cudaStream_t st);
+                      const uint64_t* seed_dev, int layer, int64_t row_offset, float* E_out, cudaStream_t st,
+                      const int32_t* row_ids = nullptr, float* E_rows = nullptr);
 
 bool ngcf_dense_bwd_tc_eligible(int d_in, int d_out, int gh_normalized);
 int ngcf_dense_bwd_tc(const float* gE_next, const int32_t* slot, const float* gsum, int64_t ld_gsum, int col_off,
@@ -444,7 +445,8 @@
                       const float* W1, const float* W2, float slope, const float* mess_mult, const uint32_t* mess_bits,
                       float mess_p,
                       uint64_t seed, const uint64_t* seed_dev, int layer, int64_t row_offset, int gh_normalized, float* gS, float* gEl,
-                      float* gW1, float* gb1, float* gW2, float* gb2, float* gM_scratch, cudaStream_t st);
+                      float* gW1, float* gb1, float* gW2, float* gb2, float* gM_scratch, cudaStream_t st,
+                      int compact = 0);
 
 extern "C" int ngcf_pack_weights(const float* W1, const float* b1, const float* W2, const float* b2, int d_in,
                                  int d_out, float* wcat, float* bias_eff, void* stream) {
@@ -548,6 +550,43 @@
     return NGCF_OK;
 }
 
+extern "C" int ngcf_dense_rows_eligible(int d_in, int d_out) {
+    return ngcf_dense_fwd_tc_eligible(d_in, d_out) && ngcf_dense_bwd_tc_eligible(d_in, d_out, 1) ? 1 : 0;
+}
+
+extern "C" int ngcf_dense_fwd_rows(const float* S, const float* E, int64_t n, int d_in, int d_out, const float* wcat,
+                                   const float* bias_eff, float slope, float mess_p, uint64_t seed,
+                                   const uint64_t* seed_dev, int layer, const int32_t* row_ids, float* E_out,
+                                   float* E_rows, void* stream) {
+    NGCF_REQUIRE(S && E && wcat && bias_eff && row_ids && E_out, "dense_fwd_rows: null pointer");
+    NGCF_REQUIRE(ngcf_dense_rows_eligible(d_in, d_out), "dense_fwd_rows: widths %d -> %d not taken", d_in, d_out);
+    NGCF_REQUIRE(aligned16(S) && aligned16(E) && aligned16(E_out) && (!E_rows || aligned16(E_rows)),
+                 "dense_fwd_rows: S, E, E_out and E_rows must be 16-byte aligned");
+    NGCF_REQUIRE(mess_p >= 0.f && mess_p < 1.f, "dense_fwd_rows: mess_p %f not in [0,1)", mess_p);
+    NGCF_REQUIRE(n >= 0 && n < ((int64_t)1 << 31), "dense_fwd_rows: n %lld", (long long)n);
+    if (n == 0) return NGCF_OK;
+    return ngcf_dense_fwd_tc(S, E, n, d_in, d_out, wcat, bias_eff, slope, nullptr, nullptr, mess_p, seed, seed_dev, layer,
+                             0, E_out, as_stream(stream), row_ids, E_rows);
+}
+
+extern "C" int ngcf_dense_bwd_rows(const int32_t* row_ids, const float* gsum, int64_t ld_gsum, int col_off,
+                                   const float* E_out, const float* S, const float* E, int64_t n, int d_in, int d_out,
+                                   const float* W1, const float* W2, float slope, float mess_p, uint64_t seed,
+                                   const uint64_t* seed_dev, int layer, float* gS, float* gEl, float* gW1, float* gb1,
+                                   float* gW2, float* gb2, float* gM_scratch, void* stream) {
+    NGCF_REQUIRE(row_ids && gsum && E_out && S && E && W1 && W2 && gS && gEl && gW1 && gb1 && gW2 && gb2 && gM_scratch,
+                 "dense_bwd_rows: null pointer");
+    NGCF_REQUIRE(ngcf_dense_rows_eligible(d_in, d_out), "dense_bwd_rows: widths %d -> %d not taken", d_in, d_out);
+    NGCF_REQUIRE(aligned16(S) && aligned16(E) && aligned16(gS) && aligned16(gEl) && aligned16(gM_scratch),
+                 "dense_bwd_rows: S, E, gS, gEl and gM_scratch must be 16-byte aligned");
+    NGCF_REQUIRE(mess_p >= 0.f && mess_p < 1.f, "dense_bwd_rows: mess_p %f not in [0,1)", mess_p);
+    NGCF_REQUIRE(n >= 0 && n < ((int64_t)1 << 31), "dense_bwd_rows: n %lld", (long long)n);
+    if (n == 0) return NGCF_OK;
+    return ngcf_dense_bwd_tc(nullptr, row_ids, gsum, ld_gsum, col_off, E_out, S, E, n, d_in, d_out, W1, W2, slope,
+                             nullptr, nullptr, mess_p, seed, seed_dev, layer, 0, 1, gS, gEl, gW1, gb1, gW2, gb2,
+                             gM_scratch, as_stream(stream), 1);
+}
+
 namespace {
 __global__ void mess_bits_kernel(int64_t n_rows, int d_out, int words, float p, uint64_t seed0, const uint64_t* seed_dev,
                                  int layer, int64_t row_off, uint32_t* __restrict__ bits) {
diff --git a/seoul_tourism_recommendation_ngcf_b200/csrc/dense_tc.cu b/seoul_tourism_recommendation_ngcf_b200/csrc/dense_tc.cu
--- a/seoul_tourism_recommendation_ngcf_b200/csrc/dense_tc.cu
+++ b/seoul_tourism_recommendation_ngcf_b200/csrc/dense_tc.cu
@@ -40,6 +40,8 @@
     int64_t row_off;
     int64_t ld_in;
     int in_off, w_row1, w_row2, out_off, d_out_full, mode;
+    const int32_t* row_ids;
+    float* E_rows;
 };
 enum { FW_SINGLE = 0, FW_PARTIAL = 1, FW_FINAL = 2 };
 
@@ -80,6 +82,12 @@
         BWD_STAMP(0, it, 3);
         if (!has_chunk) continue;
         const int64_t row_base = (int64_t)tile * TC_ROWS + quarter * 32;
+        int grow[8];
+        if (a.row_ids) {
+            const int rid = row_base + lane < a.n_rows ? a.row_ids[row_base + lane] : -1;
+#pragma unroll
+            for (int i = 0; i < 8; ++i) grow[i] = __shfl_sync(FULL_MASK, rid, i * 4 + rr);
+        }
 #pragma unroll
         for (int j = 0; j < 32; j += 4)
             st_f4(st + stage_off(lane, j >> 2), make_float4(v[j], v[j + 1], v[j + 2], v[j + 3]));
@@ -118,12 +126,17 @@
                     x.x = w & 1u ? x.x * inv_keep : 0.f; x.y = w & 2u ? x.y * inv_keep : 0.f;
                     x.z = w & 4u ? x.z * inv_keep : 0.f; x.w = w & 8u ? x.w * inv_keep : 0.f;
                 } else if (MM == MM_HASH) {
+                    const int64_t krow = a.row_ids ? (int64_t)grow[i] : row + a.row_off;
                     const float4 mm = mess_multiplier4_pre(thr, inv_keep, seed, a.layer,
-                                                           (uint64_t)((row + a.row_off) * a.d_out_full + gcol) >> 2);
+                                                           (uint64_t)(krow * a.d_out_full + gcol) >> 2);
                     x.x *= mm.x; x.y *= mm.y; x.z *= mm.z; x.w *= mm.w;
                 } else if (MM == MM_MULT) {
                     const float4 mm = ld_f4(a.mess_mult + row * a.d_out_full + gcol);
                     x.x *= mm.x; x.y *= mm.y; x.z *= mm.z; x.w *= mm.w;
+                }
+                if (a.row_ids) {
+                    if (grow[i] < 0) x = make_float4(0.f, 0.f, 0.f, 0.f);
+                    else if (a.E_rows) st_f4(a.E_rows + (int64_t)grow[i] * a.d_out_full + gcol, x);
                 }
                 st_f4(dst, x);
             }
@@ -399,7 +412,7 @@
 
 __device__ __forceinline__ uint32_t es_off(int r, int c) { return (uint32_t)r * 256u + (uint32_t)((c ^ (r & 15)) << 4); }
 
-template <int MM, bool PRE>
+template <int MM, bool PRE, bool COMPACT = false>
 __global__ void __launch_bounds__(TC_THREADS, 1) dense_bwd_tc_kernel(BwdTcArgs a) {
     extern __shared__ uint8_t smem_raw[];
     const uint32_t base = (smem_u32(smem_raw) + 1023u) & ~1023u;
@@ -612,7 +625,7 @@
                 if (ok) {
                     h.e[j] = ld_stream_f4(a.E_out + row * a.d_out_full + a.out_off + c0);
                     if (a.gE_next) h.gn[j] = ld_stream_f4(a.gE_next + row * a.d_out_full + a.out_off + c0);
-                    if (a.slot) h.sl[j] = a.slot[row];
+                    if (a.slot) h.sl[j] = COMPACT ? (a.slot[row] >= 0 ? (int)row : -1) : a.slot[row];
                 }
             }
         };
@@ -672,8 +685,9 @@
                     mult = make_float4(w & 1u ? inv_keep : 0.f, w & 2u ? inv_keep : 0.f, w & 4u ? inv_keep : 0.f,
                                        w & 8u ? inv_keep : 0.f);
                 } else if (MM == MM_HASH) {
+                    const int64_t krow = COMPACT ? (int64_t)a.slot[row] : row + a.row_off;
                     mult = mess_multiplier4_pre(thr, inv_keep, seed, a.layer,
-                                                (uint64_t)((row + a.row_off) * a.d_out_full + a.out_off + c0) >> 2);
+                                                (uint64_t)(krow * a.d_out_full + a.out_off + c0) >> 2);
                 }
                 g.x *= mult.x * (e.x > 0.f ? 1.f : a.slope);
                 g.y *= mult.y * (e.y > 0.f ? 1.f : a.slope);
@@ -928,7 +942,7 @@
 int ngcf_dense_fwd_tc(const float* S, const float* E, int64_t n_rows, int d_in, int d_out, const float* wcat,
                       const float* bias_eff, float slope, const float* mess_mult, const uint32_t* mess_bits, float mess_p,
                       uint64_t seed, const uint64_t* seed_dev, int layer, int64_t row_offset, float* E_out,
-                      cudaStream_t st) {
+                      cudaStream_t st, const int32_t* row_ids, float* E_rows) {
     static bool attr_set_dev[64] = {};
     int cur_dev = 0;
     NGCF_CUDA(cudaGetDevice(&cur_dev));
@@ -963,6 +977,7 @@
             a.w_row1 = kh * bk; a.w_row2 = d_in + kh * bk;
             a.out_off = nh * bn; a.d_out_full = d_out;
             a.mode = KH == 1 ? FW_SINGLE : (kh == 0 ? FW_PARTIAL : FW_FINAL);
+            a.row_ids = row_ids; a.E_rows = E_rows;
             const int mm = a.mode == FW_PARTIAL ? MM_NONE : mess_mode(mess_mult, mess_bits, mess_p);
             p.b = a;
             switch (mm) {
@@ -1009,7 +1024,7 @@
                       const float* W1, const float* W2, float slope, const float* mess_mult, const uint32_t* mess_bits,
                       float mess_p, uint64_t seed, const uint64_t* seed_dev, int layer, int64_t row_offset,
                       int gh_normalized, float* gS, float* gEl, float* gW1, float* gb1, float* gW2, float* gb2,
-                      float* gM_scratch, cudaStream_t st) {
+                      float* gM_scratch, cudaStream_t st, int compact) {
     const int bn = d_out > 64 ? 64 : d_out;
     const int IH = d_in / 64, OH = d_out / bn;
     const int KBo = bn / 32;
@@ -1024,6 +1039,9 @@
         case MM_BITS: kern = pre ? dense_bwd_tc_kernel<MM_BITS, true> : dense_bwd_tc_kernel<MM_BITS, false>; break;
         default: kern = pre ? dense_bwd_tc_kernel<MM_HASH, true> : dense_bwd_tc_kernel<MM_HASH, false>; break;
     }
+    if (compact)
+        kern = mess_mode(mess_mult, mess_bits, mess_p) == MM_HASH ? dense_bwd_tc_kernel<MM_HASH, true, true>
+                                                                  : dense_bwd_tc_kernel<MM_NONE, true, true>;
     NGCF_CUDA(cudaFuncSetAttribute(kern, cudaFuncAttributeMaxDynamicSharedMemorySize, 227 * 1024));
     NGCF_CUDA(cudaFuncSetAttribute(wgrad_tc_kernel, cudaFuncAttributeMaxDynamicSharedMemorySize, 227 * 1024));
     for (int ih = 0; ih < IH; ++ih)
diff --git a/seoul_tourism_recommendation_ngcf_b200/csrc/spmm.cu b/seoul_tourism_recommendation_ngcf_b200/csrc/spmm.cu
--- a/seoul_tourism_recommendation_ngcf_b200/csrc/spmm.cu
+++ b/seoul_tourism_recommendation_ngcf_b200/csrc/spmm.cu
@@ -475,6 +475,9 @@
     const uint32_t* key_t;
     int2* out_ent[2][NGCF_MAX_LAYERS];
     int32_t* out_cnt[2][NGCF_MAX_LAYERS];
+    const int32_t* col_slot;
+    int slot_layer;
+    bool want_l, want_t;
 };
 
 constexpr int CW_WARPS = 4;
@@ -486,7 +489,7 @@
     const TileInfo ti{raw.x, raw.y, raw.z, raw.w};
     const int cnt = ti.e1 - ti.e0;
     const int K = a.n_layers;
-    const bool want_l = a.out_ent[0][0] != nullptr, want_t = a.out_ent[1][0] != nullptr;
+    const bool want_l = a.want_l, want_t = a.want_t;
     int2 e[WS_PER];
     uint32_t kl[WS_PER], kt[WS_PER];
 #pragma unroll
@@ -520,21 +523,210 @@
             if (want_t) keep[q] |= node_keep_bits_key(thr, seed, K, kt[q]) << K;
         }
     }
+    const int cs_bit = K + a.slot_layer;
+    int cs[WS_PER];
+#pragma unroll
+    for (int q = 0; q < WS_PER; ++q) {
+        cs[q] = -1;
+        if (a.col_slot && ((keep[q] >> cs_bit) & 1u)) cs[q] = a.col_slot[ent_col(e[q].x)];
+    }
     const uint32_t below = (1u << lane) - 1u;
     for (int c = 0; c < 2 * K; ++c) {
         const int dir = c >= K, layer = dir ? c - K : c;
         int2* out = a.out_ent[dir][layer];
         if (!out) continue;
+        const bool cols = a.col_slot && c == cs_bit;
         int base = 0;
 #pragma unroll
         for (int q = 0; q < WS_PER; ++q) {
-            const bool k = (keep[q] >> c) & 1u;
+            const bool k = cols ? cs[q] >= 0 : ((keep[q] >> c) & 1u);
             const uint32_t m = __ballot_sync(FULL_MASK, k);
-            if (k) out[ti.e0 + base + __popc(m & below)] = e[q];
+            const int2 v = cols ? make_int2((int)(((uint32_t)e[q].x & ~COL_MASK) | (uint32_t)cs[q]), e[q].y) : e[q];
+            if (k) out[ti.e0 + base + __popc(m & below)] = v;
             base += __popc(m);
         }
         if (lane == 0) a.out_cnt[dir][layer][t] = base;
     }
+}
+
+
+constexpr int RW_WARPS = 4;
+struct RowsArgs {
+    const int32_t* row_ids;
+    const int32_t* slot;
+    int64_t n;
+    const TileInfo* tiles;
+    const int32_t* tile_of_row;
+    const int2* cent;
+    const int32_t* ccnt;
+    const TileInfo* ctiles;
+    const int32_t* ctile_of_chunk;
+    const int2* ccent;
+    const int32_t* cccnt;
+    const int32_t* hub_of_row;
+    const int32_t* hub_chunk_ptr;
+    const int32_t* chunk_row;
+    const int32_t* hub_rows;
+    int n_chunks;
+    const float* X;
+    int d;
+    float* partial;
+    float* Y;
+    float* Xrows;
+};
+
+template <int G>
+__global__ void __launch_bounds__(RW_WARPS * 32, 4) spmm_rows_kernel(RowsArgs a) {
+    constexpr int NG = 32 / G;
+    constexpr int NGRP = SP_THREADS / G;
+    constexpr int EPL = SP_TILE_ENT / 32;
+    constexpr int RU = 16;
+    __shared__ __align__(16) float part_s[RW_WARPS][NGRP * G * 4];
+    __shared__ __align__(16) int2 ent_s[RW_WARPS][SP_TILE_ENT];
+    const int lane = threadIdx.x & 31, warp = threadIdx.x >> 5;
+    const int g = lane / G, l = lane % G;
+    const bool ok = l * 4 < a.d;
+    const int64_t w = (int64_t)blockIdx.x * RW_WARPS + warp;
+    pdl_launch_dependents();
+    pdl_wait();
+    TileInfo ti;
+    int cnt, lr;
+    const int2* ent;
+    float* dst;
+    if (w < a.n) {
+        const int r = a.row_ids[w];
+        float4 x = make_float4(0.f, 0.f, 0.f, 0.f);
+        if (r >= 0 && ok) x = ld_f4(a.X + (int64_t)r * a.d + l * 4);
+        if (g == 0 && ok) {
+            st_f4(a.Xrows + w * a.d + l * 4, x);
+            if (r < 0) st_f4(a.Y + w * a.d + l * 4, x);
+        }
+        if (r < 0 || (a.hub_of_row && a.hub_of_row[r] >= 0)) return;
+        const int t = a.tile_of_row[r];
+        const int4 raw = *reinterpret_cast<const int4*>(a.tiles + t);
+        ti = TileInfo{raw.x, raw.y, raw.z, raw.w};
+        cnt = a.ccnt[t]; ent = a.cent + ti.e0; lr = r - ti.r0;
+        dst = a.Y + w * a.d;
+    } else {
+        const int64_t c = w - a.n;
+        if (c >= a.n_chunks) return;
+        if (a.slot[a.chunk_row[c]] < 0) return;
+        const int t = a.ctile_of_chunk[c];
+        const int4 raw = *reinterpret_cast<const int4*>(a.ctiles + t);
+        ti = TileInfo{raw.x, raw.y, raw.z, raw.w};
+        cnt = a.cccnt[t]; ent = a.ccent + ti.e0; lr = (int)c - ti.r0;
+        dst = a.partial + c * a.d;
+    }
+    int2* es = ent_s[warp];
+    int2 ev[EPL];
+#pragma unroll
+    for (int q = 0; q < EPL; ++q) {
+        const int j = q * 32 + lane;
+        ev[q] = j < cnt ? ld_stream_i2(ent + j) : make_int2((int)((uint32_t)SP_TILE_ROWS << LR_SHIFT), 0);
+    }
+    int b0 = 0, b1 = 0;
+#pragma unroll
+    for (int q = 0; q < EPL; ++q) {
+        es[q * 32 + lane] = ev[q];
+        const int lrow = ent_lrow(ev[q].x);
+        b0 += __popc(__ballot_sync(FULL_MASK, lrow < lr));
+        b1 += __popc(__ballot_sync(FULL_MASK, lrow <= lr));
+    }
+    __syncwarp();
+    const int per = (cnt + NGRP - 1) / NGRP;
+    const char* xl = reinterpret_cast<const char*>(a.X + (ok ? l * 4 : 0));
+    const uint32_t row_bytes = (uint32_t)a.d * 4u;
+    float* ps = part_s[warp];
+    const int q1 = b1 > b0 ? b0 / per : 0, q2 = b1 > b0 ? (b1 - 1) / per : -1;
+    for (int q = q1 + g; q <= q2; q += NG) {
+        const int j1 = min(b1, (q + 1) * per);
+        float4 acc = make_float4(0.f, 0.f, 0.f, 0.f);
+        for (int j = max(b0, q * per); j < j1; j += RU) {
+            float wt[RU];
+            float4 x[RU];
+#pragma unroll
+            for (int u = 0; u < RU; ++u) {
+                const int2 e = es[min(j + u, j1 - 1)];
+                wt[u] = j + u < j1 ? __int_as_float(e.y) : 0.f;
+                x[u] = ld_f4(reinterpret_cast<const float*>(xl + (uint64_t)ent_col(e.x) * row_bytes));
+            }
+#pragma unroll
+            for (int u = 0; u < RU; ++u) {
+                acc.x = fmaf(wt[u], x[u].x, acc.x);
+                acc.y = fmaf(wt[u], x[u].y, acc.y);
+                acc.z = fmaf(wt[u], x[u].z, acc.z);
+                acc.w = fmaf(wt[u], x[u].w, acc.w);
+            }
+        }
+        st_f4(ps + (q - q1) * (G * 4) + l * 4, acc);
+    }
+    __syncwarp();
+    if (g == 0 && ok) {
+        float4 y = make_float4(0.f, 0.f, 0.f, 0.f);
+        for (int q = q1; q <= q2; ++q) {
+            const float4 p = ld_f4(ps + (q - q1) * (G * 4) + l * 4);
+            if (q == q1 && b0 > q1 * per) {
+                y = p;
+            } else {
+                y.x += p.x; y.y += p.y; y.z += p.z; y.w += p.w;
+            }
+        }
+        st_f4(dst + l * 4, y);
+    }
+}
+
+template <int G>
+__global__ void __launch_bounds__(HF_THREADS) hub_rows_kernel(RowsArgs a) {
+    constexpr int NGRP = HF_THREADS / G;
+    __shared__ __align__(16) float gs[HF_THREADS * 4];
+    pdl_launch_dependents();
+    const int tid = threadIdx.x, g = tid / G, l = tid % G;
+    const int h = blockIdx.x;
+    const int c0 = a.hub_chunk_ptr[h], c1 = a.hub_chunk_ptr[h + 1];
+    const int row = a.hub_rows[h];
+    pdl_wait();
+    const int s = a.slot[row];
+    if (s < 0) return;
+    const bool ok = l * 4 < a.d;
+    float4 acc = make_float4(0.f, 0.f, 0.f, 0.f);
+    if (ok) {
+        const float* p = a.partial + l * 4;
+        int c = c0 + g;
+        for (; c + 3 * NGRP < c1; c += 4 * NGRP) {
+            float4 x[4];
+#pragma unroll
+            for (int u = 0; u < 4; ++u) x[u] = __ldcg(reinterpret_cast<const float4*>(p + (int64_t)(c + u * NGRP) * a.d));
+#pragma unroll
+            for (int u = 0; u < 4; ++u) { acc.x += x[u].x; acc.y += x[u].y; acc.z += x[u].z; acc.w += x[u].w; }
+        }
+        for (; c < c1; c += NGRP) {
+            const float4 x = __ldcg(reinterpret_cast<const float4*>(p + (int64_t)c * a.d));
+            acc.x += x.x; acc.y += x.y; acc.z += x.z; acc.w += x.w;
+        }
+    }
+    st_f4(gs + g * (G * 4) + l * 4, acc);
+    __syncthreads();
+    if (g == 0 && ok) {
+        float4 sum = acc;
+#pragma unroll
+        for (int q = 1; q < NGRP; ++q) {
+            const float4 v = ld_f4(gs + q * (G * 4) + l * 4);
+            sum.x += v.x; sum.y += v.y; sum.z += v.z; sum.w += v.w;
+        }
+        st_f4(a.Y + (int64_t)s * a.d + l * 4, sum);
+    }
+}
+
+template <int G>
+int launch_rows(const RowsArgs& a, int n_hub, cudaStream_t st) {
+    const int64_t items = a.n + a.n_chunks;
+    NGCF_CUDA(ngcf_launch_pdl(spmm_rows_kernel<G>, dim3((unsigned)ceil_div64(items, RW_WARPS)), dim3(RW_WARPS * 32), 0, st, a));
+    NGCF_LAUNCH_OK("spmm_rows_kernel");
+    if (n_hub > 0) {
+        NGCF_CUDA(ngcf_launch_pdl(hub_rows_kernel<G>, dim3((unsigned)n_hub), dim3(HF_THREADS), 0, st, a));
+        NGCF_LAUNCH_OK("hub_rows_kernel");
+    }
+    return NGCF_OK;
 }
 
 template <int G>
@@ -676,10 +868,10 @@
     return NGCF_OK;
 }
 
-extern "C" int ngcf_node_dropout_compact(const ngcf_csr* g, float drop_p, uint64_t seed, const uint64_t* seed_dev,
-                                         int n_layers, int64_t row_offset, int32_t* const* ent_as_L_host,
-                                         int32_t* const* cnt_as_L_host, int32_t* const* ent_as_Lt_host,
-                                         int32_t* const* cnt_as_Lt_host, void* stream) {
+static int compact_impl(const ngcf_csr* g, float drop_p, uint64_t seed, const uint64_t* seed_dev, int n_layers,
+                        int64_t row_offset, int32_t* const* ent_as_L_host, int32_t* const* cnt_as_L_host,
+                        int32_t* const* ent_as_Lt_host, int32_t* const* cnt_as_Lt_host, const int32_t* col_slot,
+                        int slot_layer, void* stream) {
     int rc = ngcf_check_csr(g, "node_dropout_compact");
     if (rc != NGCF_OK) return rc;
     NGCF_REQUIRE(drop_p > 0.f && drop_p < 1.f, "node_dropout_compact: drop_p %f not in (0,1)", drop_p);
@@ -688,10 +880,18 @@
     NGCF_REQUIRE((ent_as_L_host == nullptr) == (cnt_as_L_host == nullptr) &&
                  (ent_as_Lt_host == nullptr) == (cnt_as_Lt_host == nullptr), "node_dropout_compact: ent/cnt go together");
     NGCF_REQUIRE(row_offset >= 0 && row_offset < ((int64_t)1 << 31), "node_dropout_compact: row_offset");
+    NGCF_REQUIRE(!col_slot || (slot_layer >= 0 && slot_layer < n_layers && ent_as_Lt_host),
+                 "node_dropout_compact: column slots need an L^T output at a layer in [0, %d)", n_layers);
+    bool want_l = false, want_t = false;
     for (int k = 0; k < n_layers; ++k) {
-        NGCF_REQUIRE(!ent_as_L_host || (ent_as_L_host[k] && cnt_as_L_host[k]), "node_dropout_compact: null L output %d", k);
-        NGCF_REQUIRE(!ent_as_Lt_host || (ent_as_Lt_host[k] && cnt_as_Lt_host[k]), "node_dropout_compact: null L^T output %d", k);
-    }
+        NGCF_REQUIRE(!ent_as_L_host || (ent_as_L_host[k] == nullptr) == (cnt_as_L_host[k] == nullptr),
+                     "node_dropout_compact: L output %d: ent/cnt go together", k);
+        NGCF_REQUIRE(!ent_as_Lt_host || (ent_as_Lt_host[k] == nullptr) == (cnt_as_Lt_host[k] == nullptr),
+                     "node_dropout_compact: L^T output %d: ent/cnt go together", k);
+        want_l |= ent_as_L_host && ent_as_L_host[k];
+        want_t |= ent_as_Lt_host && ent_as_Lt_host[k];
+    }
+    NGCF_REQUIRE(want_l || want_t, "node_dropout_compact: no output");
     cudaStream_t st = as_stream(stream);
     for (int pass = 0; pass < 2; ++pass) {
         const int n_tiles = pass ? g->n_chunk_tiles : g->n_tiles;
@@ -701,17 +901,18 @@
         a.ent = reinterpret_cast<const int2*>(pass ? g->hub_ent : g->ent);
         a.row_key = pass ? g->chunk_row : nullptr;
         a.p = drop_p; a.seed = seed; a.seed_dev = seed_dev; a.n_layers = n_layers; a.row_off = (uint32_t)row_offset;
+        a.col_slot = col_slot; a.slot_layer = col_slot ? slot_layer : 0; a.want_l = want_l; a.want_t = want_t;
         const size_t e_off = pass ? (size_t)g->rowptr_nnz : 0, t_off = pass ? (size_t)g->n_tiles : 0;
         if (g->key_l && g->key_t && g->key_row_offset == row_offset) {
             a.key_l = g->key_l + e_off;
             a.key_t = g->key_t + e_off;
         }
         for (int k = 0; k < n_layers; ++k) {
-            if (ent_as_L_host) {
+            if (ent_as_L_host && ent_as_L_host[k]) {
                 a.out_ent[0][k] = reinterpret_cast<int2*>(ent_as_L_host[k]) + e_off;
                 a.out_cnt[0][k] = cnt_as_L_host[k] + t_off;
             }
-            if (ent_as_Lt_host) {
+            if (ent_as_Lt_host && ent_as_Lt_host[k]) {
                 a.out_ent[1][k] = reinterpret_cast<int2*>(ent_as_Lt_host[k]) + e_off;
                 a.out_cnt[1][k] = cnt_as_Lt_host[k] + t_off;
             }
@@ -720,6 +921,65 @@
         NGCF_LAUNCH_OK(pass ? "compact_kernel(hub chunks)" : "compact_kernel(rows)");
     }
     return NGCF_OK;
+}
+
+extern "C" int ngcf_node_dropout_compact(const ngcf_csr* g, float drop_p, uint64_t seed, const uint64_t* seed_dev,
+                                         int n_layers, int64_t row_offset, int32_t* const* ent_as_L_host,
+                                         int32_t* const* cnt_as_L_host, int32_t* const* ent_as_Lt_host,
+                                         int32_t* const* cnt_as_Lt_host, void* stream) {
+    for (int k = 0; k < n_layers && k < NGCF_MAX_LAYERS; ++k) {
+        NGCF_REQUIRE(!ent_as_L_host || (ent_as_L_host[k] && cnt_as_L_host && cnt_as_L_host[k]),
+                     "node_dropout_compact: null L output %d", k);
+        NGCF_REQUIRE(!ent_as_Lt_host || (ent_as_Lt_host[k] && cnt_as_Lt_host && cnt_as_Lt_host[k]),
+                     "node_dropout_compact: null L^T output %d", k);
+    }
+    return compact_impl(g, drop_p, seed, seed_dev, n_layers, row_offset, ent_as_L_host, cnt_as_L_host, ent_as_Lt_host,
+                        cnt_as_Lt_host, nullptr, 0, stream);
+}
+
+extern "C" int ngcf_node_dropout_compact_cols(const ngcf_csr* g, float drop_p, uint64_t seed, const uint64_t* seed_dev,
+                                              int n_layers, int64_t row_offset, int32_t* const* ent_as_L_host,
+                                              int32_t* const* cnt_as_L_host, int32_t* const* ent_as_Lt_host,
+                                              int32_t* const* cnt_as_Lt_host, const int32_t* col_slot, int slot_layer,
+                                              void* stream) {
+    return compact_impl(g, drop_p, seed, seed_dev, n_layers, row_offset, ent_as_L_host, cnt_as_L_host, ent_as_Lt_host,
+                        cnt_as_Lt_host, col_slot, slot_layer, stream);
+}
+
+extern "C" int ngcf_spmm_rows(const ngcf_csr* g, const int32_t* row_ids, const int32_t* slot, int64_t n, const float* X,
+                              int d, const int32_t* c_ent, const int32_t* c_cnt, const int32_t* tile_of_row,
+                              const int32_t* tile_of_chunk, float* hub_partial, float* Y, float* Xrows, void* stream) {
+    int rc = ngcf_check_csr(g, "spmm_rows");
+    if (rc != NGCF_OK) return rc;
+    NGCF_REQUIRE(row_ids && slot && X && Y && Xrows && c_ent && c_cnt && tile_of_row, "spmm_rows: null pointer");
+    NGCF_REQUIRE(n >= 0 && n < ((int64_t)1 << 31), "spmm_rows: n %lld", (long long)n);
+    NGCF_REQUIRE(d > 0 && d <= NGCF_MAX_WIDTH && d % 4 == 0, "spmm_rows: width %d (multiples of 4 up to %d)", d,
+                 NGCF_MAX_WIDTH);
+    NGCF_REQUIRE(aligned16(X) && aligned16(Y) && aligned16(Xrows), "spmm_rows: X, Y and Xrows must be 16-byte aligned");
+    const bool hubs = g->n_hub > 0 && g->n_chunks > 0;
+    NGCF_REQUIRE(!hubs || (hub_partial && aligned16(hub_partial) && g->hub_rows && tile_of_chunk && g->chunk_tiles),
+                 "spmm_rows: hub arrays missing");
+    if (n == 0) return NGCF_OK;
+    RowsArgs a{};
+    a.row_ids = row_ids; a.slot = slot; a.n = n;
+    a.tiles = reinterpret_cast<const TileInfo*>(g->tiles); a.tile_of_row = tile_of_row;
+    a.cent = reinterpret_cast<const int2*>(c_ent); a.ccnt = c_cnt;
+    if (hubs) {
+        a.ctiles = reinterpret_cast<const TileInfo*>(g->chunk_tiles); a.ctile_of_chunk = tile_of_chunk;
+        a.ccent = reinterpret_cast<const int2*>(c_ent) + g->rowptr_nnz; a.cccnt = c_cnt + g->n_tiles;
+        a.hub_of_row = g->hub_of_row; a.hub_chunk_ptr = g->hub_chunk_ptr; a.chunk_row = g->chunk_row;
+        a.hub_rows = g->hub_rows; a.n_chunks = g->n_chunks;
+    }
+    a.X = X; a.d = d; a.partial = hub_partial; a.Y = Y; a.Xrows = Xrows;
+    cudaStream_t st = as_stream(stream);
+    const int nh = hubs ? g->n_hub : 0;
+    const int d4 = d / 4;
+    if (d4 <= 1) return launch_rows<1>(a, nh, st);
+    if (d4 <= 2) return launch_rows<2>(a, nh, st);
+    if (d4 <= 4) return launch_rows<4>(a, nh, st);
+    if (d4 <= 8) return launch_rows<8>(a, nh, st);
+    if (d4 <= 16) return launch_rows<16>(a, nh, st);
+    return launch_rows<32>(a, nh, st);
 }
 
 extern "C" int ngcf_debug_spmm_timeline(unsigned long long* dev_buf_or_null) {
diff --git a/seoul_tourism_recommendation_ngcf_b200/graph.py b/seoul_tourism_recommendation_ngcf_b200/graph.py
--- a/seoul_tourism_recommendation_ngcf_b200/graph.py
+++ b/seoul_tourism_recommendation_ngcf_b200/graph.py
@@ -92,6 +92,7 @@
         g, loss, grads, last = entry
         g.replay()
         self.model._last, self.model._all_E = last, None
+        self.model._rearm_last(last)
         if self.optimizer is not None:
             from . import _lib
             _lib.bump_param_epoch()
diff --git a/seoul_tourism_recommendation_ngcf_b200/plan.py b/seoul_tourism_recommendation_ngcf_b200/plan.py
--- a/seoul_tourism_recommendation_ngcf_b200/plan.py
+++ b/seoul_tourism_recommendation_ngcf_b200/plan.py
@@ -120,6 +120,12 @@
             self.tile_hubmask = (bits & 0xFFFFFFFF).to(torch.int32)
         else:
             self.tile_hubmask = None
+        i32 = dict(dtype=torch.int32, device=dev)
+        self.tile_of_row = torch.repeat_interleave(torch.arange(self.tiles.shape[0], **i32),
+                                                   (self.tiles[:, 1] - self.tiles[:, 0]).to(torch.int64))
+        self.tile_of_chunk = torch.repeat_interleave(
+            torch.arange(self.chunk_tiles.shape[0], **i32),
+            (self.chunk_tiles[:, 1] - self.chunk_tiles[:, 0]).to(torch.int64)) if self.n_chunks else None
         self.ent = None
         self.key_l = self.key_t = None
         self.key_row_offset = 0
@@ -308,7 +314,8 @@
 
 
 def node_dropout_compact(side: CsrSide, drop_p: float, seed: int, seed_dev, n_layers: int, row_offset: int = 0,
-                         as_L: bool = True, as_Lt: bool = False, static_keys: bool = True):
+                         as_L: bool = True, as_Lt: bool = False, static_keys: bool = True, col_slot=None,
+                         slot_layer: int = 0):
     lib = _lib.load()
     dev = side.rowptr.device
     if static_keys:
@@ -332,9 +339,13 @@
 
     el, tl = arrs(cl)
     et, tt = arrs(ct)
-    _lib.check(lib.ngcf_node_dropout_compact(C.byref(side.descriptor(None)), float(drop_p), int(seed) & (2 ** 64 - 1),
-                                             _lib.ptr(seed_dev), int(n_layers), int(row_offset), el, tl, et, tt,
-                                             _stream()), "node_dropout_compact")
+    args = (C.byref(side.descriptor(None)), float(drop_p), int(seed) & (2 ** 64 - 1), _lib.ptr(seed_dev), int(n_layers),
+            int(row_offset), el, tl, et, tt)
+    if col_slot is None:
+        _lib.check(lib.ngcf_node_dropout_compact(*args, _stream()), "node_dropout_compact")
+    else:
+        _lib.check(lib.ngcf_node_dropout_compact_cols(*args, col_slot.data_ptr(), int(slot_layer), _stream()),
+                   "node_dropout_compact_cols")
     return cl, ct
 
 
```
